# shwetabhardwaj44/EfficientVideoClassification_Youtube8M

Measured on AMD Instinct MI355X. Metric: frames/sec (whole node) H-LSTM teacher+student B=256x300x1152; GAP@20, higher is better.
Workload: dtype bf16; 1 GPU; HierarchicalLstmModel teacher_student every_n=10, lstm_cells=1024x2, MoE(2), batch 256 x 300 x 1152 per GPU; global_batch=256, frames_per_video=300, parallelism=dp1, num_frames=U{120..300}

## Files before the change

efficientvideoclassification_youtube8m_amd/_lib.py:

```python
from __future__ import annotations

import ctypes as C
import os

_HERE = os.path.dirname(os.path.abspath(__file__))
LIB_PATH = os.environ.get("EVC_LIB", os.path.join(_HERE, "libevc_hip.so"))

vp, i32, i64, f32 = C.c_void_p, C.c_int, C.c_int64, C.c_float

SIGNATURES = {
    "evc_check_device": [i32],
    "evc_l2norm_chunk_fwd": [vp, vp, vp, i32, i32, i32, i32, vp, i32, i32, vp, i32, vp, vp, i32, vp, i32, vp, i32, vp],
    "evc_sort_rows_by_len": [vp, i32, i32, vp, vp, vp, vp],
    "evc_frame_counts": [vp, i32, i32, i32, i32, i32, i32, vp, vp, vp, vp],
    "evc_gemm_nt": [vp, i64, vp, i64, vp, i64, i32, i32, i32, vp, i32, i32, vp],
    "evc_gemm_nt_sqnorm": [vp, i64, vp, i64, vp, i64, i32, i32, i32, vp, f32, vp, vp, i64, vp],
    "evc_gemm_tn": [vp, i64, vp, i64, vp, i64, i32, i32, i32, i32, i32, vp],
    "evc_gemm_tn2": [vp, i64, vp, i64, i32, vp, i64, i32, i32, vp, i64, i32, i32, i32, i32, vp],
    "evc_gemm_tn2_rows": [vp, i64, vp, i64, i32, vp, i64, i32, i32, vp, i64, i32, i32, i32, vp, i32, i32, vp],
    "evc_gemm_tn2_slabs": [vp, i64, vp, i64, i32, vp, i64, i32, i32, vp, i64, i64, i32, i32, i32, i32, vp],
    "evc_sum_slabs": [vp, i64, i32, i32, i32, i64, vp, i64, i32, vp],
    "evc_colsum_bf16": [vp, i64, i32, i32, i32, vp, vp],
    "evc_colsum_bf16_det": [vp, i64, i32, i32, i32, vp, vp, i32, vp],
    "evc_lstm_layer_fwd": [vp, vp, vp, vp, i32, i32, i32, i32, i32, vp, vp, vp, vp, i64, vp, vp, vp, vp, vp],
    "evc_lstm_layer_fwd_hp": [vp, vp, i64, vp, i64, vp, vp, i32, i32, i32, i32, vp, vp, vp, vp, vp, i64, vp, vp, vp],
    "evc_gemm_nt_split": [vp, i64, vp, i64, vp, i64, i32, i32, i32, vp, vp],
    "evc_cast_f32_to_f16_wide": [vp, i64, i32, i32, i32, i32, i32, vp, vp],
    "evc_cast_f32_to_bf16_wide": [vp, i64, i32, i32, vp, i64, i32, vp],
    "evc_lstm_layer_fwd_f16": [vp, i64, vp, vp, vp, i32, i32, i32, i32, vp, i32, vp, vp, vp, i64, vp, vp, vp, vp, vp],
    "evc_lstm_layer_fwd_f16_fp8lo": [vp, i64, i32, i64, i32, vp, vp, i32, i32, vp, vp, i32, i32, i32, vp, vp, vp, vp, i64, vp, vp, vp, vp, vp, vp, i32, vp],
    "evc_l2norm_chunk_int": [vp, vp, i32, i32, i32, i32, vp, i32, i32, vp, vp, vp, vp, vp, vp, i32, vp, i32, vp],
    "evc_lstm_level2_fwd_high": [vp, i64, i32, i64, i32, vp, vp, i32, i32, vp, vp, vp, i32, vp, i64, vp, vp, i32, i32, i32, vp, vp, vp, vp, vp, vp, vp, vp, i64,
                                 vp, vp, vp, vp, vp, vp, vp],
    "evc_lstm_layer_fwd_f16_dith": [vp, i64, i32, i64, i32, vp, i64, vp, i64, i32, vp, vp, i32, i32, i32, vp, vp, vp, vp, i64, vp, vp, vp, vp, vp],
    "evc_cast_f32_to_f16_dither": [vp, i64, i32, i64, C.c_uint32, vp, i64, i64, vp],
    "evc_lstm_stack2_fwd_f16_fp8lo": [vp, i32, vp, vp, vp, vp, vp, i32, i32, vp, vp, i32, i32, i32, i32, vp, vp, vp, vp, vp, vp, vp, vp, vp, i64, vp, vp, vp, vp, vp],
    "evc_cast_f32_to_fp8_lo": [vp, i64, i32, i32, i32, i32, i32, vp, i64, vp],
    "evc_cast_f32_to_fp8_lohi": [vp, i64, i32, i32, i32, i32, i32, vp, i64, vp],
    "evc_lstm_layer_bwd": [vp, vp, i32, i32, i32, i32, vp, vp, vp, vp, i64, vp, vp, vp, vp, vp, vp, vp, vp, vp],
    "evc_transpose_to_bf16": [vp, i32, i64, i32, i32, vp, i64, i32, i32, vp],
    "evc_cast_f32_to_bf16": [vp, i64, i32, i32, vp, i64, vp],
    "evc_cast_f32_to_f16": [vp, i64, i32, i32, vp, i64, vp],
    "evc_cast_f32_to_bf16_split": [vp, i64, i32, i32, vp, vp, i64, vp],
    "evc_rowsum_bf16": [vp, i64, i32, i32, vp, vp],
    "evc_lstm_stack2_fwd_f16": [vp, i32, vp, i32, vp, vp, vp, vp, i32, i32, i32, i32, vp, vp, vp, vp, vp, vp, vp, vp, vp, i64, vp, vp, vp, vp, vp],
    "evc_cast_f32_to_f16_segs": [vp, i64, i32, i32, i32, vp, vp],
    "evc_cast_f32_to_f16_wlo": [vp, i64, i32, i32, i32, vp, vp],
    "evc_lstm_level2_fwd": [vp, vp, vp, vp, vp, vp, i32, i32, i32, i32, vp, vp, vp, vp, vp, vp, i64, vp, vp, vp, vp, vp, vp, vp],
    "evc_lstm_stack2_fwd": [vp, vp, vp, vp, vp, vp, i32, i32, i32, i32, vp, vp, vp, vp, vp, vp, vp, i64, vp, vp, vp, vp, vp],
    "evc_moe_grad_update": [vp, i64, vp, i64, i32, i32, i32, vp, vp, vp, vp, vp, i64, f32, vp, vp, f32, f32, f32, f32, f32, vp],
    "evc_moe_grad_update_wide": [vp, i64, vp, i64, i32, i32, i32, vp, vp, vp, vp, vp, i64, vp, vp, vp, i32, i32, f32, vp, vp, f32, f32, f32, f32, f32, vp],
    "evc_gram_slabs": [vp, i64, i32, i32, i32, vp, vp],
    "evc_moe_grad_norms": [vp, i32, vp, i32, i32, vp, i64, vp, i64, vp, i32, i32, f32, vp, vp, vp, vp],
    "evc_moe_grad_update_apply": [vp, i64, vp, i64, i32, i32, i32, vp, vp, vp, vp, vp, i64, vp, vp, vp, i32, i32, f32, vp, vp, f32, f32, f32, f32, f32, vp, vp],
    "evc_gemm_nt_f16_fp8": [vp, i64, vp, i64, vp, i64, vp, i64, vp, i64, i32, i32, i32, i32, i32, vp, vp],
    "evc_cast_f32_to_f16_fp8x": [vp, i64, i32, i32, i32, i32, vp, vp],
    "evc_absmax_partials": [vp, i64, i32, i32, vp, vp],
    "evc_cast_f32_to_f16_fp8x_dyn": [vp, i64, i32, i32, i32, i32, vp, vp, vp],
    "evc_gemm_nt_f16_fp8_dyn": [vp, i64, vp, i64, vp, i64, vp, i64, vp, i64, i32, i32, i32, i32, i32, vp, i32, vp, vp],
    "evc_moe_grad_update_phase": [vp, i64, vp, i64, i32, i32, i32, vp, vp, vp, vp, vp, i64, f32, vp, vp, f32, f32, f32, f32, f32, i32, vp],
    "evc_moe_tail_fwd": [vp, vp, i32, i32, i32, vp, vp, vp],
    "evc_moe_tail_bwd": [vp, vp, vp, i32, i32, i32, vp, i64, vp, i64, vp],
    "evc_ce_loss": [vp, vp, i32, i32, f32, vp, vp, i32, vp],
    "evc_ce_loss_ordered": [vp, vp, i32, i32, f32, vp, vp, i32, vp, vp],
    "evc_rep_loss_ordered": [vp, vp, i32, i32, f32, vp, vp, i32, vp, vp],
    "evc_kl_pred_loss": [vp, vp, vp, vp, i32, i32, f32, vp, vp, i32, vp],
    "evc_kl_pred_loss_ordered": [vp, vp, vp, vp, i32, i32, f32, vp, vp, i32, vp, vp],
    "evc_rep_loss": [vp, vp, i32, i32, f32, vp, vp, i32, vp],
    "evc_distill_losses": [vp, vp, vp, vp, vp, vp, vp, i32, i32, i32, f32, f32, f32, vp, vp, vp, vp, vp],
    "evc_distill_losses_multi": [vp, vp, vp, vp, i32, vp, vp, vp, vp, vp, vp, vp, vp, i32, i32, i32, vp, vp, vp],
    "evc_distill_losses_ensemble": [i32, vp, vp, vp, vp, i32, vp, vp, vp, i32, i32, i32, f32, f32, f32, vp, vp, vp, vp, vp, vp, vp],
    "evc_distill_losses_sparse": [i32, vp, vp, i32, vp, i32, vp, vp, i32, i32, f32, f32, vp, vp, vp, vp, vp],
    "evc_label_loss": [i32, vp, vp, i32, i32, f32, vp, vp, vp, i32, vp, vp],
    "evc_grad_sqnorm": [vp, vp, f32, i64, vp, vp],
    "evc_clip_adam_step": [vp, vp, vp, vp, i64, f32, vp, f32, f32, f32, f32, f32, vp, vp],
    "evc_clip_adam_small": [i32, vp, vp, vp, vp, vp, vp, f32, f32, f32, f32, f32, vp],
    "evc_sqnorm2_partials": [vp, i64, vp, i64, vp, vp],
    "evc_lstm_adam_fused": [vp, vp, vp, vp, vp, vp, vp, vp, i32, i32, vp, vp, vp, f32, f32, f32, f32, f32, vp, vp, i64, vp, i64, i32, i32,
                            vp, i64, i32, i32, i32, i32, i32, vp],
    "evc_adam2d_fused": [vp, vp, vp, vp, i32, i32, vp, vp, f32, f32, f32, f32, f32, vp, vp, i64, vp, i64, vp, i64, i32, i32, i32, vp],
    "evc_meanpool_fwd": [vp, vp, vp, i32, i32, i32, i32, vp, vp, vp],
    "evc_sigmoid_fwd": [vp, i64, vp],
    "evc_sigmoid_bwd": [vp, vp, i64, vp, vp],
    "evc_sample_frames_gather": [vp, vp, vp, vp, i32, i32, i32, i32, i32, vp, vp, vp],
    "evc_sample_sequence_gather": [vp, vp, vp, vp, i32, i32, i32, i32, i32, vp, vp, vp],
    "evc_relu6_fwd": [vp, i64, vp, vp, vp],
    "evc_relu6_bwd": [vp, vp, i64, vp, vp, vp],
    "evc_framepool_mean_fwd": [vp, i32, i32, i32, vp, vp, vp],
    "evc_framepool_mean_bwd": [vp, i32, i32, i32, vp, vp],
    "evc_bn_stats": [vp, i32, i32, vp, vp, vp, vp],
    "evc_bn_apply": [vp, i32, i32, vp, vp, vp, vp, i32, vp, vp, vp],
    "evc_bn_relu6_bwd": [vp, vp, i32, i32, vp, vp, vp, vp, i32, vp, i32, vp, vp, vp, vp, vp, vp],
# ... 14 lines not shown
    "evc_netvlad_softmax_bwd": [vp, vp, i32, i32, vp, vp],
    "evc_netvlad_aggregate_fwd": [vp, vp, i32, i32, i32, i32, vp, vp, vp, vp, vp, vp, vp, vp],
    "evc_netvlad_aggregate_bwd": [vp, vp, i32, i32, i32, i32, vp, vp, vp, vp, vp, vp, vp, vp, vp],
    "evc_netvlad_aggregate_packed_fwd": [vp, vp, vp, i32, i32, i32, i32, i32, i32, vp, vp, vp, vp, vp, vp, vp, vp],
    "evc_netvlad_aggregate_packed_bwd": [vp, vp, vp, i32, i32, i32, i32, i32, i32, vp, vp, vp, vp, vp, vp, vp, vp, vp, i64, vp],
    "evc_netvlad_dcenters": [vp, vp, i32, i32, i32, vp, vp],
    "evc_netvlad_normalize_fwd": [vp, i32, i32, i32, vp, vp, vp, vp, vp],
    "evc_netvlad_normalize_bwd": [vp, vp, vp, vp, i32, i32, i32, vp, vp],
    "evc_nextvlad_assign_fwd": [vp, i32, i32, i32, vp, vp, vp, vp, vp, i64, vp, vp, vp],
    "evc_nextvlad_assign_bwd": [vp, i32, i32, i32, vp, vp, vp, vp, vp, i64, vp, vp, vp, vp, vp, i64, vp],
    "evc_nextvlad_aggregate_fwd": [vp, vp, i32, i32, i32, i32, i32, vp, vp, vp, vp],
    "evc_nextvlad_aggregate_bwd": [vp, vp, i32, i32, i32, i32, i32, vp, vp, vp, vp, vp, i64, vp],
    "evc_nextvlad_aggregate_packed_fwd": [vp, vp, vp, i32, i32, i32, i32, i32, i32, i32, vp, vp, vp, vp],
    "evc_nextvlad_aggregate_packed_fwd_mfma": [vp, vp, vp, i32, i32, i32, i32, i32, i32, i32, vp, vp, vp, vp],
    "evc_nextvlad_aggregate_packed_bwd": [vp, vp, vp, i32, i32, i32, i32, i32, i32, i32, vp, vp, vp, vp, vp, i64, vp],
    "evc_frames_gather_packed": [vp, vp, vp, vp, i32, i32, i32, i32, i32, i32, i32, vp, vp, vp],
    "evc_frames_gather_packed_sel": [vp, vp, vp, vp, vp, i32, i32, i32, i32, i32, i32, i32, i32, vp, vp, vp],
    "evc_scatter_rows": [vp, i64, vp, i32, i32, i32, vp, i64, vp],
    "evc_nextvlad_normalize_fwd": [vp, i32, i32, i32, vp, vp, vp],
    "evc_nextvlad_normalize_bwd": [vp, vp, vp, i32, i32, i32, vp, vp],
    "evc_nextvlad_gate_fwd": [vp, vp, i64, vp, vp],
    "evc_nextvlad_gate_bwd": [vp, vp, vp, i64, vp, vp, vp, vp],
    "evc_nextvlad_gate_bwd_add": [vp, vp, vp, vp, i64, vp, vp, vp, vp],
    "evc_nextvlad_colsum": [vp, i64, i32, i32, vp, vp, i64, vp],
    "evc_nextvlad_center_cast": [vp, i32, i32, vp, vp, vp],
    "evc_nextvlad_bias_logits": [vp, vp, i32, i32, vp, vp, i32, vp],
    "evc_nextvlad_wgrad_uncenter": [vp, vp, vp, i32, i32, vp, vp],
    "evc_nextvlad_dropout_fwd": [vp, i32, i32, vp, vp, vp, vp, C.c_uint32, f32, C.c_uint32, C.c_uint32, C.c_uint64, vp, vp],
    "evc_nextvlad_dropout_bwd": [vp, i32, i32, C.c_uint32, f32, C.c_uint32, C.c_uint32, C.c_uint64, vp],
    "evc_dbof_workspace": [i32, i32, vp, vp, vp],
    "evc_dbof_gather": [vp, vp, vp, vp, i32, i32, i32, i32, i32, vp, vp, vp, vp],
    "evc_bn_partials_reduce": [vp, i32, i32, vp, vp],
    "evc_bn_finalize_ema": [vp, i32, i32, vp, vp, vp, vp, f32, vp],
    "evc_dbof_input_bn_apply": [vp, i32, i32, i32, vp, vp, vp, vp, vp, vp, vp, vp],
    "evc_dbof_cluster_pool_fwd": [vp, vp, vp, vp, i32, i32, i32, i32, vp, vp, vp, vp, vp, vp],
    "evc_dbof_input_bn_apply_f16fp8": [vp, i32, i32, i32, vp, vp, vp, vp, vp, i32, i32, vp, vp],
    "evc_dbof_cluster_pool_fwd_f16fp8": [vp, vp, vp, i32, i32, i32, i32, i32, vp, vp, vp, vp, vp, vp],
    "evc_dbof_pool_finish": [vp, i32, i32, vp, vp, vp, vp, vp, vp, vp, vp],
    "evc_dbof_dact": [vp, vp, vp, vp, vp, vp, vp, vp, i32, i32, i32, i32, vp, vp, vp],
    "evc_gemm_tn_slabs": [vp, i64, vp, i64, vp, i32, i32, i32, i32, vp],
    "evc_dbof_wgrad_finish": [vp, i32, i32, i32, vp, vp, vp, vp, vp, vp, vp],
    "evc_topk_rows": [vp, i32, i32, i32, i32, vp, vp, vp],
    "evc_eval_select_rows": [vp, i32, vp, i32, i32, i32, i32, vp, vp, vp, vp, vp, vp, vp],
    "evc_ensemble_topk_rows": [vp, vp, vp, i32, vp, vp, i32, i32, i32, i32, i32, i32, vp, vp, vp, i64, vp],
    "evc_student_frame_select": [vp, i32, i32, i32, i32, C.c_uint32, C.c_uint32, i32, vp, vp],
    "evc_l2norm_chunk_sel_fwd": [vp, vp, vp, vp, i32, i32, i32, i32, i32, vp, i32, vp, i32, vp, i32, vp],
    "evc_l2norm_chunk_sel_int": [vp, vp, vp, i32, i32, i32, i32, i32, vp, vp, vp, vp, i32, vp],
    "evc_frame_change_keys": [vp, vp, vp, i32, i32, i32, vp, vp],
    "evc_student_frame_select_scored": [vp, vp, i32, i32, i32, i32, vp, vp],
    "evc_cascade_confidence_rows": [vp, i64, vp, i32, i32, i32, i32, vp, vp, i64, vp, vp],
    "evc_cascade_pick_rows": [vp, vp, vp, i32, f32, i32, vp, vp, vp, vp],
}
EXPORTS = tuple(SIGNATURES) + ("evc_version", "evc_last_error")

_lib = None


class EvcError(RuntimeError):
    pass


def load():
    global _lib
    if _lib is not None:
        return _lib
    if not os.path.exists(LIB_PATH):
        raise EvcError(
            "libevc_hip.so not found at %s - build it with "
            "`python -c 'import __graft_entry__ as g; g.build()'` or csrc/build.sh. "
            "There is no CPU fallback for the HIP kernels." % LIB_PATH)
    import torch
    lib = C.CDLL(LIB_PATH)
    for name, args in SIGNATURES.items():
        fn = getattr(lib, name)
        fn.argtypes = args
        fn.restype = C.c_int
    lib.evc_version.argtypes = []
    lib.evc_version.restype = C.c_int
    lib.evc_last_error.argtypes = []
    lib.evc_last_error.restype = C.c_char_p
    _lib = lib
    return lib


def call(name, *args):
    lib = load()
    rc = getattr(lib, name)(*args)
    if rc != 0:
        raise EvcError("%s failed (%d): %s" % (name, rc, lib.evc_last_error().decode()))
```

efficientvideoclassification_youtube8m_amd/csrc/evc_elementwise.hip:

```cpp
#include <stdarg.h>
#include "evc_common.h"
#include <mutex>

static thread_local char g_err[512] = "";
void evc_set_error(const char* fmt, ...) {
  va_list ap;
  va_start(ap, fmt);
  vsnprintf(g_err, sizeof(g_err), fmt, ap);
  va_end(ap);
}
extern "C" const char* evc_last_error(void) { return g_err; }
extern "C" int evc_version(void) { return EVC_VERSION; }
extern "C" int evc_check_device(int dev) {
  hipDeviceProp_t prop;
  EVC_CHECK_HIP(hipGetDeviceProperties(&prop, dev));
  EVC_REQUIRE(strncmp(prop.gcnArchName, "gfx950", 6) == 0, EVC_ERR_UNSUPPORTED_ARCH,
              "device %d is %s; libevc_hip is built for gfx950 only", dev, prop.gcnArchName);
  return EVC_OK;
}

__device__ __forceinline__ float block_sum(float v, float* sh) {
  v = wave_sum(v);
  const int lane = threadIdx.x & 63, w = threadIdx.x >> 6, nw = (blockDim.x + 63) >> 6;
  __syncthreads();
// ... 1748 lines not shown
  for (int s = 1; s < S; ++s) {
    const float v = yp[(long)s * C];
    if (v > best) { best = v; bi = s; }
  }
  const long o = (long)b * C + c;
  if (pf) pf[o] = best;
  if (pb) pb[o] = f32_to_bf16(best);
  if (am) am[o] = bi;
}
extern "C" int evc_framepool_max_fwd(const float* y, int B, int S, int C, float* pooled_f32, evc_bf16* pooled_bf16,
                                     int32_t* argmax, void* stream) {
  EVC_REQUIRE(B > 0 && S > 0 && C > 0, EVC_ERR_BAD_SHAPE, "evc_framepool_max_fwd: bad shape");
  hipLaunchKernelGGL(framepool_max_fwd_kernel, dim3((C + 255) / 256, B), dim3(256), 0, (hipStream_t)stream, y, S, C, pooled_f32,
                     pooled_bf16, argmax);
  EVC_LAUNCH_CHECK();
  return EVC_OK;
}
__global__ void framepool_max_bwd_kernel(const float* __restrict__ dp, const int* __restrict__ am, int S, int C, long n,
                                         float* __restrict__ dy) {
  for (long i = (long)blockIdx.x * blockDim.x + threadIdx.x; i < n; i += (long)gridDim.x * blockDim.x) {
    const int c = (int)(i % C);
    const long bs = i / C;
    const int s = (int)(bs % S);
    const long b = bs / S;
    dy[i] = (am[b * C + c] == s) ? dp[b * C + c] : 0.f;
  }
}
extern "C" int evc_framepool_max_bwd(const float* dpooled, const int32_t* argmax, int B, int S, int C, float* dy, void* stream) {
  EVC_REQUIRE(B > 0 && S > 0 && C > 0, EVC_ERR_BAD_SHAPE, "evc_framepool_max_bwd: bad shape");
  const long n = (long)B * S * C;
  hipLaunchKernelGGL(framepool_max_bwd_kernel, dim3(grid_for(n)), dim3(256), 0, (hipStream_t)stream, dpooled, argmax, S, C, n, dy);
  EVC_LAUNCH_CHECK();
  return EVC_OK;
}

__global__ void fill_kernel(float* p, long n, float v) {
  const long stride = (long)gridDim.x * blockDim.x, tid = (long)blockIdx.x * blockDim.x + threadIdx.x;
  if ((((uintptr_t)p) & 15) == 0) {
    const long n4 = n >> 2;
    const float4 v4 = make_float4(v, v, v, v);
    for (long i = tid; i < n4; i += stride) ((float4*)p)[i] = v4;
    for (long i = (n4 << 2) + tid; i < n; i += stride) p[i] = v;
  } else {
    for (long i = tid; i < n; i += stride) p[i] = v;
  }
}
extern "C" int evc_fill_f32(float* p, int64_t n, float value, void* stream) {
  EVC_REQUIRE(n > 0, EVC_ERR_BAD_SHAPE, "evc_fill_f32: n");
  hipLaunchKernelGGL(fill_kernel, dim3(grid_for(n)), dim3(256), 0, (hipStream_t)stream, p, (long)n, value);
  EVC_LAUNCH_CHECK();
  return EVC_OK;
}

__global__ void occupy_kernel(long long ticks) {
  extern __shared__ char occ_lds[];
  if (threadIdx.x == 0) occ_lds[0] = 0;
  const long long t0 = wall_clock64();
  while (wall_clock64() - t0 < ticks) __builtin_amdgcn_s_sleep(32);
  if (occ_lds[0] == 1) occ_lds[1] = 2;
}
extern "C" int evc_debug_occupy(int blocks, int threads, int lds_bytes, double microseconds, void* stream) {
  EVC_REQUIRE(blocks > 0 && blocks <= 1024 && threads >= 64 && threads <= 1024 && lds_bytes >= 0 && lds_bytes <= 160 * 1024 && microseconds >= 0,
              EVC_ERR_BAD_ARG, "evc_debug_occupy: blocks=%d threads=%d lds=%d us=%g", blocks, threads, lds_bytes, microseconds);
  if (lds_bytes > 64 * 1024) (void)hipFuncSetAttribute((const void*)occupy_kernel, hipFuncAttributeMaxDynamicSharedMemorySize, lds_bytes);
  hipLaunchKernelGGL(occupy_kernel, dim3(blocks), dim3(threads), lds_bytes, (hipStream_t)stream, (long long)(microseconds * 100.0));
  EVC_LAUNCH_CHECK();
  return EVC_OK;
}

extern "C" int evc_stream_create_cu_mask(const unsigned* mask, int words, void** stream_out) {
  EVC_REQUIRE(mask != nullptr && stream_out != nullptr && words > 0 && words <= 32, EVC_ERR_BAD_ARG, "evc_stream_create_cu_mask: words=%d", words);
  hipStream_t s = nullptr;
  hipError_t e = hipExtStreamCreateWithCUMask(&s, (uint32_t)words, mask);
  EVC_REQUIRE(e == hipSuccess, EVC_ERR_HIP, "hipExtStreamCreateWithCUMask: %s", hipGetErrorString(e));
  *stream_out = (void*)s;
  return EVC_OK;
}

extern "C" int evc_stream_destroy(void* stream) {
  EVC_REQUIRE(stream != nullptr, EVC_ERR_BAD_ARG, "evc_stream_destroy: null stream");
  hipError_t e = hipStreamDestroy((hipStream_t)stream);
  EVC_REQUIRE(e == hipSuccess, EVC_ERR_HIP, "hipStreamDestroy: %s", hipGetErrorString(e));
  return EVC_OK;
}
```

efficientvideoclassification_youtube8m_amd/csrc/evc_gemm_tn.hip:

```cpp
#include "gemm_shared.h"

struct StoreParamsT {
  float* C; long ldc; int M, N;
  int row_il_H;
  int accumulate, splits, ksteps_per_split;
  long slab_stride;
};

template <class Cfg, bool SEG = false>
__global__ __launch_bounds__(Cfg::NT) void gemm_tn_kernel(GemmOperandsT p, StoreParamsT s, int tiles_m, int tiles_n) {
  const int nwg = tiles_m * tiles_n;
  int bid = blockIdx.x, split = 0;
  if (s.splits > 1) {
    split = bid / nwg;
    bid -= split * nwg;
  }
  const int id = xcd_remap(bid, nwg);
  int tm, tn;
  tile_of(id, tiles_m, tiles_n, tm, tn, s.splits > 1 ? patch_rows(nwg, tiles_n) : 8);
  const int m0 = tm * Cfg::BM;
  int n0 = tn * Cfg::BU;
  int nb = n0;
  if (p.B2) {
    if (n0 >= p.N1) {
      p.B = p.B2; p.ldb = p.ldb2; nb = n0 - p.N1; p.N = s.N - p.N1;
      s.N = p.c_col2 + p.N;
      n0 = p.c_col2 + nb;
    } else {
      p.N = s.N = p.N1;
    }
  }
  if (SEG) {
    int off = split * s.ksteps_per_split, sg = 0;
    p.nk = min(s.ksteps_per_split, p.nk - off);
#pragma unroll
    for (int i = 0; i < 15; ++i) {
      const bool adv = sg == i && i + 1 < p.nseg && off >= (int)p.seg_len[i];
      off -= adv ? (int)p.seg_len[i] : 0;
      sg += adv ? 1 : 0;
    }
    p.seg0 = sg; p.seg_off0 = off;
  } else if (s.splits > 1) {
    const int k0 = split * s.ksteps_per_split;
    p.A += (long)k0 * 32 * p.lda;
    p.B += (long)k0 * 32 * p.ldb;
    p.nk = min(s.ksteps_per_split, p.nk - k0);
  }
  f32x4 acc[Cfg::MI][1][Cfg::NI];
  gemm_mainloop_tn<Cfg, true, TN_LOOP_MODE, SEG>(p, m0, nb, lds_dyn, acc);
  float* C = s.C + split * s.slab_stride;
  const int wave = threadIdx.x >> 6, wc = wave % Cfg::WC;
  const bool plain = s.slab_stride > 0 || (s.splits == 1 && !s.accumulate);
  const bool aligned = (s.ldc % 4) == 0 && ((uintptr_t)C % 16) == 0 && n0 + wc * Cfg::WU + Cfg::WU <= s.N;
  __syncthreads();
  if (plain && aligned) {
    store_tile_via_lds<Cfg, 4, false>(acc, lds_dyn, C, s.ldc, s.M, s.N, m0, n0, nullptr, s.row_il_H);
  } else if (s.splits == 1 && s.accumulate && aligned) {
    store_tile_via_lds<Cfg, 4, false, true>(acc, lds_dyn, C, s.ldc, s.M, s.N, m0, n0, nullptr, s.row_il_H);
  } else if (plain) {
    TileCoordsT<Cfg> tc;
#pragma unroll
    for (int mi = 0; mi < Cfg::MI; ++mi) {
      const int m = m0 + tc.row0 + mi * 16;
      if (m >= s.M) continue;
      const long mo = s.row_il_H > 0 ? (long)(m & 3) * s.row_il_H + (m >> 2) : m;
#pragma unroll
      for (int ni = 0; ni < Cfg::NI; ++ni)
#pragma unroll
        for (int r = 0; r < 4; ++r) {
          const int n = n0 + tc.unit0 + ni * 16 + r;
          if (n < s.N) C[mo * s.ldc + n] = acc[mi][0][ni][r];
        }
    }
  } else {
    store_tile_via_lds<Cfg, 4, true>(acc, lds_dyn, C, s.ldc, s.M, s.N, m0, n0, nullptr, s.row_il_H);
  }
}

static int tn_args_ok(const char* entry, const void* A, int64_t lda, const void* B, int64_t ldb, int M, int N, int K, int row_interleave_H,
                      int N1, const void* B2, int64_t ldb2, int c_col2, int nslab = 1, bool slabs_ok = true) {
  EVC_REQUIRE(M >= 8 && N >= 8 && K > 0 && M % 8 == 0 && N % 8 == 0 && K % 32 == 0, EVC_ERR_BAD_SHAPE,
              "%s: needs M %% 8 == 0, N %% 8 == 0, K %% 32 == 0 (M=%d N=%d K=%d)", entry, M, N, K);
  EVC_REQUIRE(nslab >= 1 && nslab <= K / 32, EVC_ERR_BAD_SHAPE, "%s: needs 1 <= nslab <= K/32 (K=%d nslab=%d)", entry, K, nslab);
  EVC_REQUIRE(lda % 8 == 0 && ldb % 8 == 0 && ((uintptr_t)A % 16) == 0 && ((uintptr_t)B % 16) == 0, EVC_ERR_BAD_ALIGN,
              "%s: operands must be 16-byte aligned (lda=%ld ldb=%ld)", entry, (long)lda, (long)ldb);
  EVC_REQUIRE(slabs_ok, EVC_ERR_BAD_ALIGN, "%s: slabs == NULL or slab_stride < M * ldc", entry);
  EVC_REQUIRE(row_interleave_H == 0 || M == 4 * row_interleave_H, EVC_ERR_BAD_SHAPE, "%s: row_interleave_H needs M == 4*H", entry);
  EVC_REQUIRE(!B2 || (N1 > 0 && N1 < N && N1 % 256 == 0 && ldb2 % 8 == 0 && ((uintptr_t)B2 % 16) == 0 && c_col2 >= N1), EVC_ERR_BAD_SHAPE,
              "%s: N1=%d must be a multiple of 256 inside (0, N=%d), B2 16-byte aligned with ldb2 %% 8 == 0, c_col2=%d >= N1", entry, N1, N, c_col2);
  EVC_REQUIRE((long)ceil_div(K / 32, nslab) * (nslab - 1) < K / 32, EVC_ERR_BAD_SHAPE, "%s: nslab=%d leaves an empty slab at K=%d", entry, nslab, K);
  return EVC_OK;
}

static inline GemmOperandsT tn_operands(const evc_bf16* A, int64_t lda, const evc_bf16* B, int64_t ldb, int M, int N, int K,
                                        int N1 = 0, const evc_bf16* B2 = nullptr, int64_t ldb2 = 0, int c_col2 = 0) {
  GemmOperandsT p{A, lda, B, ldb, M, N, K / 32};
  if (B2) { p.B2 = B2; p.ldb2 = ldb2; p.N1 = N1; p.c_col2 = c_col2; }
  return p;
}

static bool tn_live_segments(GemmOperandsT& p, int K, int slab_rows, const int32_t* rows_per_slab) {
  if (slab_rows % 32 != 0 || K % slab_rows != 0) return false;
  const int nslabs = K / slab_rows, slab_steps = slab_rows / 32;
  const long ld_max = p.lda > p.ldb ? p.lda : p.ldb;
  if ((long)nslabs * slab_steps >= 65536 || (long)K * (p.B2 && p.ldb2 > ld_max ? p.ldb2 : ld_max) * 2 >= (1L << 32)) return false;
  int n = 0, total = 0;
  for (int t = 0; t < nslabs; ++t) {
    const int r = rows_per_slab[t] < 0 ? 0 : (rows_per_slab[t] > slab_rows ? slab_rows : rows_per_slab[t]);
    const int steps = (r + 31) / 32;
    if (steps == 0) continue;
    if (n == 16) return false;
    p.seg_start[n] = (unsigned short)(t * slab_steps); p.seg_len[n] = (unsigned short)steps;
    ++n; total += steps;
  }
  if (total == 0 || total >= K / 32) return false;
  p.nseg = n; p.nk = total;
  return true;
}

template <class Cfg>
static int launch_tn(const GemmOperandsT& p, StoreParamsT s, bool seg, int tm, int tn, hipStream_t st) {
  s.ksteps_per_split = ceil_div(p.nk, s.splits);
  if (seg) launch_cfg<Cfg>(gemm_tn_kernel<Cfg, true>, tm * tn * s.splits, st, p, s, tm, tn);
  else launch_cfg<Cfg>(gemm_tn_kernel<Cfg>, tm * tn * s.splits, st, p, s, tm, tn);
  EVC_LAUNCH_CHECK();
  return EVC_OK;
}

static int gemm_tn_impl(const char* entry, const evc_bf16* A, int64_t lda, const evc_bf16* B, int64_t ldb, int N1, const evc_bf16* B2, int64_t ldb2,
                        int c_col2, float* C, int64_t ldc, int M, int N, int K, int row_interleave_H, int accumulate, void* stream,
                        int slab_rows = 0, const int32_t* rows_per_slab = nullptr) {
  EVC_TRY(tn_args_ok(entry, A, lda, B, ldb, M, N, K, row_interleave_H, N1, B2, ldb2, c_col2));
  hipStream_t st = (hipStream_t)stream;
  GemmOperandsT p = tn_operands(A, lda, B, ldb, M, N, K, N1, B2, ldb2, c_col2);
  const bool seg = rows_per_slab && slab_rows > 0 && !evc_deterministic() && tn_live_segments(p, K, slab_rows, rows_per_slab);
  K = p.nk * 32;
  StoreParamsT s{C, ldc, M, N, row_interleave_H, accumulate, 1, 0, 0};
  const int tm1 = ceil_div(M, 128), tn1 = ceil_div(N, 128);
  const bool short128 = forced_tile() == 11 || (forced_tile() == 0 && K <= 2048 && (long)tm1 * tn1 >= 192);
  const bool strip128 = !short128 && forced_tile() == 0 && N <= 128 && !B2;
  const bool tile128 = short128 || strip128;
  const int tm = tile128 ? tm1 : ceil_div(M, CfgPlainV2::BM), tn = short128 ? tn1 : strip128 ? 1 : ceil_div(N, CfgPlainV2::BU);
  if (!short128 && !evc_deterministic()) s.splits = split_k(256 / (tm * tn), p.nk, 32);
  if (s.splits > 1 && !accumulate) EVC_CHECK_HIP(hipMemset2DAsync(C, ldc * sizeof(float), 0, (size_t)N * sizeof(float), M, st));
  return tile128 ? launch_tn<CfgTn128>(p, s, seg, tm, tn, st) : launch_tn<CfgPlainV2>(p, s, seg, tm, tn, st);
}

extern "C" int evc_gemm_tn2_rows(const evc_bf16* A, int64_t lda, const evc_bf16* B1, int64_t ldb1, int N1, const evc_bf16* B2, int64_t ldb2,
                                 int N2, int c_col2, float* C, int64_t ldc, int M, int slab_rows, int nslabs, const int32_t* rows_per_slab,
                                 int row_interleave_H, int accumulate, void* stream) {
  EVC_REQUIRE(B1 && N1 > 0 && slab_rows > 0 && nslabs > 0 && rows_per_slab && (long)slab_rows * nslabs < (1L << 31), EVC_ERR_BAD_ARG,
              "evc_gemm_tn2_rows: B1, N1, slab_rows, nslabs, rows_per_slab are required");
  EVC_REQUIRE(!B2 || N2 > 0, EVC_ERR_BAD_ARG, "evc_gemm_tn2_rows: N2=%d", N2);
  EVC_REQUIRE(!B2 || accumulate || c_col2 == N1, EVC_ERR_BAD_ARG, "evc_gemm_tn2_rows: segments that are not adjacent in C (c_col2=%d, N1=%d) need accumulate", c_col2, N1);
  return gemm_tn_impl("evc_gemm_tn2_rows", A, lda, B1, ldb1, B2 ? N1 : 0, B2, ldb2, B2 ? c_col2 : 0, C, ldc, M, N1 + (B2 ? N2 : 0), slab_rows * nslabs,
                      row_interleave_H, accumulate, stream, slab_rows, rows_per_slab);
}

extern "C" int evc_gemm_tn(const evc_bf16* A, int64_t lda, const evc_bf16* B, int64_t ldb, float* C, int64_t ldc,
                           int M, int N, int K, int row_interleave_H, int accumulate, void* stream) {
  return gemm_tn_impl("evc_gemm_tn", A, lda, B, ldb, 0, nullptr, 0, 0, C, ldc, M, N, K, row_interleave_H, accumulate, stream);
}

extern "C" int evc_gemm_tn2(const evc_bf16* A, int64_t lda, const evc_bf16* B1, int64_t ldb1, int N1, const evc_bf16* B2, int64_t ldb2,
                            int N2, int c_col2, float* C, int64_t ldc, int M, int K, int row_interleave_H, int accumulate, void* stream) {
  EVC_REQUIRE(B1 && B2 && N1 > 0 && N2 > 0, EVC_ERR_BAD_ARG, "evc_gemm_tn2: two column segments are required");
  EVC_REQUIRE(accumulate || c_col2 == N1, EVC_ERR_BAD_ARG, "evc_gemm_tn2: segments that are not adjacent in C (c_col2=%d, N1=%d) need accumulate "
              "(the split-K join adds into a C the caller has zeroed)", c_col2, N1);
  return gemm_tn_impl("evc_gemm_tn2", A, lda, B1, ldb1, N1, B2, ldb2, c_col2, C, ldc, M, N1 + N2, K, row_interleave_H, accumulate, stream);
}

static int gemm_tn_slabs_impl(const char* entry, const evc_bf16* A, int64_t lda, const evc_bf16* B1, int64_t ldb1, int N1, const evc_bf16* B2, int64_t ldb2,
                              int N2, int c_col2, float* slabs, int64_t ldc, int64_t slab_stride, int M, int K, int row_interleave_H, int nslab, void* stream) {
  const int N = N1 + (B2 ? N2 : 0);
  EVC_REQUIRE(N1 >= 8, EVC_ERR_BAD_SHAPE, "%s: N1=%d", entry, N1);
  EVC_TRY(tn_args_ok(entry, A, lda, B1, ldb1, M, N, K, row_interleave_H, N1, B2, ldb2, c_col2, nslab, slabs && slab_stride >= (int64_t)M * ldc));
  return launch_tn<CfgPlainV2>(tn_operands(A, lda, B1, ldb1, M, N, K, N1, B2, ldb2, c_col2), StoreParamsT{slabs, ldc, M, N, row_interleave_H, 0, nslab, 0, slab_stride},
                               false, ceil_div(M, CfgPlainV2::BM), ceil_div(N, CfgPlainV2::BU), (hipStream_t)stream);
}
extern "C" int evc_gemm_tn2_slabs(const evc_bf16* A, int64_t lda, const evc_bf16* B1, int64_t ldb1, int N1, const evc_bf16* B2, int64_t ldb2,
                                  int N2, int c_col2, float* slabs, int64_t ldc, int64_t slab_stride, int M, int K, int row_interleave_H,
                                  int nslab, void* stream) {
  return gemm_tn_slabs_impl("evc_gemm_tn2_slabs", A, lda, B1, ldb1, N1, B2, ldb2, N2, c_col2, slabs, ldc, slab_stride, M, K, row_interleave_H, nslab, stream);
}
extern "C" int evc_gemm_tn_slabs(const evc_bf16* A, int64_t lda, const evc_bf16* B, int64_t ldb, float* slabs, int M, int N, int K,
                                 int nslab, void* stream) {
  return gemm_tn_slabs_impl("evc_gemm_tn_slabs", A, lda, B, ldb, N, nullptr, 0, 0, 0, slabs, N, (int64_t)M * N, M, K, 0, nslab, stream);
}

__global__ __launch_bounds__(256) void sum_slabs_kernel(const float* __restrict__ slabs, long slab_stride, int nslab, int M, int N4, long ld,
                                                        float* __restrict__ C, long ldc, int accumulate) {
  const long n = (long)M * N4;
  for (long i = (long)blockIdx.x * 256 + threadIdx.x; i < n; i += (long)gridDim.x * 256) {
    const long r = i / N4, c = (i - r * N4) * 4;
    float4 a = accumulate ? *(const float4*)(C + r * ldc + c) : make_float4(0.f, 0.f, 0.f, 0.f);
    for (int s = 0; s < nslab; ++s) {
      const float4 v = *(const float4*)(slabs + s * slab_stride + r * ld + c);
      a.x += v.x; a.y += v.y; a.z += v.z; a.w += v.w;
    }
    *(float4*)(C + r * ldc + c) = a;
  }
}
extern "C" int evc_sum_slabs(const float* slabs, int64_t slab_stride, int nslab, int M, int N, int64_t ld, float* C, int64_t ldc, int accumulate,
                             void* stream) {
  EVC_REQUIRE(slabs && C && nslab >= 1 && M > 0 && N > 0 && N % 4 == 0 && ld % 4 == 0 && ldc % 4 == 0 && slab_stride % 4 == 0 &&
              ((uintptr_t)slabs % 16) == 0 && ((uintptr_t)C % 16) == 0, EVC_ERR_BAD_SHAPE, "evc_sum_slabs: N, ld, ldc, slab_stride multiples of 4, 16-byte aligned");
  const long n = (long)M * (N / 4);
  long nb = (n + 255) / 256;
  nb = nb > 2048 ? 2048 : nb;
  hipLaunchKernelGGL(sum_slabs_kernel, dim3((unsigned)nb), dim3(256), 0, (hipStream_t)stream, slabs, (long)slab_stride, nslab, M, N / 4, (long)ld, C, (long)ldc,
                     accumulate);
  EVC_LAUNCH_CHECK();
  return EVC_OK;
}

struct MoeUpdateParams {
  float* p; float* m; float* v;
  bf16_t* p_bf16;
  bf16_t* pT_bf16; long ldT;
  bf16_t* p_wide;
  bf16_t* p_f16; uint8_t* p_fp8;
  float lo_scale, hi_scale;
  float* partial;
  float* wsq_partial;
  const float* sums;
  int V, K;
  float l2, clip, lr_t, b1, b2, eps;
};

__device__ __forceinline__ float4 ld_stream_moe(const float* p) {
  const f32x4 v = __builtin_nontemporal_load((const f32x4*)p);
// ... 294 lines not shown
```

efficientvideoclassification_youtube8m_amd/csrc/evc_lstm_bwd.hip:

```cpp
#include "gemm_shared.h"

struct LstmBwdParams {
  const int* len; int t;
  const uint2* gates;
  const bf16_t* c_new; const bf16_t* c_old;
  const float* dS_c; const float* dS_h; long ld_dS;
  const bf16_t* dh_above;
  float* dc_ws;
  int dc_bf16;
  uint2* dz4;
  const int* row_map;
  float* db;
  int m_active;
  int M, H;
  int fused_above;
};

static inline int bwd_dc_bf16() {
  static int v = -1;
  if (v < 0) { const char* e = getenv("EVC_BWD_DC_BF16"); v = (e && e[0] == '1') ? 1 : 0; }
  return v;
}

struct LstmBwdIn {
  int ln;
  float4 dcv;
  float4 dhs;
  uint2 dha;
  uint4 g01, g23;
  uint2 cnq, coq;
};

__device__ __forceinline__ void lstm_bwd_load(const LstmBwdParams& e, const int m, const int u, const bool in_range, LstmBwdIn& q) {
  q.ln = in_range ? e.len[m] : -1;
  q.dcv = q.dhs = make_float4(0.f, 0.f, 0.f, 0.f);
  q.dha = q.cnq = q.coq = make_uint2(0u, 0u);
  q.g01 = q.g23 = make_uint4(0u, 0u, 0u, 0u);
  if (e.t >= q.ln) return;
  const long hu = (long)m * e.H + u;
  if (e.t == q.ln - 1) {
    const long su = (long)(e.row_map ? e.row_map[m] : m) * e.ld_dS + u;
    q.dhs = *(const float4*)(e.dS_h + su);
    q.dcv = *(const float4*)(e.dS_c + su);
  } else {
    if (e.dc_bf16) {
      const uint2 d = *(const uint2*)((const bf16_t*)e.dc_ws + hu);
      q.dcv = make_float4(__uint_as_float(d.x << 16), __uint_as_float(d.x & 0xffff0000u), __uint_as_float(d.y << 16), __uint_as_float(d.y & 0xffff0000u));
    } else {
      q.dcv = *(const float4*)(e.dc_ws + hu);
    }
  }
  if (e.dh_above) q.dha = *(const uint2*)(e.dh_above + hu);
  const uint4* gp = (const uint4*)(e.gates + hu);
  q.g01 = gp[0]; q.g23 = gp[1];
  q.cnq = *(const uint2*)(e.c_new + hu);
  if (e.c_old) q.coq = *(const uint2*)(e.c_old + hu);
}

__device__ __forceinline__ void lstm_bwd_finish(const LstmBwdParams& e, const int m, const int u, const float (&dh_in)[4],
                                                const LstmBwdIn& q, float (&dzv)[4][4]) {
#pragma unroll
  for (int r = 0; r < 4; ++r)
#pragma unroll
    for (int g = 0; g < 4; ++g) dzv[r][g] = 0.f;
  if (q.ln < 0) return;
  const long hu = (long)m * e.H + u;
  uint4* dzp = (uint4*)(e.dz4 + hu);
  if (e.t >= q.ln) {
    dzp[0] = make_uint4(0u, 0u, 0u, 0u);
    dzp[1] = make_uint4(0u, 0u, 0u, 0u);
    return;
  }
  float dh[4] = {dh_in[0], dh_in[1], dh_in[2], dh_in[3]};
  if (e.t == q.ln - 1) {
    if (e.fused_above) { dh[0] += q.dhs.x; dh[1] += q.dhs.y; dh[2] += q.dhs.z; dh[3] += q.dhs.w; }
    else { dh[0] = q.dhs.x; dh[1] = q.dhs.y; dh[2] = q.dhs.z; dh[3] = q.dhs.w; }
  }
  if (e.dh_above) {
    dh[0] += __uint_as_float(q.dha.x << 16); dh[1] += __uint_as_float(q.dha.x & 0xffff0000u);
    dh[2] += __uint_as_float(q.dha.y << 16); dh[3] += __uint_as_float(q.dha.y & 0xffff0000u);
  }
  const float dci[4] = {q.dcv.x, q.dcv.y, q.dcv.z, q.dcv.w};
  const uint2 recs[4] = {make_uint2(q.g01.x, q.g01.y), make_uint2(q.g01.z, q.g01.w), make_uint2(q.g23.x, q.g23.y), make_uint2(q.g23.z, q.g23.w)};
  const float cna[4] = {__uint_as_float(q.cnq.x << 16), __uint_as_float(q.cnq.x & 0xffff0000u),
                        __uint_as_float(q.cnq.y << 16), __uint_as_float(q.cnq.y & 0xffff0000u)};
  const float coa[4] = {__uint_as_float(q.coq.x << 16), __uint_as_float(q.coq.x & 0xffff0000u),
                        __uint_as_float(q.coq.y << 16), __uint_as_float(q.coq.y & 0xffff0000u)};
  float dcn[4];
  uint2 dzr[4];
#pragma unroll
  for (int r = 0; r < 4; ++r) {
    const uint2 rec = recs[r];
    const float gi = __uint_as_float(rec.x << 16), gj = __uint_as_float(rec.x & 0xffff0000u);
    const float gf = __uint_as_float(rec.y << 16), go = __uint_as_float(rec.y & 0xffff0000u);
    const float tcv = tanhf_(cna[r]);
    const float cp = coa[r];
    const float dc = dci[r] + dh[r] * go * (1.f - tcv * tcv);
    dcn[r] = dc * gf;
    dzv[r][0] = dc * gj * gi * (1.f - gi); dzv[r][1] = dc * gi * (1.f - gj * gj);
    dzv[r][2] = dc * cp * gf * (1.f - gf); dzv[r][3] = dh[r] * tcv * go * (1.f - go);
    dzr[r] = make_uint2(pack_bf16x2(dzv[r][0], dzv[r][1]), pack_bf16x2(dzv[r][2], dzv[r][3]));
  }
  if (e.dc_bf16) *(uint2*)((bf16_t*)e.dc_ws + hu) = make_uint2(pack_bf16x2(dcn[0], dcn[1]), pack_bf16x2(dcn[2], dcn[3]));
  else *(float4*)(e.dc_ws + hu) = make_float4(dcn[0], dcn[1], dcn[2], dcn[3]);
  dzp[0] = make_uint4(dzr[0].x, dzr[0].y, dzr[1].x, dzr[1].y);
  dzp[1] = make_uint4(dzr[2].x, dzr[2].y, dzr[3].x, dzr[3].y);
}

template <int BM, int BU, int NT>
__device__ __forceinline__ void lstm_bwd_zero_tile(const LstmBwdParams& e, int m0, int u0) {
  const int cols = min(BU, e.H - u0) / 2;
  for (int i = threadIdx.x; i < BM * cols; i += NT) {
    const int m = m0 + i / cols, u = u0 + (i % cols) * 2;
    if (m < e.M) *(uint4*)(e.dz4 + (long)m * e.H + u) = make_uint4(0u, 0u, 0u, 0u);
  }
}

constexpr int BWD_TAIL_PRE = 8;
template <int N>
struct BwdTailRows {
  unsigned long long dcv[N], dhs[N];
  uint4 grec[N];
  uint32_t cn[N], co[N], dha[N];
};
__device__ __forceinline__ int bwd_tail_len(const LstmBwdParams& e, int m) {
  return m < e.M ? ((const __attribute__((address_space(4))) int*)e.len)[m] : -1;
}
template <int N>
__device__ __forceinline__ void lstm_bwd_tail_load(const LstmBwdParams& e, int m0, int u, bool u_in, int wave, int p0, BwdTailRows<N>& r) {
#pragma unroll
  for (int i = 0; i < N; ++i) {
    const int m = m0 + (p0 + i) * 8 + wave;
    const int ln = u_in ? bwd_tail_len(e, m) : -1;
    r.dcv[i] = r.dhs[i] = 0ull;
    r.grec[i] = make_uint4(0u, 0u, 0u, 0u);
    r.cn[i] = r.co[i] = r.dha[i] = 0u;
    if (e.t < ln) {
      const long hu = (long)m * e.H + u;
      const bool last = e.t == ln - 1;
      long su = 0;
      if (last) su = (long)(e.row_map ? ((const __attribute__((address_space(4))) int*)e.row_map)[m] : m) * e.ld_dS + u;
      if (e.dc_bf16 && !last) {
        const uint32_t d = *(const uint32_t*)((const bf16_t*)e.dc_ws + hu);
        r.dcv[i] = (unsigned long long)(d << 16) | ((unsigned long long)(d & 0xffff0000u) << 32);
      } else {
        r.dcv[i] = *(const unsigned long long*)(last ? e.dS_c + su : e.dc_ws + hu);
      }
      if (last) r.dhs[i] = *(const unsigned long long*)(e.dS_h + su);
      if (e.dh_above) r.dha[i] = *(const uint32_t*)(e.dh_above + hu);
      r.grec[i] = *(const uint4*)(e.gates + hu);
      r.cn[i] = *(const uint32_t*)(e.c_new + hu);
      if (e.c_old) r.co[i] = *(const uint32_t*)(e.c_old + hu);
    }
  }
}
template <int RS, int N>
__device__ __forceinline__ void lstm_bwd_tail_finish(const LstmBwdParams& e, int m0, int u, bool u_in, int lane, int wave, int p0, const BwdTailRows<N>& r,
                                                     const char* lds, float (&bs)[2][4]) {
  float2 dcn[N];
// ... 67 lines not shown
        *(f32x4*)(lds + (wr * Cfg::WM + mi * 16 + l) * RS + (wc * Cfg::WU + ni * 16 + g * 4) * 4) = acc[mi][0][ni];
    __syncthreads();
  }
  const int u = u0 + lane * 2;
  const bool u_in = u < e.H;
  float bs[2][4] = {{0.f, 0.f, 0.f, 0.f}, {0.f, 0.f, 0.f, 0.f}};
  constexpr int SLOTS = Cfg::BM / 8;
  constexpr int GROUP = PRE > 0 ? 8 : 4;
  static_assert(PRE % 4 == 0 && PRE <= SLOTS && (SLOTS - PRE) % GROUP == 0, "tile rows must divide into 8 waves x (PRE + k GROUP)");
  if constexpr (PRE > 0) {
    if constexpr (PRE < SLOTS) {
      BwdTailRows<GROUP> nb;
      lstm_bwd_tail_load<GROUP>(e, m0, u, u_in, wave, PRE, nb);
      lstm_bwd_tail_finish<RS, PRE>(e, m0, u, u_in, lane, wave, 0, pre, lds, bs);
#pragma unroll
      for (int p0 = PRE; p0 < SLOTS; p0 += GROUP) {
        lstm_bwd_tail_finish<RS, GROUP>(e, m0, u, u_in, lane, wave, p0, nb, lds, bs);
        if (p0 + GROUP < SLOTS) lstm_bwd_tail_load<GROUP>(e, m0, u, u_in, wave, p0 + GROUP, nb);
      }
    } else {
      lstm_bwd_tail_finish<RS, PRE>(e, m0, u, u_in, lane, wave, 0, pre, lds, bs);
    }
  } else {
#pragma unroll 1
    for (int p0 = 0; p0 < SLOTS; p0 += GROUP) {
      BwdTailRows<GROUP> cur;
      lstm_bwd_tail_load<GROUP>(e, m0, u, u_in, wave, p0, cur);
      lstm_bwd_tail_finish<RS, GROUP>(e, m0, u, u_in, lane, wave, p0, cur, lds, bs);
    }
  }
  if (e.db) {
    float* red = (float*)lds;
    __syncthreads();
    *(float4*)(red + ((wave * 128) + lane * 2) * 4) = make_float4(bs[0][0], bs[0][1], bs[0][2], bs[0][3]);
    *(float4*)(red + ((wave * 128) + lane * 2 + 1) * 4) = make_float4(bs[1][0], bs[1][1], bs[1][2], bs[1][3]);
    __syncthreads();
    const int uu = threadIdx.x >> 2, gg = threadIdx.x & 3;
    float v = 0.f;
#pragma unroll
    for (int w = 0; w < 8; ++w) v += red[(w * 128 + uu) * 4 + gg];
    if (u0 + uu < e.H) atomicAdd(e.db + (long)gg * e.H + u0 + uu, v);
  }
}

template <class Cfg, bool BATCH_LOADS = true>
__device__ __forceinline__ void lstm_bwd_step_body(const GemmOperands& p, const LstmBwdParams& e, int bid, int tiles_m, int tiles_n) {
  static_assert(Cfg::G == 1, "bwd step is a plain GEMM over the H units");
  const int nwg = tiles_m * tiles_n;
  const int id = xcd_remap(bid, nwg);
  int tm, tn;
  tile_of(id, tiles_m, tiles_n, tm, tn);
  const int m0 = tm * Cfg::BM, u0 = tn * Cfg::BU;
  if (m0 >= e.m_active) {
    lstm_bwd_zero_tile<Cfg::BM, Cfg::BU, Cfg::NT>(e, m0, u0);
    return;
  }
  f32x4 acc[Cfg::MI][1][Cfg::NI];
  constexpr bool ROWMAJOR = is_v2<Cfg>::value && Cfg::BU == 128 && Cfg::NT == 512 && Cfg::BM % 32 == 0 && BATCH_LOADS;
  constexpr int PRE = (ROWMAJOR && (Cfg::BM / 8 - BWD_TAIL_PRE) % 8 == 0 && BWD_TAIL_PRE <= Cfg::BM / 8) ? BWD_TAIL_PRE : 0;
  BwdTailRows<(PRE > 0 ? PRE : 1)> pre;
  if constexpr (PRE > 0) {
    const int lane = threadIdx.x & 63, wave = __builtin_amdgcn_readfirstlane(threadIdx.x >> 6);
    const int u = u0 + lane * 2;
    lstm_bwd_tail_load<PRE>(e, m0, u, u < e.H, wave, 0, pre);
  }
  run_mainloop<Cfg, 1, true, true, BWD_LOOP_MODE>(p, m0, u0, acc);
  if constexpr (ROWMAJOR) {
    lstm_bwd_tail_rowmajor<Cfg, PRE>(acc, e, m0, u0, lds_dyn, pre);
    return;
  }
  TileCoordsT<Cfg> tc;
#pragma unroll
  for (int ni = 0; ni < Cfg::NI; ++ni) {
    const int u = u0 + tc.unit0 + ni * 16;
    if (u >= e.H) continue;
    LstmBwdIn in[BATCH_LOADS ? Cfg::MI : 1];
    if constexpr (BATCH_LOADS) {
#pragma unroll
      for (int mi = 0; mi < Cfg::MI; ++mi) {
        const int m = m0 + tc.row0 + mi * 16;
        lstm_bwd_load(e, m, u, m < e.M, in[mi]);
      }
    }
    float bs[4][4];
#pragma unroll
    for (int r = 0; r < 4; ++r)
#pragma unroll
      for (int g = 0; g < 4; ++g) bs[r][g] = 0.f;
#pragma unroll
    for (int mi = 0; mi < Cfg::MI; ++mi) {
      const int m = m0 + tc.row0 + mi * 16;
      const float dh[4] = {acc[mi][0][ni][0], acc[mi][0][ni][1], acc[mi][0][ni][2], acc[mi][0][ni][3]};
      float dzv[4][4];
      if constexpr (!BATCH_LOADS) lstm_bwd_load(e, m, u, m < e.M, in[0]);
      lstm_bwd_finish(e, m, u, dh, in[BATCH_LOADS ? mi : 0], dzv);
#pragma unroll
      for (int r = 0; r < 4; ++r)
#pragma unroll
        for (int g = 0; g < 4; ++g) bs[r][g] += dzv[r][g];
    }
    if (e.db) {
#pragma unroll
      for (int r = 0; r < 4; ++r)
#pragma unroll
        for (int g = 0; g < 4; ++g) {
          float v = bs[r][g];
          v += __shfl_xor(v, 1, 64); v += __shfl_xor(v, 2, 64); v += __shfl_xor(v, 4, 64); v += __shfl_xor(v, 8, 64);
          if ((threadIdx.x & 15) == 0) atomicAdd(e.db + (long)g * e.H + u + r, v);
        }
    }
  }
}

template <class Cfg>
__global__ __launch_bounds__(Cfg::NT) void lstm_bwd_step_kernel(GemmOperands p, LstmBwdParams e, int tiles_m, int tiles_n) {
  lstm_bwd_step_body<Cfg>(p, e, blockIdx.x, tiles_m, tiles_n);
}

template <class Cfg>
__global__ __launch_bounds__(Cfg::NT, 4) void lstm_bwd_pair_kernel(GemmOperands pa, LstmBwdParams ea, int tma, GemmOperands pb,
                                                                LstmBwdParams eb, int tmb, int tiles_n) {
  const int na = tma * tiles_n;
  const bool first = (int)blockIdx.x < na;
  const GemmOperands p = first ? pa : pb;
  const LstmBwdParams e = first ? ea : eb;
  lstm_bwd_step_body<Cfg, false>(p, e, first ? blockIdx.x : blockIdx.x - na, first ? tma : tmb, tiles_n);
}

template <int KW, int STAGES, bool TWO_SEG>
__device__ __forceinline__ void lstm_bwd_skinny_lds_body(const GemmOperands& p, const LstmBwdParams& e, const int tiles_m, const int tiles_n, const int bid) {
  constexpr int NT = 64 * KW;
  constexpr int STAGE = 8192, RING = STAGES * STAGE;
  float (*part)[32][36] = (float (*)[32][36])lds_dyn;
  const int nwg = tiles_m * tiles_n;
  const int id = xcd_remap(bid, nwg);
  const int tm = id % tiles_m, tn = id / tiles_m;
  const int m0 = tm * 32, u0 = tn * 32;
  if (m0 >= e.m_active) {
    lstm_bwd_zero_tile<32, 32, NT>(e, m0, u0);
    return;
  }
  const int lane = threadIdx.x & 63;
  const int wave = __builtin_amdgcn_readfirstlane(threadIdx.x >> 6);
  char* ring = lds_dyn + wave * RING;
  const int nk = TWO_SEG ? p.nk1 + p.nk2 : p.nk1;
  const int per = (nk + KW - 1) / KW;
  const int k0 = min(wave * per, nk), k1 = min(nk, wave * per + per);
  const int n = k1 - k0;
  const int lc8 = ((lane & 7) ^ ((lane >> 3) & 7)) * 8;
  const bf16_t* asrc[4];
  const bf16_t* bsrc[4];
  long a2off[4], boff[4];
#pragma unroll
  for (int i = 0; i < 4; ++i) {
    const int r = (lane >> 3) + i * 8;
    const int m = min(m0 + r, p.M - 1), u = min(u0 + r, p.Nu - 1);
    asrc[i] = p.A1 + (long)m * p.lda1 + (long)k0 * 64 + lc8;
    bsrc[i] = p.B + (long)u * p.ldb + (long)k0 * 64 + lc8;
    a2off[i] = (long)m * p.lda2 + lc8;
    boff[i] = (long)u * p.ldb + lc8;
  }
  const bf16_t* const b2 = (TWO_SEG && p.B2) ? p.B2 : p.B + (long)p.nk1 * 64;
  auto stage = [&](int j) {
    char* sb = ring + (j % STAGES) * STAGE;
    const int kk = k0 + j;
    const bool s2 = TWO_SEG && kk >= p.nk1;
#pragma unroll
    for (int i = 0; i < 4; ++i) {
      const bf16_t* src = s2 ? p.A2 + a2off[i] + (long)(kk - p.nk1) * 64 : asrc[i] + (long)j * 64;
      __builtin_amdgcn_global_load_lds((const __attribute__((address_space(1))) void*)src,
                                       (__attribute__((address_space(3))) void*)(sb + i * 1024), 16, 0, 0);
    }
#pragma unroll
    for (int i = 0; i < 4; ++i) {
      const bf16_t* src = s2 ? b2 + boff[i] + (long)(kk - p.nk1) * 64 : bsrc[i] + (long)j * 64;
      __builtin_amdgcn_global_load_lds((const __attribute__((address_space(1))) void*)src,
                                       (__attribute__((address_space(3))) void*)(sb + 4096 + i * 1024), 16, 0, 0);
    }
  };
  f32x4 acc[2][2];
#pragma unroll
  for (int i = 0; i < 2; ++i)
#pragma unroll
    for (int j = 0; j < 2; ++j) acc[i][j] = f32x4{0.f, 0.f, 0.f, 0.f};
  const int frow = lane & 15, fq = lane >> 4;
#pragma unroll
  for (int j = 0; j < STAGES - 1; ++j)
    if (j < n) stage(j);
  for (int k = 0; k < n; ++k) {
    const int younger = min(n - 1 - k, STAGES - 2);
    if (younger >= 2) wait_vmcnt<16>();
    else if (younger == 1) wait_vmcnt<8>();
// ... 43 lines not shown
    if (m < e.M && u < e.H) {
      const float dh[4] = {s.x, s.y, s.z, s.w};
      LstmBwdIn in;
      lstm_bwd_load(e, m, u, true, in);
      lstm_bwd_finish(e, m, u, dh, in, dzv);
    }
  }
  if (e.db) {
    __syncthreads();
    float* cs = &part[0][0][0];
#pragma unroll
    for (int r = 0; r < 4; ++r)
#pragma unroll
      for (int g = 0; g < 4; ++g) cs[row * 128 + (ug + r) * 4 + g] = dzv[r][g];
    __syncthreads();
    if (threadIdx.x < 128) {
      float v = 0.f;
#pragma unroll 8
      for (int r = 0; r < 32; ++r) v += cs[r * 128 + threadIdx.x];
      const int u = u0 + (threadIdx.x >> 2), g = threadIdx.x & 3;
      if (u < e.H) atomicAdd(e.db + (long)g * e.H + u, v);
    }
  }
}

template <int KW, int STAGES>
__global__ __launch_bounds__(64 * KW) void lstm_bwd_step_skinny_lds_kernel(GemmOperands p, LstmBwdParams e, int tiles_m, int tiles_n) {
  lstm_bwd_skinny_lds_body<KW, STAGES, false>(p, e, tiles_m, tiles_n, blockIdx.x);
}

template <int KW, int STAGES>
__global__ __launch_bounds__(64 * KW) void lstm_bwd_skinny_pair_kernel(GemmOperands pa, LstmBwdParams ea, GemmOperands pb, LstmBwdParams eb,
                                                                       int tiles_m, int tiles_n) {
  const int n = tiles_m * tiles_n;
  const bool first = blockIdx.x < n;
  const GemmOperands p = first ? pa : pb;
  const LstmBwdParams e = first ? ea : eb;
  lstm_bwd_skinny_lds_body<KW, STAGES, true>(p, e, tiles_m, tiles_n, first ? blockIdx.x : blockIdx.x - n);
}

template <class Cfg>
static inline void launch_lstm_bwd(GemmOperands p, const LstmBwdParams& e, int k1, hipStream_t st) {
  p.nk1 = k1 / kdiv<Cfg>();
  const int tm = ceil_div(e.M, Cfg::BM), tn = ceil_div(e.H, Cfg::BU);
  launch_cfg<Cfg>(lstm_bwd_step_kernel<Cfg>, tm * tn, st, p, e, tm, tn);
}

typedef TileCfg2<128, 1, 128, 2, 4, 5, true> CfgBwdV2_128;
typedef TileCfg3<128, 1, 128, 2, 4, 4> CfgBwdV3_128;
typedef TileCfg3<64, 1, 64, 2, 4, 4> CfgBwdV3_64;
typedef TileCfg2<160, 1, 128, 2, 4, 5, true> CfgBwdV2_160;
typedef TileCfg2<192, 1, 128, 2, 4, 5, true> CfgBwdV2_192;

extern "C" int evc_lstm_layer_bwd(const evc_bf16* w_il, const int32_t* len, int T, int M, int Kin, int H,
                                  const void* gates, const evc_bf16* c_all, const float* dS_c, const float* dS_h, int64_t ld_dS,
                                  const evc_bf16* dh_above, float* dc_ws, evc_bf16* dz4, float* db,
                                  const int32_t* row_map, const int32_t* rows_per_step, const evc_bf16* dz_above,
                                  const evc_bf16* w_above, void* stream) {
  EVC_REQUIRE(T > 0 && M > 0 && H > 0 && Kin > 0 && H % 64 == 0, EVC_ERR_BAD_SHAPE, "evc_lstm_layer_bwd: bad shape");
  EVC_REQUIRE(ring_operand_ok(M, 4L * H) && ring_operand_ok(H, 4L * H), EVC_ERR_BAD_SHAPE,
              "evc_lstm_layer_bwd: a dz time slab spans 4 GiB or more (M=%d H=%d)", M, H);
  EVC_REQUIRE((dz_above != nullptr) == (w_above != nullptr) && !(dz_above && dh_above), EVC_ERR_BAD_ARG,
              "evc_lstm_layer_bwd: dz_above and w_above come together, and instead of dh_above");
  EVC_REQUIRE(!dz_above || (((uintptr_t)dz_above % 16) == 0 && ((uintptr_t)w_above % 16) == 0 && H % 128 == 0), EVC_ERR_BAD_ALIGN,
              "evc_lstm_layer_bwd: dz_above / w_above must be 16-byte aligned, H %% 128 == 0");
  EVC_REQUIRE(gates && c_all && ((uintptr_t)gates % 16) == 0 && ((uintptr_t)c_all % 8) == 0 && ((uintptr_t)dz4 % 16) == 0,
              EVC_ERR_BAD_ALIGN, "evc_lstm_layer_bwd: gates/c_all/dz4 alignment");
  EVC_REQUIRE(ld_dS % 4 == 0 && ((uintptr_t)dS_c % 16) == 0 && ((uintptr_t)dS_h % 16) == 0 && ((uintptr_t)dc_ws % 16) == 0 &&
              (!dh_above || ((uintptr_t)dh_above % 8) == 0), EVC_ERR_BAD_ALIGN, "evc_lstm_layer_bwd: f32 operands must allow 16-byte vector access");
  EVC_TRY(rows_per_step_ok("evc_lstm_layer_bwd", rows_per_step, T, M));
  hipStream_t st = (hipStream_t)stream;
  for (int t = T - 1; t >= 0; --t) {
    const int Mt = rows_per_step ? rows_per_step[t] : M;
    static const int cand[6] = {0, 1, 2, 3, 4, 6};
    static const int bm[7] = {192, 160, 128, 64, 32, 0, 64}, bn[7] = {128, 128, 128, 64, 32, 0, 64};
    static const double cf[7] = {1.0, 1.0, 1.02, 2.0, 1.9, 0.0, 1.36};
    int pick = 3;
    double bc = 1e300;
    const int ma = Mt > 0 ? Mt : 1;
    for (int ci = 0; ci < 6; ++ci) {
      const int i = cand[ci];
      const double c = tile_cost((long)ceil_div(ma, bm[i]) * ceil_div(H, bn[i]), bm[i], bn[i], cf[i]);
      if (c < bc) { bc = c; pick = i; }
    }
    if ((long)ceil_div(ma, 32) * ceil_div(H, 32) <= 512) pick = 5;
    if (forced_tile()) pick = forced_tile() - 1;
    if (dz_above && pick > 2) pick = 2;
    GemmOperands p;
    p.M = M; p.Nu = H; p.group_stride = 0; p.nk1 = p.nk2 = 0;
    p.A1lo = p.A2lo = p.Blo = nullptr;
    p.A1 = dz4 + (long)(t + 1 < T ? t + 1 : t) * M * 4 * H; p.lda1 = 4L * H;
    p.A2 = p.A1; p.lda2 = p.lda1;
    p.B = w_il + (long)Kin * 4 * H; p.ldb = 4L * H;
    const int k1 = (t == T - 1) ? 0 : 4 * H;
    if (dz_above) {
      p.A2 = dz_above + (long)t * M * 4 * H;
      p.nk2 = 4 * H / 32;
      p.B2 = w_above;
    }
    LstmBwdParams e;
    e.len = len; e.t = t;
    e.gates = (const uint2*)gates + (long)t * M * H;
    e.c_new = c_all + (long)(t + 1) * M * H;
    e.c_old = t > 0 ? c_all + (long)t * M * H : nullptr;
    e.dS_c = dS_c; e.dS_h = dS_h; e.ld_dS = ld_dS;
    e.dh_above = dh_above ? dh_above + (long)t * M * H : nullptr;
    e.dc_ws = dc_ws; e.dz4 = (uint2*)dz4 + (long)t * M * H;
    e.dc_bf16 = bwd_dc_bf16();
    e.row_map = row_map; e.db = db; e.m_active = Mt;
    e.M = M; e.H = H; e.fused_above = dz_above ? 1 : 0;
    switch (pick) {
      case 0: launch_lstm_bwd<CfgBwdV2_192>(p, e, k1, st); break;
      case 1: launch_lstm_bwd<CfgBwdV2_160>(p, e, k1, st); break;
      case 2:
        if (dz_above) launch_lstm_bwd<CfgBwdV2_128>(p, e, k1, st);
        else launch_lstm_bwd<CfgBwdV3_128>(p, e, k1, st);
        break;
      case 4: launch_lstm_bwd<CfgPlainTiny>(p, e, k1, st); break;
      case 6: launch_lstm_bwd<CfgBwdV3_64>(p, e, k1, st); break;
      case 5: {
        const int tm = ceil_div(M, 32), tn = ceil_div(H, 32);
        constexpr int KW = 4, STG = 2, LDS = KW * STG * 8192;
        p.nk1 = k1 / 64;
        allow_big_lds((const void*)lstm_bwd_step_skinny_lds_kernel<KW, STG>, LDS);
        hipLaunchKernelGGL((lstm_bwd_step_skinny_lds_kernel<KW, STG>), dim3(tm * tn), dim3(64 * KW), LDS, st, p, e, tm, tn);
        break;
      }
      default: launch_lstm_bwd<CfgPlainSmall>(p, e, k1, st); break;
    }
  }
  EVC_LAUNCH_CHECK();
  return EVC_OK;
}

extern "C" int evc_lstm_stack2_bwd(const evc_bf16* w_il0, const evc_bf16* w_il1, const int32_t* len, int T, int M, int Kin0, int H,
                                   const void* gates0, const evc_bf16* c_all0, const void* gates1, const evc_bf16* c_all1,
                                   const float* dS, int64_t ld_dS, float* dc_ws0, float* dc_ws1, evc_bf16* dz0, evc_bf16* dz1,
                                   float* db0, float* db1, const int32_t* row_map, const int32_t* rows_per_step, void* stream) {
  EVC_REQUIRE(T > 0 && M > 0 && H > 0 && Kin0 > 0 && H % 128 == 0, EVC_ERR_BAD_SHAPE, "evc_lstm_stack2_bwd: bad shape (H %% 128)");
  EVC_REQUIRE(ring_operand_ok(M, 4L * H) && ring_operand_ok(H, 4L * H), EVC_ERR_BAD_SHAPE, "evc_lstm_stack2_bwd: a dz time slab spans 4 GiB or more");
  EVC_REQUIRE(gates0 && gates1 && c_all0 && c_all1 && dz0 && dz1 && dc_ws0 && dc_ws1 && dS, EVC_ERR_BAD_ARG, "evc_lstm_stack2_bwd: null operand");
  EVC_REQUIRE(ld_dS % 4 == 0 && ((uintptr_t)dS % 16) == 0 && ((uintptr_t)dc_ws0 % 16) == 0 && ((uintptr_t)dc_ws1 % 16) == 0 &&
              ((uintptr_t)dz0 % 16) == 0 && ((uintptr_t)dz1 % 16) == 0, EVC_ERR_BAD_ALIGN, "evc_lstm_stack2_bwd: 16-byte alignment");
  EVC_TRY(rows_per_step_ok("evc_lstm_stack2_bwd", rows_per_step, T, M));
  typedef CfgBwdV2_128 Cfg;
  hipStream_t st = (hipStream_t)stream;
  const long slab = (long)M * H;
  const bool skinny = M <= 512;
  const int kdv = skinny ? 64 : 32;
  const int tn = skinny ? ceil_div(H, 32) : ceil_div(H, Cfg::BU), tm = skinny ? ceil_div(M, 32) : ceil_div(M, Cfg::BM);
  constexpr int SKW = 4, SSTG = 2;
  if (skinny) {
    allow_big_lds((const void*)lstm_bwd_skinny_pair_kernel<SKW, SSTG>, SKW * SSTG * 8192);
    allow_big_lds((const void*)lstm_bwd_step_skinny_lds_kernel<SKW, SSTG>, SKW * SSTG * 8192);
  }
  auto base = [&](GemmOperands& p) {
    p.M = M; p.Nu = H; p.group_stride = 0; p.nk1 = p.nk2 = 0;
    p.A1lo = p.A2lo = p.Blo = nullptr; p.B2 = nullptr;
    p.lda1 = p.lda2 = 4L * H; p.ldb = 4L * H;
  };
  auto tail = [&](LstmBwdParams& e, int layer, int t) {
    e.len = len; e.t = t;
    e.gates = (const uint2*)(layer ? gates1 : gates0) + (long)t * slab;
    const evc_bf16* ca = layer ? c_all1 : c_all0;
    e.c_new = ca + (long)(t + 1) * slab;
    e.c_old = t > 0 ? ca + (long)t * slab : nullptr;
    e.dS_c = dS + (long)(2 * layer) * H; e.dS_h = dS + (long)(2 * layer + 1) * H; e.ld_dS = ld_dS;
    e.dh_above = nullptr;
    e.dc_ws = layer ? dc_ws1 : dc_ws0;
    e.dc_bf16 = bwd_dc_bf16();
    e.dz4 = (uint2*)(layer ? dz1 : dz0) + (long)t * slab;
    e.row_map = row_map; e.db = layer ? db1 : db0;
    e.m_active = rows_per_step ? rows_per_step[t] : M;
    e.M = M; e.H = H;
    e.fused_above = layer == 0;
  };
  for (int i = 0; i <= T; ++i) {
    const int t1 = T - 1 - i, t0 = T - i;
    GemmOperands pa, pb;
    LstmBwdParams ea, eb;
    const bool has_a = t0 <= T - 1, has_b = t1 >= 0;
    if (has_a) {
      base(pa);
      pa.A1 = dz0 + (long)(t0 + 1 < T ? t0 + 1 : t0) * slab * 4;
      pa.nk1 = (t0 == T - 1) ? 0 : 4 * H / kdv;
// ... 30 lines not shown
```

efficientvideoclassification_youtube8m_amd/csrc/gemm_core_tn.h:

```cpp
#pragma once
#include "gemm_core_v2.h"

typedef __attribute__((ext_vector_type(4))) short s16x4;

struct GemmOperandsT {
  const bf16_t* A; long lda;
  const bf16_t* B; long ldb;
  int M, N;
  int nk;
  const bf16_t* B2 = nullptr; long ldb2 = 0; int N1 = 0;
  int c_col2 = 0;
  int nseg = 0, seg0 = 0, seg_off0 = 0;
  unsigned short seg_start[16] = {0}, seg_len[16] = {0};
};

__device__ __forceinline__ int tn_h(int row) { return (((row >> 3) & 1) << 2) | (row & 3); }

template <class Cfg, bool SWAP = false, int MODE = 0, bool SEG = false>
__device__ __forceinline__ void gemm_mainloop_tn(const GemmOperandsT& p, const int m0, const int n0, char* lds,
                                                 f32x4 (&acc)[Cfg::MI][1][Cfg::NI]) {
  static_assert(Cfg::G == 1 && Cfg::PIPE && !Cfg::RAGGED, "TN loop: plain tiles, pipelined, even staging");
  const int tid = threadIdx.x;
  const int lane = tid & 63;
  const int wave = __builtin_amdgcn_readfirstlane(tid >> 6);
  const int wr = wave / Cfg::WC, wc = wave % Cfg::WC;
  constexpr int ACPR = Cfg::BM / 8, BCPR = Cfg::BN / 8;
  constexpr int AROWB = Cfg::BM * 2, BROWB = Cfg::BN * 2;

#pragma unroll
  for (int mi = 0; mi < Cfg::MI; ++mi)
#pragma unroll
    for (int ni = 0; ni < Cfg::NI; ++ni) acc[mi][0][ni] = f32x4{0.f, 0.f, 0.f, 0.f};
  const int nk = p.nk;
  if (nk == 0) return;

  constexpr bool PRODUCERS = (MODE & LOOP_PRODUCER) != 0 && Cfg::NT == 512;
  constexpr int NPW = PRODUCERS ? 4 : Cfg::NT / 64;
  const bool producer = wave < NPW;
  constexpr int ACH = Cfg::BM / 16 / NPW, BCH = Cfg::BN / 16 / NPW, PER = ACH + BCH;
  static_assert(ACH * NPW * 16 == Cfg::BM && BCH * NPW * 16 == Cfg::BN, "pieces must divide over the staging waves");
  uint32_t a_vo[ACH], b_vo[BCH];
#pragma unroll
  for (int i = 0; i < ACH; ++i) {
    const int c = ((wave % NPW) + i * NPW) * 64 + lane;
    const int row = c / ACPR, pc = c % ACPR;
    int col = m0 + ((pc ^ (tn_h(row) << 1)) << 3);
    col = col + 8 <= p.M ? col : p.M - 8;
    a_vo[i] = (uint32_t)(((long)row * p.lda + col) * 2);
  }
#pragma unroll
  for (int i = 0; i < BCH; ++i) {
    const int c = ((wave % NPW) + i * NPW) * 64 + lane;
    const int row = c / BCPR, pc = c % BCPR;
    int col = n0 + ((pc ^ (tn_h(row) << 1)) << 3);
    col = col + 8 <= p.N ? col : p.N - 8;
    b_vo[i] = (uint32_t)(((long)row * p.ldb + col) * 2);
  }
  const char* const a_base = (const char*)p.A;
  const char* const b_base = (const char*)p.B;
  const uint32_t a_step = (uint32_t)(64 * p.lda), b_step = (uint32_t)(64 * p.ldb);
  uint32_t a_k = 0, b_k = 0;
  int slot_issue = 0, slot_read = 0;
  uint32_t seg_e[16];
  int seg = 0, seg_left = 0;
  auto seg_entry = [&](int sidx) {
    uint32_t e = 0;
#pragma unroll
    for (int i = 0; i < 16; ++i) e = sidx == i ? seg_e[i] : e;
    return e;
  };
  if constexpr (SEG) {
#pragma unroll
    for (int i = 0; i < 16; ++i) seg_e[i] = ((uint32_t)p.seg_len[i] << 16) | (uint32_t)p.seg_start[i];
    seg = p.seg0;
    const uint32_t e = seg_entry(seg);
    seg_left = (int)(e >> 16) - p.seg_off0;
    a_k = ((e & 0xffffu) + (uint32_t)p.seg_off0) * a_step;
    b_k = ((e & 0xffffu) + (uint32_t)p.seg_off0) * b_step;
  }
  auto advance = [&]() {
    if constexpr (SEG) {
      seg_left -= 1;
      if (__builtin_expect(seg_left == 0, 0)) {
        seg += 1;
        const uint32_t e = seg_entry(seg);
        a_k = (e & 0xffffu) * a_step;
        b_k = (e & 0xffffu) * b_step;
// ... 169 lines not shown
```

efficientvideoclassification_youtube8m_amd/engine.py:

```python
from __future__ import annotations

import math
import os
from collections import OrderedDict

import torch

from . import ops

BF16, F32 = torch.bfloat16, torch.float32


def _align(n, a=16):
    return (n + a - 1) // a * a


def drain(gen):
    try:
        while True:
            next(gen)
    except StopIteration as e:
        return e.value


# ... 15 lines not shown
    def drop_training_state(self):
        self.grad = self.m = self.v = None

    def view(self, buf, k):
        shp = self.shapes[k]
        n = int(math.prod(shp))
        o = self.offsets[k]
        return buf[o:o + n].view(*shp)

    def p(self, k):
        return self.view(self.master, k)

    def g(self, k):
        return self.view(self.grad, k)


class LstmStack:

    def __init__(self, tower, scope, T, M, Kin, training):
        self.tw, self.scope, self.T, self.M, self.Kin = tower, scope, T, M, Kin
        H, L, dev = tower.H, tower.L, tower.device
        self.H, self.L = H, L
        self.S = torch.zeros((M, 2 * L * H), dtype=F32, device=dev)
        self.hbuf = [torch.zeros((T + 1, M, H), dtype=BF16, device=dev) for _ in range(L)]
        self.kin = [Kin] + [H] * (L - 1)
        self.hoist = [M < self.HOIST_BELOW for _ in range(L)]
        self.zx = None
        if any(self.hoist):
            self.zx = torch.empty((T * M, 4 * H), dtype=F32, device=dev)
        self.training = training
        if training:
            self.gates = [torch.empty((T, M, H, 2), dtype=torch.int32, device=dev) for _ in range(L)]
            self.c_all = [torch.empty((T + 1, M, H), dtype=BF16, device=dev) for _ in range(L)]
            self.KP = ops.round_up(T * M, 64)
            self.dz = [torch.zeros((T, M, 4 * H), dtype=BF16, device=dev) for _ in range(L)]
            self.use_tn = (T * M) % 32 == 0 and all(k % 8 == 0 for k in self.kin)
            if not self.use_tn:
                self.dzT = torch.zeros((4 * H, self.KP), dtype=BF16, device=dev)
                self.xT = torch.empty((max(self.kin), self.KP), dtype=BF16, device=dev)
                self.hT_ws = torch.empty((H, self.KP), dtype=BF16, device=dev)
            self.dc_ws = torch.empty((M, H), dtype=F32, device=dev)
            self.dc_ws2 = torch.empty((M, H), dtype=F32, device=dev) if L == 2 else None
            self.dx = [torch.empty((T * M, self.kin[l]), dtype=BF16, device=dev) if (l > 0) else None for l in range(L)]

    def names(self, l):
        base = "%s/rnn/multi_rnn_cell/cell_%d/basic_lstm_cell/" % (self.scope, l)
        return base + "kernel", base + "bias"

    HOIST_BELOW = 1025
    fwd_walk2 = True
    fwd_walk2_high = False
    bwd_fuse = "off"
    small_pair = False
    timing = None
    timing_bwd = None

    def _timed(self, kind, launches, flops, stream=None):
        stack = self

        class _T:
            def __enter__(self_):
                self_.on = stack.timing_bwd is not None and kind in stack.timing_bwd
                if self_.on:
                    self_.e0 = torch.cuda.Event(enable_timing=True)
                    self_.e0.record(stream) if stream is not None else self_.e0.record()

            def __exit__(self_, *exc):
                if self_.on:
                    e1 = torch.cuda.Event(enable_timing=True)
                    e1.record(stream) if stream is not None else e1.record()
                    stack.timing_bwd[kind].append((self_.e0, e1, launches, flops))
                return False
        return _T()

    @staticmethod
    def _v(buf, *shape):
        n = 1
        for d in shape:
            n *= d
        return buf.view(-1)[:n].view(*shape)

    def forward(self, x, lens, plan=None):
        tw, H, L, T = self.tw, self.H, self.L, self.T
        M = plan.P if plan is not None else self.M
        self.plan, self.Mrun = plan, M
        if plan is not None:
            lens = plan.lens
            if plan.rows[0] < self.M:
                self.S.zero_()
        hb = [self._v(h, T + 1, M, H) for h in self.hbuf]
        gates = [self._v(g, T, M, H, 2) for g in self.gates] if self.training else [None] * L
        c_all = [self._v(c, T + 1, M, H) for c in self.c_all] if self.training else [None] * L
        self._hb = hb
        rows = plan.rows if plan is not None else [M] * T
        if isinstance(x, tuple) and x[1].dtype == ops.F16:
            x_bf, x16 = x[0], x[1]
            x_rs = x[2] if len(x) > 2 else None
            self.x_in, self.lens = x_bf, lens
            if self.scope == "RNN_L2" and L == 2 and plan is None:
                if self.zx is None:
                    self.zx = torch.empty((self.T * self.M, 4 * H), dtype=F32, device=self.S.device)
                (k0, b0), (k1, b1) = self.names(0), self.names(1)
                if k1 in tw.shadow8:
                    al = tw.act_lo()
                    wrow = 2 * H if al else 3 * H // 2
                    if not hasattr(self, "hrows16") or self.hrows16[0].shape[-1] != wrow:
                        self.hrows16 = [torch.zeros((self.T + 1, self.M, wrow), dtype=ops.F16, device=h.device) for h in self.hbuf]
                    hr = [self._v(h, T + 1, M, wrow) for h in self.hrows16]
                    ops.lstm_stack2_fwd_f16_fp8lo(x16, tw.shadow16[k0], tw.shadow8[k0], tw.store.p(b0), tw.shadow16[k1], tw.shadow8[k1], tw.store.p(b1),
                                                  lens, T, M, self.Kin, H, self.zx, hr[0], hr[1], hb[0], hb[1], self.S, gates, c_all,
                                                  x_segments=tw.f16_l2_x_segments, h_lo=al)
                    return self.S
                if not hasattr(self, "hbuf16w"):
                    self.hbuf16w = [torch.zeros((self.T + 1, self.M, 2 * H), dtype=ops.F16, device=h.device) for h in self.hbuf]
                hw = [self._v(h, T + 1, M, 2 * H) for h in self.hbuf16w]
                (k0, b0), (k1, b1) = self.names(0), self.names(1)
                ops.lstm_stack2_fwd_f16(x16, tw.shadow16[k0], tw.store.p(b0), tw.shadow16[k1], tw.store.p(b1), lens, T, M, self.Kin, H,
                                        self.zx, hw[0], hw[1], hb[0], hb[1], self.S, gates, c_all,
                                        x_segments=tw.f16_l2_x_segments, h0_ext=tw.f16_l2_h0_ext)
                return self.S
            if self.scope == "RNN_L1" and tw.fp8_lo():
                dl = tw.dither_layers()
                wh0 = tw.dither_wh0()
                al = tw.act_lo()
                widths = [H if (l in dl or (l == 0 and wh0)) else (2 * H if al else 3 * H // 2) for l in range(L)]
                if getattr(self, "_hbuf16_widths", None) != widths:
                    self.hbuf16 = [torch.zeros((self.T + 1, self.M, widths[l]), dtype=ops.F16, device=self.hbuf[l].device) for l in range(L)]
                    self._hbuf16_widths = widths
                h16 = [self._v(self.hbuf16[l], T + 1, M, widths[l]) for l in range(L)]
                assert x16.shape[-1] == (3 * self.Kin // 2 if x_rs is not None else 2 * self.Kin), \
                    "the fp8 L1 level takes ops.l2norm_chunk(..., f16_segments=1, fp8_tail=True) rows (or ops.l2norm_chunk_int's)"
                assert x_rs is None or tw.x_int(), "integer-frame rows need layer 0 on the f16 + e4m3 form (HLstmTower.x_int)"
                inp, ldx, kx16 = x16, x16.shape[-1], self.Kin
                if L == 2 and tuple(dl) == (1,) and not wh0 and self.fwd_walk2_high:
                    (k0, b0), (k1, b1) = self.names(0), self.names(1)
# ... 115 lines not shown
                e0.record()
            ops.lstm_layer_fwd(inp, tw.shadow_fwd[kn], tw.store.p(bn), lens, T, M, self.kin[l], H,
                               hb[l], self.S[:, (2 * l) * H:], self.S[:, (2 * l + 1) * H:], 2 * L * H,
                               gates[l], c_all[l], hoist=self.hoist[l], zx_ws=self.zx, plan=plan)
            if self.timing is not None:
                e1 = torch.cuda.Event(enable_timing=True)
                e1.record()
                kx = 0 if self.hoist[l] else self.kin[l]
                flops = sum(2.0 * r * 4 * H * (kx + (H if t > 0 else 0)) for t, r in enumerate(rows))
                self.timing.append((e0, e1, sum(1 for r in rows if r > 0), flops))
            inp = hb[l][1:]
        return self.S

    def profile_fwd_layers(self, reps=3):
        tw, H, T, M, plan = self.tw, self.H, self.T, self.Mrun, self.plan
        rows = plan.rows if plan is not None else [M] * T
        res = []
        inp = self.x_in
        if self.L == 2 and self.fwd_walk2 and not any(self.hoist) and self.Kin % 64 == 0 and H % 64 == 0:
            (k0, b0), (k1, b1) = self.names(0), self.names(1)
            gates = [self._v(self.gates[l], T, M, H, 2) if self.training else None for l in range(2)]
            c_all = [self._v(self.c_all[l], T + 1, M, H) if self.training else None for l in range(2)]
            args = (inp, tw.shadow_fwd[k0], tw.store.p(b0), tw.shadow_fwd[k1], tw.store.p(b1), self.lens, T, M, self.Kin, H, self._hb[0], self._hb[1],
                    self.S, gates, c_all)
            ops.lstm_level2_fwd(*args, plan=plan)
            e0, e1 = torch.cuda.Event(enable_timing=True), torch.cuda.Event(enable_timing=True)
            e0.record()
            for _ in range(reps):
                ops.lstm_level2_fwd(*args, plan=plan)
            e1.record()
            e1.synchronize()
            flops = sum(2.0 * r * 4 * H * (self.kin[l] + (H if t > 0 else 0)) for l in range(2) for t, r in enumerate(rows))
            live = sum(1 for r in rows if r > 0)
            return [(e0.elapsed_time(e1) / reps, live + 1 if live else 0, flops)]
        for l in range(self.L):
            kn, bn = self.names(l)
            gates = self._v(self.gates[l], T, M, H, 2) if self.training else None
            c_all = self._v(self.c_all[l], T + 1, M, H) if self.training else None
            args = (inp, tw.shadow_fwd[kn], tw.store.p(bn), self.lens, T, M, self.kin[l], H, self._hb[l],
                    self.S[:, (2 * l) * H:], self.S[:, (2 * l + 1) * H:], 2 * self.L * H, gates, c_all)
            ops.lstm_layer_fwd(*args, hoist=self.hoist[l], zx_ws=self.zx, plan=plan)
            e0, e1 = torch.cuda.Event(enable_timing=True), torch.cuda.Event(enable_timing=True)
            e0.record()
            for _ in range(reps):
                ops.lstm_layer_fwd(*args, hoist=self.hoist[l], zx_ws=self.zx, plan=plan)
            e1.record()
            e1.synchronize()
            kx = 0 if self.hoist[l] else self.kin[l]
            flops = sum(2.0 * r * 4 * H * (kx + (H if t > 0 else 0)) for t, r in enumerate(rows))
            res.append((e0.elapsed_time(e1) / reps, sum(1 for r in rows if r > 0), flops))
            inp = self._hb[l][1:]
        return res

    def _wgrad_tn(self, dz2, layer_in, h_prev, kin, rows, gW, live=None):
        H = self.H
        n1 = kin // 256 * 256
        if ops.DETERMINISTIC and rows % 32 == 0 and kin % 8 == 0:
            if n1 >= 256 and (kin == n1 or kin - n1 >= 8):
                ops.gemm_tn_det(dz2, layer_in, 4 * H, n1, rows, gW, row_interleave_H=H, accumulate=True, ldc=kin + H, B2=h_prev, N2=H, c_col2=kin)
                if kin > n1:
                    ops.gemm_tn_det(dz2, layer_in[:, n1:], 4 * H, kin - n1, rows, gW[:, n1:kin], row_interleave_H=H, accumulate=True, ldc=kin + H)
            else:
                ops.gemm_tn_det(dz2, layer_in, 4 * H, kin, rows, gW, row_interleave_H=H, accumulate=True, ldc=kin + H)
                ops.gemm_tn_det(dz2, h_prev, 4 * H, H, rows, gW[:, kin:], row_interleave_H=H, accumulate=True, ldc=kin + H)
            return
        if kin == H and kin % 256 == 0:
            ops.gemm_tn2(dz2, layer_in, kin, h_prev, H, 4 * H, rows, gW, row_interleave_H=H, accumulate=True, live_rows=live)
        elif kin - n1 in (64, 128) and n1 >= H and rows >= 16384 and (n1 + H) % 2048 == 0:
            ops.gemm_tn2(dz2, layer_in, n1, h_prev, H, 4 * H, rows, gW, row_interleave_H=H, accumulate=True, c_col2=kin, live_rows=live)
            ops.gemm_tn(dz2, layer_in[:, n1:], 4 * H, kin - n1, rows, gW[:, n1:kin], row_interleave_H=H, lda=dz2.stride(0),
                        ldb=layer_in.stride(0), ldc=kin + H, accumulate=True, live_rows=live)
        else:
            ops.gemm_tn(dz2, layer_in, 4 * H, kin, rows, gW, row_interleave_H=H, ldc=kin + H, accumulate=True, live_rows=live)
            ops.gemm_tn(dz2, h_prev, 4 * H, H, rows, gW[:, kin:], row_interleave_H=H, ldc=kin + H, accumulate=True, live_rows=live)

    def backward(self, dS, need_dx, aux=None, on_layer_grads=None):
        return drain(self.backward_layers(dS, need_dx, aux, on_layer_grads))

    def backward_layers(self, dS, need_dx, aux=None, on_layer_grads=None):
        tw, H, L, T, plan = self.tw, self.H, self.L, self.T, self.plan
        M = self.Mrun
        assert plan is None or not need_dx, "dX of a row-planned stack would be in slot order"
        dh_above = None
        dx_out = None
        main = torch.cuda.current_stream(tw.device)
        use_tn = (T * M) % 32 == 0 and all(k % 8 == 0 for k in self.kin)
        assert use_tn or not self.use_tn or M == self.M
        fuse_ok = L == 2 and use_tn and not need_dx and M >= 1024 and H % 128 == 0
        small_pair = (L == 2 and self.small_pair and use_tn and M <= 512 and H % 128 == 0 and plan is None and not ops.DETERMINISTIC
                      and self.dc_ws2 is not None)
        if small_pair or (fuse_ok and self.bwd_fuse == "pair"):
            (k0, b0), (k1, b1) = self.names(0), self.names(1)
            dz = [self._v(self.dz[l], T, M, 4 * H) for l in range(2)]
            gb = [tw.store.g(b0), tw.store.g(b1)]
            for g in gb:
                ops.fill_f32(g, 0.0)
            ops.lstm_stack2_bwd(tw.shadow_bwd[k0], tw.shadow_bwd[k1], self.lens, T, M, self.kin[0], H,
                                [self._v(self.gates[l], T, M, H, 2) for l in range(2)],
                                [self._v(self.c_all[l], T + 1, M, H) for l in range(2)], dS,
                                [self._v(self.dc_ws, M, H), self._v(self.dc_ws2, M, H)], dz, gb, plan=plan)
            side = main
            if aux is not None:
                ev = torch.cuda.Event()
                ev.record(main)
                aux.wait_event(ev)
                side = aux
            with torch.cuda.stream(side):
                for l, kn in ((1, k1), (0, k0)):
                    kin = self.kin[l]
                    gW = tw.store.g(kn)
                    dz2 = dz[l].view(T * M, 4 * H)
                    layer_in = (self.x_in if l == 0 else self._hb[0][1:]).reshape(T * M, kin)
                    h_prev = self._hb[l][:T].reshape(T * M, H)
                    ops.fill_f32(gW, 0.0)
                    self._wgrad_tn(dz2, layer_in, h_prev, kin, T * M, gW)
                    if on_layer_grads is not None:
                        on_layer_grads(l)
            if need_dx:
                if self.dx[0] is None:
                    self.dx[0] = torch.empty((T * M, self.kin[0]), dtype=F32, device=tw.device)
                ops.gemm_nt(dz[0].view(T * M, 4 * H), tw.shadow_bwd[k0], T * M, self.kin[0], 4 * H, self.dx[0])
                dx_out = self.dx[0]
            yield 1
            yield 0
            return dx_out
        if fuse_ok and self.bwd_fuse == "fused" and on_layer_grads is not None:
            deferred, user_cb = [], on_layer_grads
            on_layer_grads = deferred.append
        else:
            deferred = user_cb = None
        for l in range(L - 1, -1, -1):
            kn, bn = self.names(l)
            w = tw.shadow_bwd[kn]
            kin = self.kin[l]
            KP = self.KP
            dz = self._v(self.dz[l], T, M, 4 * H)
            gb = tw.store.g(bn)
            det = ops.DETERMINISTIC
            if not det:
                ops.fill_f32(gb, 0.0)
            fused = fuse_ok and self.bwd_fuse == "fused" and l + 1 < L
            rows = plan.rows if plan is not None else [M] * T
            with self._timed("bwd_step", sum(1 for r in rows if r > 0), sum(2.0 * r * H * 4 * H for r in rows[1:])):
                ops.lstm_layer_bwd(w, self.lens, T, M, kin, H, self._v(self.gates[l], T, M, H, 2), self._v(self.c_all[l], T + 1, M, H),
                                   dS[:, (2 * l) * H:], dS[:, (2 * l + 1) * H:], 2 * L * H,
                                   dh_above, self._v(self.dc_ws, M, H), dz, plan=plan, db=None if det else gb,
                                   dz_above=self._v(self.dz[l + 1], T, M, 4 * H) if fused else None,
                                   w_above=tw.shadow_bwd[self.names(l + 1)[0]] if fused else None)
            ops.mark("%s:%s_bptt%d_done" % (tw.scope, self.scope, l))
            dz2 = dz.view(T * M, 4 * H)
            if l > 0 and fuse_ok and self.bwd_fuse == "fused":
                pass
            elif l > 0:
                dxl = self._v(self.dx[l], T * M, kin)
                with self._timed("dx_nt", 1, 2.0 * T * M * kin * 4 * H):
                    ops.gemm_nt(dz2, w, T * M, kin, 4 * H, dxl)
                dh_above = dxl
            elif need_dx:
                if self.dx[0] is None:
                    self.dx[0] = torch.empty((T * M, kin), dtype=F32, device=tw.device)
                ops.gemm_nt(dz2, w, T * M, kin, 4 * H, self.dx[0])
                dx_out = self.dx[0]
            side = main
            if aux is not None:
                ev = torch.cuda.Event()
                ev.record(main)
                aux.wait_event(ev)
                side = aux
            with torch.cuda.stream(side):
                gW = tw.store.g(kn)
                layer_in = (self.x_in if l == 0 else self._hb[l - 1][1:]).reshape(T * M, kin)
                h_prev = self._hb[l][:T].reshape(T * M, H)
                if det:
                    ops.colsum_bf16(dz2, T * M, 4 * H, gb, deinterleave_H=H)
                if use_tn:
                    ops.fill_f32(gW, 0.0)
                    with self._timed("wgrad_tn", 1, 2.0 * (sum(rows) if plan is not None else T * M) * 4 * H * (kin + H), stream=side):
                        self._wgrad_tn(dz2, layer_in, h_prev, kin, T * M, gW, live=(rows, M) if plan is not None and M % 32 == 0 else None)
                else:
                    ops.transpose_to_bf16(dz2, T * M, 4 * H, self.dzT, KP, interleave_H=-H)
                    inT = self.xT[:kin]
                    ops.transpose_to_bf16(layer_in, T * M, kin, inT, KP)
                    ops.transpose_to_bf16(h_prev, T * M, H, self.hT_ws, KP)
                    ops.gemm_nt(self.dzT, inT, 4 * H, kin, KP, gW, ldc=kin + H)
                    ops.gemm_nt(self.dzT, self.hT_ws, 4 * H, H, KP, gW[:, kin:], ldc=kin + H)
                if on_layer_grads is not None:
                    on_layer_grads(l)
                if deferred is not None and l == 0:
                    for ll in deferred:
                        user_cb(ll)
            yield l
        return dx_out


class MoeHead:

    GATES, EXPERTS, EBIAS = "classifier/gates/weights", "classifier/experts/weights", "classifier/experts/biases"

    def __init__(self, tower, K, V, Mx):
        self.tw, self.K, self.V, self.Mx = tower, K, V, Mx

    @staticmethod
    def shapes(K, V, Mx):
        sh = OrderedDict()
        sh[MoeHead.GATES] = (V * (Mx + 1), K)
        sh[MoeHead.EXPERTS] = (V * Mx, K)
        sh[MoeHead.EBIAS] = (V * Mx,)
        return sh

    def alloc(self, B, training):
        dev, K, V, Mx = self.tw.device, self.K, self.V, self.Mx
        self.B = B
        self.Br = ops.round_up(B, 32)
        self.x_full = torch.zeros((self.Br, K), dtype=BF16, device=dev)
        self.x_bf = self.x_full[:B]
        self.gate_logits = torch.empty((B, V * (Mx + 1)), dtype=F32, device=dev)
        self.expert_logits = torch.empty((B, V * Mx), dtype=F32, device=dev)
        self.pred = torch.empty((B, V), dtype=F32, device=dev)
        self.rowsum = torch.empty((B,), dtype=F32, device=dev)
        if training:
            self.Bp = ops.round_up(B, 64)
            self.dgl_full = torch.zeros((self.Br, ops.round_up(V * (Mx + 1), 64)), dtype=BF16, device=dev)
            self.del_full = torch.zeros((self.Br, ops.round_up(V * Mx, 64)), dtype=BF16, device=dev)
            self.dgl, self.del_ = self.dgl_full[:B], self.del_full[:B]
            self.partial_ws = torch.empty(2 * ((V * (Mx + 1) + 127) // 128) * ((K + 127) // 128), dtype=F32, device=dev)
            self.gram_S = {"a": max(1, min(16, self.dgl_full.shape[1] // 32 // 16)), "x": max(1, min(8, K // 32 // 16))}
            self.gram_a = torch.empty(self.gram_S["a"] * self.Br * self.Br, dtype=F32, device=dev) if self.Br <= 512 else None
            self.gram_x = torch.empty(self.gram_S["x"] * self.Br * self.Br, dtype=F32, device=dev) if self.Br <= 512 else None
            self.norm_part = torch.empty(256 + 4 * self.Br, dtype=F32, device=dev)
            self.wsq = torch.zeros((2, 2), dtype=F32, device=dev)
            self._wsq_valid = [False, False]
# ... 950 lines not shown
```

efficientvideoclassification_youtube8m_amd/ops.py:

```python
from __future__ import annotations

import ctypes as C

import os

import torch

from . import _lib

BF16 = torch.bfloat16
F16 = torch.float16
F32 = torch.float32


def _p(t):
    if t is None:
        return None
    if not t.is_cuda:
        raise _lib.EvcError("evc ops need device tensors (got a CPU tensor); there is no CPU path")
    return t.data_ptr()


def _stream():
    return torch.cuda.current_stream().cuda_stream
# ... 2 lines not shown
MARKS = None


def mark(name):
    if MARKS is not None:
        ev = torch.cuda.Event(enable_timing=True)
        ev.record()
        MARKS.append((name, torch.cuda.current_stream().cuda_stream, ev))


def round_up(x, m):
    return (x + m - 1) // m * m


def check_device(dev=0):
    _lib.call("evc_check_device", dev)


def gemm_nt(A, B, M, N, K, out, bias=None, accumulate=False, lda=None, ldb=None, ldc=None):
    assert A.dtype == BF16 and B.dtype == BF16
    lda = A.stride(0) if lda is None else lda
    ldb = B.stride(0) if ldb is None else ldb
    ldc = out.stride(0) if ldc is None else ldc
    _lib.call("evc_gemm_nt", _p(A), lda, _p(B), ldb, _p(out), ldc, M, N, K, _p(bias),
              1 if out.dtype == BF16 else 0, 1 if accumulate else 0, _stream())
    return out


def _slab_rows_arg(live_rows, K):
    rows, slab = live_rows
    assert slab % 32 == 0 and K == slab * len(rows), (K, slab, len(rows))
    return slab, len(rows), (C.c_int32 * len(rows))(*[int(r) for r in rows])


def gemm_nt_sqnorm(A, B, M, N, K, out, p, l2_coeff, sums, ws=None):
    assert A.dtype == BF16 and B.dtype == BF16 and out.dtype == F32 and out.is_contiguous() and (p is None or (p.dtype == F32 and p.shape == out.shape and p.is_contiguous()))
    need = gemm_nt_sqnorm_ws(M, N)
    if ws is None:
        ws = torch.empty(need, dtype=F32, device=out.device)
    assert ws.dtype == F32 and ws.numel() >= need and ws.is_contiguous()
    _lib.call("evc_gemm_nt_sqnorm", _p(A), A.stride(0), _p(B), B.stride(0), _p(out), out.stride(0), M, N, K, _p(p), float(l2_coeff), _p(sums), _p(ws), ws.numel(),
              _stream())
    return out


def gemm_nt_sqnorm_ws(M, N):
    return 16 * ((M + 127) // 128) * ((N + 127) // 128)


def gemm_nt_sqnorm_ok(M, N, K):
    return M > 512 and N % 256 == 0 and K % 64 == 0 and K < 8192 and os.environ.get("EVC_FUSED_GRAD_NORM", "0") == "1"


def gemm_tn(A, B, M, N, K, out, row_interleave_H=0, accumulate=False, lda=None, ldb=None, ldc=None, live_rows=None):
    assert A.dtype == BF16 and B.dtype == BF16 and out.dtype == F32
    if live_rows is not None:
        slab, ns, arr = _slab_rows_arg(live_rows, K)
        _lib.call("evc_gemm_tn2_rows", _p(A), A.stride(0) if lda is None else lda, _p(B), B.stride(0) if ldb is None else ldb, N, None, 0, 0, 0,
                  _p(out), out.stride(0) if ldc is None else ldc, M, slab, ns, arr, row_interleave_H, 1 if accumulate else 0, _stream())
        return out
    _lib.call("evc_gemm_tn", _p(A), A.stride(0) if lda is None else lda, _p(B), B.stride(0) if ldb is None else ldb,
              _p(out), out.stride(0) if ldc is None else ldc, M, N, K, row_interleave_H, 1 if accumulate else 0, _stream())
    return out


def gemm_tn_det(A, B, M, N, K, out, row_interleave_H=0, accumulate=False, ldc=None, B2=None, N2=0, c_col2=None):
    assert A.dtype == BF16 and B.dtype == BF16 and out.dtype == F32
    ldc = out.stride(0) if ldc is None else ldc
    ntot = (c_col2 + N2) if B2 is not None else N
    tiles = ((M + 255) // 256) * ((N + N2 + 255) // 256)
    nslab = max(1, min(256 // max(1, tiles), K // 1024))
    while nslab > 1 and ((K // 32 + nslab - 1) // nslab) * (nslab - 1) >= K // 32:
        nslab -= 1
    ws = torch.empty((nslab, M, ntot), dtype=F32, device=out.device)
    _lib.call("evc_gemm_tn2_slabs", _p(A), A.stride(0), _p(B), B.stride(0), N, _p(B2), B2.stride(0) if B2 is not None else 0, N2,
              (c_col2 if c_col2 is not None else N), _p(ws), ntot, M * ntot, M, K, row_interleave_H, nslab, _stream())
    for c0, w in ((0, N),) + (((c_col2, N2),) if B2 is not None else ()):
        _lib.call("evc_sum_slabs", _p(ws[0, :, c0:]), M * ntot, nslab, M, w, ntot, _p(out[:, c0:]), ldc, 1 if accumulate else 0, _stream())
    return out


def gemm_tn2(A, B1, N1, B2, N2, M, K, out, row_interleave_H=0, accumulate=False, ldc=None, c_col2=None, live_rows=None):
    assert A.dtype == BF16 and B1.dtype == BF16 and B2.dtype == BF16 and out.dtype == F32
    if live_rows is not None:
        slab, ns, arr = _slab_rows_arg(live_rows, K)
        _lib.call("evc_gemm_tn2_rows", _p(A), A.stride(0), _p(B1), B1.stride(0), N1, _p(B2), B2.stride(0), N2, N1 if c_col2 is None else c_col2,
                  _p(out), out.stride(0) if ldc is None else ldc, M, slab, ns, arr, row_interleave_H, 1 if accumulate else 0, _stream())
        return out
    _lib.call("evc_gemm_tn2", _p(A), A.stride(0), _p(B1), B1.stride(0), N1, _p(B2), B2.stride(0), N2, N1 if c_col2 is None else c_col2,
              _p(out), out.stride(0) if ldc is None else ldc, M, K, row_interleave_H, 1 if accumulate else 0, _stream())
    return out


def fill_f32(t, value):
    assert t.dtype == F32 and t.is_contiguous()
    _lib.call("evc_fill_f32", _p(t), t.numel(), float(value), _stream())


DETERMINISTIC = os.environ.get("EVC_DETERMINISTIC", "0") not in ("", "0")


def colsum_bf16(x, R, C, out, deinterleave_H=0):
    if DETERMINISTIC and R >= 128:
        ws = torch.empty((128, C), dtype=F32, device=x.device)
        _lib.call("evc_colsum_bf16_det", _p(x), x.stride(0), R, C, deinterleave_H, _p(out), _p(ws), 128, _stream())
        return out
    _lib.call("evc_colsum_bf16", _p(x), x.stride(0), R, C, deinterleave_H, _p(out), _stream())
    return out


def transpose_to_bf16(x, R, C, out, Rpad, ld_in=None, interleave_H=0):
    ld_in = x.stride(0) if ld_in is None else ld_in
    _lib.call("evc_transpose_to_bf16", _p(x), 1 if x.dtype == F32 else 0, ld_in, R, C, _p(out), out.stride(0), Rpad,
              interleave_H, _stream())
    return out


def cast_bf16(x, out=None):
    x2 = x.reshape(-1, x.shape[-1]) if x.dim() > 1 else x.reshape(1, -1)
    if out is None:
        out = torch.empty(x.shape, dtype=BF16, device=x.device)
    o2 = out.reshape(x2.shape)
    _lib.call("evc_cast_f32_to_bf16", _p(x2), x2.stride(0), x2.shape[0], x2.shape[1], _p(o2), o2.stride(0), _stream())
    return out


def cast_f16(x, out):
    assert x.dtype == F32 and out.dtype == F16 and x.dim() == 2
    _lib.call("evc_cast_f32_to_f16", _p(x), x.stride(0), x.shape[0], x.shape[1], _p(out), out.stride(0), _stream())
    return out


def cast_f16_wide(w, Kin, H, nseg, out, h_ext=False):
    assert w.dtype == F32 and out.dtype == F16 and w.shape[1] == Kin + H and out.is_contiguous()
    assert out.shape == (w.shape[0], nseg * Kin + (2 if h_ext else 1) * H)
    _lib.call("evc_cast_f32_to_f16_wide", _p(w), w.stride(0), w.shape[0], Kin, H, nseg, 1 if h_ext else 0, _p(out), _stream())
    return out


def cast_f16_segs(x, nseg, out):
    assert x.dtype == F32 and out.dtype == F16 and out.shape == (x.shape[0], nseg * x.shape[1]) and out.is_contiguous()
    _lib.call("evc_cast_f32_to_f16_segs", _p(x), x.stride(0), x.shape[0], x.shape[1], nseg, _p(out), _stream())
    return out


def cast_f16_wlo(w, Kin, H, out):
    assert w.dtype == F32 and out.dtype == F16 and w.shape[1] == Kin + H and out.shape == (w.shape[0], 2 * (Kin + H)) and out.is_contiguous()
    _lib.call("evc_cast_f32_to_f16_wlo", _p(w), w.stride(0), w.shape[0], Kin, H, _p(out), _stream())
    return out

# ... 315 lines not shown


def cast_f16_dither(p, out, seed, col0=0):
    assert p.dtype == F32 and p.is_contiguous() and out.dtype == F16 and out.is_contiguous() and out.shape[1:] == p.shape
    assert col0 == 0 or (p.dim() == 2 and 0 < col0 <= p.shape[1])
    _lib.call("evc_cast_f32_to_f16_dither", _p(p), p.numel(), out.shape[0], out.stride(0) if out.shape[0] > 1 else p.numel(), int(seed) & 0xFFFFFFFF, _p(out),
              p.shape[1] if col0 else 0, col0, _stream())


def lstm_level2_fwd(x, wT0, bias0, wT1, bias1, lens, T, M, Kin, H, hbuf0, hbuf1, S, gates=(None, None), c_all=(None, None), plan=None):
    assert x.dtype == BF16 and wT0.dtype == BF16 and wT1.dtype == BF16 and hbuf0.dtype == BF16 and hbuf1.dtype == BF16
    _lib.call("evc_lstm_level2_fwd", _p(x), _p(wT0), _p(bias0), _p(wT1), _p(bias1), _p(lens), T, M, Kin, H, _p(hbuf0), _p(hbuf1),
              _p(S[:, 0:]), _p(S[:, H:]), _p(S[:, 2 * H:]), _p(S[:, 3 * H:]), S.stride(0),
              _p(gates[0]), _p(c_all[0]), _p(gates[1]), _p(c_all[1]), *_plan_args(plan), _stream())


def lstm_stack2_fwd(x, wT0, bias0, wT1, bias1, lens, T, M, Kin, H, zx_ws, hbuf0, hbuf1, S, gates=(None, None), c_all=(None, None)):
    _lib.call("evc_lstm_stack2_fwd", _p(x), _p(wT0), _p(bias0), _p(wT1), _p(bias1), _p(lens), T, M, Kin, H, _p(zx_ws),
              _p(hbuf0), _p(hbuf1), _p(S[:, 0:]), _p(S[:, H:]), _p(S[:, 2 * H:]), _p(S[:, 3 * H:]), S.stride(0),
              _p(gates[0]), _p(c_all[0]), _p(gates[1]), _p(c_all[1]), _stream())


def lstm_stack2_fwd_f16(x16, wT0_16, bias0, wT1_wlo, bias1, lens, T, M, Kin, H, zx_ws, h0_wide, h1_wide, hbuf0, hbuf1, S,
                        gates=(None, None), c_all=(None, None), x_segments=1, h0_ext=False):
    assert x16.dtype == F16 and wT0_16.dtype == F16 and wT1_wlo.dtype == F16 and h0_wide.dtype == F16 and hbuf0.dtype == BF16
    assert x16.shape[-1] == x_segments * Kin and wT0_16.shape[1] == x_segments * Kin + (2 if h0_ext else 1) * H
    _lib.call("evc_lstm_stack2_fwd_f16", _p(x16), x_segments, _p(wT0_16), 1 if h0_ext else 0, _p(bias0), _p(wT1_wlo), _p(bias1), _p(lens),
              T, M, Kin, H, _p(zx_ws),
              _p(h0_wide), _p(h1_wide), _p(hbuf0), _p(hbuf1), _p(S[:, 0:]), _p(S[:, H:]), _p(S[:, 2 * H:]), _p(S[:, 3 * H:]), S.stride(0),
              _p(gates[0]), _p(c_all[0]), _p(gates[1]), _p(c_all[1]), _stream())


def lstm_stack2_fwd_f16_fp8lo(x16, wT0_16, wT0_8, bias0, wT1_16, wT1_8, bias1, lens, T, M, Kin, H, zx_ws, h0_rows, h1_rows, hbuf0, hbuf1, S,
                              gates=(None, None), c_all=(None, None), x_segments=1, w8_scale_exp=FP8_W_SCALE_EXP, h_lo=False):
    k8 = 2 if h_lo else 1
    assert x16.dtype == F16 and wT0_16.dtype == F16 and wT1_16.dtype == F16 and wT0_8.dtype == torch.uint8 and wT1_8.dtype == torch.uint8
    assert x16.shape[-1] == x_segments * Kin and wT0_16.shape == (4 * H, x_segments * Kin + H) and wT0_8.shape == (4 * H, k8 * H)
    assert wT1_16.shape == (4 * H, 2 * H) and wT1_8.shape == (4 * H, 2 * k8 * H) and h0_rows.dtype == F16 and hbuf0.dtype == BF16
    assert h0_rows.shape[-1] == h1_rows.shape[-1] == (2 * H if h_lo else 3 * H // 2)
    assert all(t.is_contiguous() for t in (wT0_16, wT0_8, wT1_16, wT1_8))
    _lib.call("evc_lstm_stack2_fwd_f16_fp8lo", _p(x16), x_segments, _p(wT0_16), _p(wT0_8), _p(bias0), _p(wT1_16), _p(wT1_8), w8_scale_exp, 1 if h_lo else 0, _p(bias1),
              _p(lens), T, M, Kin, H, _p(zx_ws), _p(h0_rows), _p(h1_rows), _p(hbuf0), _p(hbuf1),
              _p(S[:, 0:]), _p(S[:, H:]), _p(S[:, 2 * H:]), _p(S[:, 3 * H:]), S.stride(0),
              _p(gates[0]), _p(c_all[0]), _p(gates[1]), _p(c_all[1]), _stream())


def lstm_layer_fwd_hp(x_lohi, wx_hilo, wh_hilo, bias, lens, T, M, Kin, H, zx_ws, hbuf, hbuf_lohi, c_state, h_state, ld_state,
                      gates=None, c_all=None):
    _lib.call("evc_lstm_layer_fwd_hp", _p(x_lohi), _p(wx_hilo), wx_hilo.stride(0), _p(wh_hilo), wh_hilo.stride(0), _p(bias), _p(lens),
              T, M, Kin, H, _p(zx_ws), _p(hbuf), _p(hbuf_lohi), _p(c_state), _p(h_state), ld_state, _p(gates), _p(c_all), _stream())


def lstm_layer_bwd(w_il, lens, T, M, Kin, H, gates, c_all, dS_c, dS_h, ld_dS, dh_above, dc_ws, dz4, plan=None, db=None,
                   dz_above=None, w_above=None):
    _lib.call("evc_lstm_layer_bwd", _p(w_il), _p(lens), T, M, Kin, H, _p(gates), _p(c_all), _p(dS_c), _p(dS_h), ld_dS,
              _p(dh_above), _p(dc_ws), _p(dz4), _p(db), *_plan_args(plan), _p(dz_above), _p(w_above), _stream())


def lstm_stack2_bwd(w_il0, w_il1, lens, T, M, Kin0, H, gates, c_all, dS, dc_ws, dz, db, plan=None):
    _lib.call("evc_lstm_stack2_bwd", _p(w_il0), _p(w_il1), _p(lens), T, M, Kin0, H, _p(gates[0]), _p(c_all[0]), _p(gates[1]),
              _p(c_all[1]), _p(dS), dS.stride(0), _p(dc_ws[0]), _p(dc_ws[1]), _p(dz[0]), _p(dz[1]), _p(db[0]), _p(db[1]),
              *_plan_args(plan), _stream())


TOPK_MAX_K = 256


def topk_rows(x, k):
    if x.dtype != F32 or x.dim() != 2 or (x.shape[0] > 0 and x.shape[1] > 1 and x.stride(1) != 1):
        raise _lib.EvcError("topk_rows: needs a 2-D float32 tensor with contiguous rows (got %s %s)" % (x.dtype, tuple(x.shape)))
    B, cols = x.shape
    kk = max(int(k), 0)
    values = torch.empty((B, kk), dtype=F32, device=x.device)
    indices = torch.empty((B, kk), dtype=torch.int32, device=x.device)
    ld = x.stride(0) if B > 1 else cols
    _lib.call("evc_topk_rows", _p(x), ld, B, cols, int(k), _p(values), _p(indices), _stream())
    return values, indices


def eval_select_rows(predictions, labels, k):
    x, y = predictions, labels
    if x.dtype != F32 or x.dim() != 2 or (x.shape[0] > 0 and x.shape[1] > 1 and x.stride(1) != 1):
        raise _lib.EvcError("eval_select_rows: needs 2-D float32 predictions with contiguous rows (got %s %s)" % (x.dtype, tuple(x.shape)))
    if y.dtype != torch.uint8 or y.dim() != 2 or tuple(y.shape) != tuple(x.shape) or (y.shape[0] > 0 and y.shape[1] > 1 and y.stride(1) != 1):
        raise _lib.EvcError("eval_select_rows: needs uint8 labels of the predictions' shape %s with contiguous rows (got %s %s)"
                            % (tuple(x.shape), y.dtype, tuple(y.shape)))
    if y.device != x.device:
        raise _lib.EvcError("eval_select_rows: predictions on %s, labels on %s" % (x.device, y.device))
    B, cols = x.shape
    kk = max(int(k), 0)
    out = {"top_val": torch.empty((B, kk), dtype=F32, device=x.device), "top_idx": torch.empty((B, kk), dtype=torch.int32, device=x.device),
           "top_lab": torch.empty((B, kk), dtype=torch.uint8, device=x.device), "n_pos": torch.empty((B,), dtype=torch.int32, device=x.device),
           "perr_hits": torch.empty((B,), dtype=torch.int32, device=x.device),
           "class_pos": torch.zeros((cols,), dtype=torch.int32, device=x.device)}
    _lib.call("evc_eval_select_rows", _p(x), x.stride(0) if B > 1 else cols, _p(y), y.stride(0) if B > 1 else cols, B, cols, int(k),
              _p(out["top_val"]), _p(out["top_idx"]), _p(out["top_lab"]), _p(out["n_pos"]), _p(out["perr_hits"]), _p(out["class_pos"]),
              _stream())
    return out


ENSEMBLE_MAX_MEMBERS = 8
ENSEMBLE_MAX_PRIORS = 8
ENSEMBLE_MAX_KP = 256
ENSEMBLE_MODES = {"max": 0, "mean": 1}


def ensemble_topk_rows(preds, k, mode="max", weights=None, priors=None, dense=False):
# ... 772 lines not shown
```

include/evc.h:

```cpp
#ifndef EVC_H_
#define EVC_H_

#include <stdint.h>

#ifdef __cplusplus
extern "C" {
#endif

#define EVC_OK 0
#define EVC_ERR_BAD_SHAPE (-1)
#define EVC_ERR_BAD_ALIGN (-2)
#define EVC_ERR_UNSUPPORTED_ARCH (-3)
#define EVC_ERR_HIP (-4)
#define EVC_ERR_BAD_ARG (-5)

#define EVC_VERSION 107

typedef uint16_t evc_bf16;
typedef uint16_t evc_f16;

int evc_version(void);
const char* evc_last_error(void);
int evc_check_device(int dev);

// ... 27 lines not shown

int evc_lstm_layer_fwd_hp(const evc_bf16* x_lohi, const evc_bf16* wx_hilo, int64_t ldwx, const evc_bf16* wh_hilo, int64_t ldwh,
                          const float* bias, const int32_t* len, int T, int M, int Kin, int H, float* zx_ws,
                          evc_bf16* hbuf, evc_bf16* hbuf_lohi, float* c_state, float* h_state, int64_t ld_state,
                          void* gates, evc_bf16* c_all, void* stream);
int evc_lstm_layer_fwd_f16(const evc_f16* x, int64_t ldx ,
                           const evc_f16* wT, const float* bias, const int32_t* len,
                           int T, int M, int Kin, int H, evc_f16* hbuf,
                           int h_wide ,
                           evc_bf16* hbuf_bf16,
                           float* c_state, float* h_state, int64_t ld_state, void* gates, evc_bf16* c_all,
                           const int32_t* row_map, const int32_t* rows_per_step, void* stream);
int evc_lstm_layer_fwd_f16_fp8lo(const evc_f16* x, int64_t ldx, int kx16, int64_t x8_off, int kx8, const evc_f16* wT16,
                                 const uint8_t* wT8, int w8_scale_exp, int h_lo, const float* bias, const int32_t* len,
                                 int T, int M, int H, evc_f16* hbuf, evc_bf16* hbuf_bf16, float* c_state, float* h_state,
                                 int64_t ld_state, void* gates, evc_bf16* c_all, const int32_t* row_map,
                                 const int32_t* rows_per_step, const float* x_row_scale, const float* x_col_const, int b8_gap, void* stream);
int evc_lstm_layer_fwd_f16_dith(const evc_f16* x, int64_t ldx, int kx16, int64_t x8_off, int kx8, const evc_f16* wT16,
                                int64_t w16_step_stride, const uint8_t* wT8, int64_t ldb8, int scale8_exp, const float* bias,
                                const int32_t* len, int T, int M, int H, evc_f16* hbuf, evc_bf16* hbuf_bf16, float* c_state,
                                float* h_state, int64_t ld_state, void* gates, evc_bf16* c_all, const int32_t* row_map,
                                const int32_t* rows_per_step, void* stream);
int evc_lstm_level2_fwd_high(const evc_f16* x, int64_t ldx, int kx16, int64_t x8_off, int kx8, const evc_f16* wT16_0, const uint8_t* wT8_0,
                             int w8_scale_exp, int h_lo, const float* bias0, const float* x_row_scale, const float* x_col_const, int b8_gap,
                             const evc_f16* wT16_1, int64_t w16_step_stride, const float* bias1, const int32_t* len, int T, int M, int H,
                             evc_f16* hbuf0, evc_bf16* hbuf0_bf16, evc_f16* hbuf1, evc_bf16* hbuf1_bf16, float* c_state0, float* h_state0,
                             float* c_state1, float* h_state1, int64_t ld_state, void* gates0, evc_bf16* c_all0, void* gates1, evc_bf16* c_all1,
                             const int32_t* row_map, const int32_t* rows_per_step, void* stream);
int evc_lstm_stack2_fwd_f16(const evc_f16* x, int x_segments ,
                            const evc_f16* wT0, int h0_ext , const float* bias0,
                            const evc_f16* wT1_wlo, const float* bias1,
                            const int32_t* len, int T, int M, int Kin, int H, float* zx_ws,
                            evc_f16* h0_wide, evc_f16* h1_wide, evc_bf16* hbuf0, evc_bf16* hbuf1,
                            float* c_state0, float* h_state0, float* c_state1, float* h_state1, int64_t ld_state,
                            void* gates0, evc_bf16* c_all0, void* gates1, evc_bf16* c_all1, void* stream);
int evc_lstm_stack2_fwd_f16_fp8lo(const evc_f16* x, int x_segments, const evc_f16* wT0, const uint8_t* wT0_8, const float* bias0,
                                  const evc_f16* wT1, const uint8_t* wT1_8, int w8_scale_exp, int h_lo, const float* bias1,
                                  const int32_t* len, int T, int M, int Kin, int H, float* zx_ws,
                                  evc_f16* h0_rows, evc_f16* h1_rows, evc_bf16* hbuf0, evc_bf16* hbuf1,
                                  float* c_state0, float* h_state0, float* c_state1, float* h_state1, int64_t ld_state,
                                  void* gates0, evc_bf16* c_all0, void* gates1, evc_bf16* c_all1, void* stream);
int evc_lstm_stack2_fwd(const evc_bf16* x, const evc_bf16* wT0, const float* bias0, const evc_bf16* wT1, const float* bias1,
                        const int32_t* len, int T, int M, int Kin, int H, float* zx_ws,
                        evc_bf16* hbuf0, evc_bf16* hbuf1, float* c_state0, float* h_state0, float* c_state1,
                        float* h_state1, int64_t ld_state, void* gates0, evc_bf16* c_all0, void* gates1,
                        evc_bf16* c_all1, void* stream);


int evc_lstm_layer_bwd(const evc_bf16* w_il, const int32_t* len, int T, int M, int Kin, int H,
                       const void* gates, const evc_bf16* c_all, const float* dS_c, const float* dS_h, int64_t ld_dS,
                       const evc_bf16* dh_above, float* dc_ws, evc_bf16* dz4, float* db,
                       const int32_t* row_map, const int32_t* rows_per_step, const evc_bf16* dz_above,
                       const evc_bf16* w_above, void* stream);

int evc_moe_grad_update(const evc_bf16* dlogits, int64_t ld_dlogits, const evc_bf16* x, int64_t ldx, int rows,
                        int V, int K, float* p, float* m, float* v, evc_bf16* p_bf16, evc_bf16* pT_bf16, int64_t ldT,
                        float l2_coeff, float* sums, float* partial_ws, float clip_norm, float lr_t,
                        float beta1, float beta2, float eps, void* stream);
int evc_moe_grad_update_phase(const evc_bf16* dlogits, int64_t ld_dlogits, const evc_bf16* x, int64_t ldx, int rows,
                              int V, int K, float* p, float* m, float* v, evc_bf16* p_bf16, evc_bf16* pT_bf16, int64_t ldT,
                              float l2_coeff, float* sums, float* partial_ws, float clip_norm, float lr_t,
                              float beta1, float beta2, float eps, int phase, void* stream);
int evc_gram_slabs(const evc_bf16* A, int64_t lda, int R, int Kc, int S, float* slabs, void* stream);
int evc_moe_grad_norms(const float* gram_a, int SA, const float* gram_x, int SX, int R, const evc_bf16* dlogits, int64_t ld_dlogits,
                       const float* logits, int64_t ld_logits, const float* bias, int B, int V, float l2_coeff, const float* wsq,
                       float* part_ws, float* sums, void* stream);
int evc_moe_grad_update_apply(const evc_bf16* dlogits, int64_t ld_dlogits, const evc_bf16* x, int64_t ldx, int rows,
                              int V, int K, float* p, float* m, float* v, evc_bf16* p_bf16, evc_bf16* pT_bf16, int64_t ldT,
                              evc_bf16* p_wide_hilo, evc_f16* p_f16, uint8_t* p_fp8, int fp8_lo_exp, int fp8_hi_exp,
                              float l2_coeff, const float* sums, float* partial_ws, float clip_norm, float lr_t,
                              float beta1, float beta2, float eps, float* wsq_out, void* stream);
int evc_moe_grad_update_wide(const evc_bf16* dlogits, int64_t ld_dlogits, const evc_bf16* x, int64_t ldx, int rows,
                             int V, int K, float* p, float* m, float* v, evc_bf16* p_bf16, evc_bf16* pT_bf16, int64_t ldT,
                             evc_bf16* p_wide_hilo, evc_f16* p_f16, uint8_t* p_fp8, int fp8_lo_exp, int fp8_hi_exp,
                             float l2_coeff, float* sums, float* partial_ws, float clip_norm, float lr_t,
                             float beta1, float beta2, float eps, void* stream);

int evc_transpose_to_bf16(const void* in, int in_f32, int64_t ld_in, int R, int C,
                          evc_bf16* out, int64_t ld_out, int Rpad, int interleave_H, void* stream);
int evc_cast_f32_to_bf16(const float* in, int64_t ld_in, int R, int C, evc_bf16* out, int64_t ld_out, void* stream);
int evc_cast_f32_to_fp8_lo(const float* in, int64_t ld_in, int R, int C, int lo_exp, int hi_cols, int hi_exp, uint8_t* out, int64_t ld_out,
                           void* stream);
int evc_cast_f32_to_fp8_lohi(const float* in, int64_t ld_in, int R, int C, int lo_exp, int hi_cols, int hi_exp, uint8_t* out, int64_t ld_out,
                             void* stream);
int evc_cast_f32_to_f16(const float* in, int64_t ld_in, int R, int C, evc_f16* out, int64_t ld_out, void* stream);
int evc_cast_f32_to_f16_dither(const float* in, int64_t n, int T, int64_t img_stride, uint32_t seed, evc_f16* out, int64_t row_len, int64_t col0,
                               void* stream);
int evc_cast_f32_to_f16_wide(const float* in, int64_t ld_in, int R, int Kin, int H, int nseg, int h_ext, evc_f16* out, void* stream);
int evc_cast_f32_to_f16_segs(const float* in, int64_t ld_in, int R, int C, int nseg, evc_f16* out, void* stream);
int evc_cast_f32_to_f16_wlo(const float* in, int64_t ld_in, int R, int Kin, int H, evc_f16* out, void* stream);
int evc_cast_f32_to_bf16_wide(const float* in, int64_t ld_in, int R, int C, evc_bf16* out, int64_t ld_out, int lo_first, void* stream);
int evc_gemm_nt_split(const evc_bf16* A_lohi, int64_t lda, const evc_bf16* B_hilo, int64_t ldb, float* C, int64_t ldc,
                      int M, int N, int K, const float* bias, void* stream);
int evc_gemm_nt_f16_fp8(const evc_f16* A16, int64_t lda, const uint8_t* A8, int64_t lda8, const evc_f16* B16, int64_t ldb,
                        const uint8_t* B8, int64_t ldb8, float* C, int64_t ldc, int M, int N, int K16, int K8, int scale_exp,
                        const float* bias, void* stream);
int evc_cast_f32_to_f16_fp8x(const float* in, int64_t ld_in, int R, int C, int hi_exp, int lo_exp, evc_f16* out, void* stream);
int evc_absmax_partials(const float* in, int64_t ld_in, int R, int C, float* ws, void* stream);
int evc_cast_f32_to_f16_fp8x_dyn(const float* in, int64_t ld_in, int R, int C, int hi_exp, int lo_exp, const float* amax_ws, evc_f16* out, void* stream);
int evc_gemm_nt_f16_fp8_dyn(const evc_f16* A16, int64_t lda, const uint8_t* A8, int64_t lda8, const evc_f16* B16, int64_t ldb,
                            const uint8_t* B8, int64_t ldb8, float* C, int64_t ldc, int M, int N, int K16, int K8, int scale_exp,
                            const float* amax_ws, int a8_hi_exp, const float* bias, void* stream);
int evc_cast_f32_to_bf16_split(const float* in, int64_t ld_in, int R, int C, evc_bf16* hi, evc_bf16* lo,
                               int64_t ld_out, void* stream);
int evc_rowsum_bf16(const evc_bf16* in, int64_t ld_in, int R, int C, float* out, void* stream);
int evc_colsum_bf16(const evc_bf16* in, int64_t ld_in, int R, int C, int deinterleave_H, float* out, void* stream);
// ... 77 lines not shown
                       double* ws , void* stream);
int evc_bn_bwd_finalize(const float* x, const float* dy, int R, int R_total, int C, const float* mean,
                        const float* var, const float* gamma, const float* beta, int relu6,
                        const int32_t* argmax, int S, const double* ws, float* dx_f32, evc_bf16* dx_bf16,
                        float* dgamma, float* dbeta, void* stream);
int evc_bn_relu6_bwd(const float* x, const float* dy, int R, int C, const float* mean, const float* var,
                     const float* gamma, const float* beta, int relu6, const int32_t* argmax, int S,
                     double* ws ,
                     float* dx_f32, evc_bf16* dx_bf16, float* dgamma, float* dbeta, void* stream);
int evc_bn_relu6_framepool_fwd(const float* act, int B, int S, int C, const float* mean, const float* var,
                               const float* gamma, const float* beta, float* pooled_f32, evc_bf16* pooled_bf16,
                               int32_t* argmax, void* stream);
int evc_framepool_max_fwd(const float* y, int B, int S, int C, float* pooled_f32, evc_bf16* pooled_bf16,
                          int32_t* argmax, void* stream);
int evc_framepool_max_bwd(const float* dpooled, const int32_t* argmax, int B, int S, int C, float* dy, void* stream);

int evc_lstm_level2_fwd(const evc_bf16* x, const evc_bf16* wT0, const float* bias0, const evc_bf16* wT1, const float* bias1,
                        const int32_t* len, int T, int M, int Kin, int H, evc_bf16* hbuf0, evc_bf16* hbuf1,
                        float* c_state0, float* h_state0, float* c_state1, float* h_state1, int64_t ld_state,
                        void* gates0, evc_bf16* c_all0, void* gates1, evc_bf16* c_all1,
                        const int32_t* row_map, const int32_t* rows_per_step, void* stream);

int evc_lstm_stack2_bwd(const evc_bf16* w_il0, const evc_bf16* w_il1, const int32_t* len, int T, int M, int Kin0, int H,
                        const void* gates0, const evc_bf16* c_all0, const void* gates1, const evc_bf16* c_all1,
                        const float* dS, int64_t ld_dS, float* dc_ws0, float* dc_ws1, evc_bf16* dz0, evc_bf16* dz1,
                        float* db0, float* db1, const int32_t* row_map, const int32_t* rows_per_step, void* stream);

int evc_dbof_workspace(int B, int S, int32_t* padded_rows, int32_t* gather_part_rows, int32_t* gemm_part_rows);
int evc_dbof_gather(const float* x_f32, const uint8_t* x_u8, const float* u, const int32_t* num_frames, int B, int T,
                    int F, int S, int normalize, float* r, int32_t* idx_out, float* part, void* stream);
int evc_bn_partials_reduce(const float* part, int P, int C, double* ws, void* stream);
int evc_bn_finalize_ema(const double* ws, int R_total, int C, float* mean, float* var, float* moving_mean,
                        float* moving_var, float decay, void* stream);
int evc_dbof_input_bn_apply(const float* r, int B, int S, int F, const float* mean, const float* var, const float* gamma,
                            const float* beta, evc_bf16* r_bn, evc_bf16* r_bn_lo, evc_bf16* xhat, void* stream);
int evc_dbof_cluster_pool_fwd(const evc_bf16* r_bn, const evc_bf16* r_bn_lo, const evc_bf16* wT, const evc_bf16* wT_lo,
                              int B, int S, int F, int C, const float* gamma, evc_bf16* act, float* part, float* xsel,
                              uint8_t* arg, void* stream);
int evc_dbof_input_bn_apply_f16fp8(const float* r, int B, int S, int F, const float* mean, const float* var, const float* gamma,
                                   const float* beta, evc_f16* r_rows, int hi_exp, int lo_exp, evc_bf16* xhat, void* stream);
int evc_dbof_cluster_pool_fwd_f16fp8(const evc_f16* r_rows, const evc_f16* wT16, const uint8_t* wT8, int scale_exp,
                                     int B, int S, int F, int C, const float* gamma, evc_bf16* act, float* part, float* xsel,
                                     uint8_t* arg, void* stream);
int evc_dbof_pool_finish(const float* xsel, int B, int C, const float* mean, const float* var, const float* gamma,
                         const float* beta, float* pooled_f32, evc_bf16* pooled_bf16, evc_bf16* pooled_lo, void* stream);
int evc_dbof_dact(evc_bf16* act, const float* dpooled, const float* pooled, const uint8_t* arg, const float* mean,
                  const float* var, const float* gamma, const double* ws, int R_total, int B, int S, int C, float* dgamma,
                  float* dbeta, void* stream);
int evc_gemm_tn2(const evc_bf16* A, int64_t lda, const evc_bf16* B1, int64_t ldb1, int N1, const evc_bf16* B2, int64_t ldb2,
                 int N2, int c_col2, float* C, int64_t ldc, int M, int K, int row_interleave_H, int accumulate, void* stream);
int evc_gemm_tn2_rows(const evc_bf16* A, int64_t lda, const evc_bf16* B1, int64_t ldb1, int N1, const evc_bf16* B2, int64_t ldb2,
                      int N2, int c_col2, float* C, int64_t ldc, int M, int slab_rows, int nslabs, const int32_t* rows_per_slab,
                      int row_interleave_H, int accumulate, void* stream);
int evc_gemm_tn_slabs(const evc_bf16* A, int64_t lda, const evc_bf16* B, int64_t ldb, float* slabs, int M, int N, int K,
                      int nslab, void* stream);
int evc_gemm_tn2_slabs(const evc_bf16* A, int64_t lda, const evc_bf16* B1, int64_t ldb1, int N1, const evc_bf16* B2, int64_t ldb2,
                       int N2, int c_col2, float* slabs, int64_t ldc, int64_t slab_stride, int M, int K, int row_interleave_H,
                       int nslab, void* stream);
int evc_sum_slabs(const float* slabs, int64_t slab_stride, int nslab, int M, int N, int64_t ld, float* C, int64_t ldc, int accumulate,
                  void* stream);
int evc_dbof_wgrad_finish(const float* slabs, int nslab, int C, int F, const float* W, const float* gamma_in, float* dW,
                          float* dgamma_in, float* dbeta_in, float* part_ws, void* stream);

int evc_netvlad_softmax_fwd(const float* act, int R, int K, const float* mean, const float* var, const float* gamma,
                            const float* beta, float* a, void* stream);
int evc_netvlad_softmax_bwd(const float* a, const float* da, int R, int K, float* dz, void* stream);
int evc_netvlad_aggregate_fwd(const float* a, const float* r, int B, int S, int K, int F, const float* mean, const float* var,
                              const float* gamma, const float* beta, const float* c2, float* V, float* asum, void* stream);
int evc_netvlad_aggregate_bwd(const float* a, const float* r, int B, int S, int K, int F, const float* mean, const float* var,
                              const float* gamma, const float* beta, const float* c2, const float* dV, float* da, float* dx,
                              void* stream);
int evc_netvlad_dcenters(const float* asum, const float* dV, int B, int K, int F, float* dc2, void* stream);
int evc_netvlad_normalize_fwd(const float* V, int B, int K, int F, float* n1, float* n2, float* Y_f32, evc_bf16* Y_bf16,
                              void* stream);
int evc_netvlad_normalize_bwd(const float* V, const float* n1, const float* n2, const float* dY, int B, int K, int F, float* dV,
                              void* stream);
int evc_netvlad_aggregate_packed_fwd(const float* a, const float* r, const int32_t* row_off, int B, int T, int K, int F, int R, int max_k,
                                     const float* mean, const float* var, const float* gamma, const float* beta, const float* c2,
                                     float* V, float* asum, void* stream);
int evc_netvlad_aggregate_packed_bwd(const float* a, const float* r, const int32_t* row_off, int B, int T, int K, int F, int R, int max_k,
                                     const float* mean, const float* var, const float* gamma, const float* beta, const float* c2,
                                     const float* dV, float* da, float* dx, float* ws, int64_t ws_floats, void* stream);

int evc_nextvlad_assign_fwd(const float* act, int R, int G, int K, const float* mean, const float* var, const float* gamma,
                            const float* beta, const float* att_logits, int64_t ld_att, const float* att_bias, float* a, void* stream);
int evc_nextvlad_assign_bwd(const float* act, int R, int G, int K, const float* mean, const float* var, const float* gamma,
                            const float* beta, const float* att_logits, int64_t ld_att, const float* att_bias, const float* da,
                            float* dz, float* datt_logit, evc_bf16* datt_logit_bf16, int64_t ld_bf16, void* stream);
int evc_nextvlad_aggregate_fwd(const float* a, const float* xe, int B, int S, int G, int K, int D, const float* c2, float* V,
                               float* asum, void* stream);
int evc_nextvlad_aggregate_bwd(const float* a, const float* xe, int B, int S, int G, int K, int D, const float* c2, const float* dV,
                               float* da, float* dxe, float* ws, int64_t ws_floats, void* stream);
int evc_nextvlad_aggregate_packed_fwd(const float* a, const float* xe, const int32_t* row_off, int B, int T, int G, int K, int D, int R,
                                      int max_k, const float* c2, float* V, float* asum, void* stream);
int evc_nextvlad_aggregate_packed_bwd(const float* a, const float* xe, const int32_t* row_off, int B, int T, int G, int K, int D, int R,
                                      int max_k, const float* c2, const float* dV, float* da, float* dxe, float* ws, int64_t ws_floats,
                                      void* stream);
int evc_nextvlad_aggregate_packed_fwd_mfma(const float* a, const float* xe, const int32_t* row_off, int B, int T, int G, int K, int D,
                                           int R, int max_k, const float* c2, float* V, float* asum, void* stream);
int evc_frames_gather_packed(const float* x, const uint8_t* x_u8, const int32_t* num_frames, const int32_t* row_off, int B, int T, int F,
                             int every_n, int R, int Rp, int normalize, float* out, evc_bf16* out_bf16, void* stream);
int evc_frames_gather_packed_sel(const float* x, const uint8_t* x_u8, const int32_t* num_frames, const int32_t* row_off, const int32_t* sel,
                                 int B, int Bsel, int T, int F, int every_n, int R, int Rp, int normalize, float* out, evc_bf16* out_bf16,
                                 void* stream);
int evc_scatter_rows(const float* src, int64_t ld_src, const int32_t* sel, int n, int rows_dst, int C, float* dst, int64_t ld_dst, void* stream);
int evc_nextvlad_normalize_fwd(const float* V, int B, int K, int D, float* U, float* norms, void* stream);
// ... 14 lines not shown
int evc_sqnorm2_partials(const float* ga, int64_t na, const float* gb, int64_t nb, float* part, void* stream);
int evc_lstm_adam_fused(float* p, const float* g, float* m, float* v, float* pb, const float* gb, float* mb, float* vb, int H, int C,
                        const float* part, float* sums_w, float* sums_b, float clip_norm, float lr_t, float beta1, float beta2, float eps,
                        evc_bf16* p_bf16, evc_bf16* pT_bf16, int64_t ldT, evc_f16* p_f16, int64_t ld16, int nin, int nseg,
                        uint8_t* p_fp8, int64_t ld8, int fp8_col0, int fp8_hi_cols, int fp8_lo_exp, int fp8_hi_exp, int fp8_hi_tail, void* stream);

int evc_sample_sequence_gather(const float* x, const uint8_t* x_u8, const float* u, const int32_t* num_frames, int B, int T, int F,
                               int S, int normalize, float* out, int32_t* idx_out, void* stream);
int evc_relu6_fwd(const float* x, int64_t n, float* y_f32, evc_bf16* y_bf16, void* stream);
int evc_relu6_bwd(const float* x, const float* dy, int64_t n, float* dx_f32, evc_bf16* dx_bf16, void* stream);
int evc_framepool_mean_fwd(const float* y, int B, int S, int C, float* pooled_f32, evc_bf16* pooled_bf16, void* stream);
int evc_framepool_mean_bwd(const float* dpooled, int B, int S, int C, float* dy, void* stream);
int evc_colsum_bf16_det(const evc_bf16* in, int64_t ld_in, int R, int C, int deinterleave_H, float* out, float* ws, int ws_rows, void* stream);
int evc_adam2d_fused(float* p, const float* g, float* m, float* v, int R, int C, const float* part, float* sums_w, float clip_norm, float lr_t,
                     float beta1, float beta2, float eps, evc_bf16* p_bf16, evc_bf16* pT_bf16, int64_t ldT, evc_f16* p_f16, int64_t ld16,
                     uint8_t* p_fp8, int64_t ld8, int fp8_hi_cols, int fp8_lo_exp, int fp8_hi_exp, void* stream);

int evc_topk_rows(const float* x, int ld, int rows, int cols, int k, float* out_val, int32_t* out_idx, void* stream);
int evc_eval_select_rows(const float* pred, int ld, const uint8_t* labels, int ld_lab, int rows, int cols, int k, float* top_val,
                         int32_t* top_idx, uint8_t* top_lab, int32_t* n_pos, int32_t* perr_hits, int32_t* class_pos, void* stream);
int evc_ensemble_topk_rows(const float* const* preds, const int64_t* ld, const float* weights, int M, const int32_t* prior_idx,
                           const float* prior_val, int P, int kp, int rows, int cols, int mode, int k, float* out_val, int32_t* out_idx,
                           float* out_dense, int64_t ld_dense, void* stream);

#define EVC_SELECT_UNIFORM 0
#define EVC_SELECT_FIRST 1
#define EVC_SELECT_MIDDLE 2
#define EVC_SELECT_LAST 3
#define EVC_SELECT_FIRST_MIDDLE_LAST 4
#define EVC_SELECT_RANDOM 5
int evc_student_frame_select(const int32_t* num_frames, int B, int T, int every_n, int strategy, uint32_t seed, uint32_t draw, int row0,
                             int32_t* src, void* stream);
int evc_l2norm_chunk_sel_fwd(const float* x_raw, const uint8_t* x_u8, const int32_t* num_frames, const int32_t* src, int B, int T, int F,
                             int every_n, int C2, evc_bf16* out2, int normalize, evc_bf16* out2_lo, int aux_mode,
                             const int32_t* row_pos2, int rows2, void* stream);
int evc_l2norm_chunk_sel_int(const uint8_t* x_u8, const int32_t* num_frames, const int32_t* src, int B, int T, int F, int every_n, int C2,
                             evc_bf16* out2, evc_f16* out2_int, float* rs2, const int32_t* row_pos2, int rows2, void* stream);

#define EVC_SELECT_CHANGE 6
#define EVC_SELECT_SEGMENT_CHANGE 7
int evc_frame_change_keys(const float* x_f32, const uint8_t* x_u8, const int32_t* num_frames, int B, int T, int F, uint32_t* keys ,
                          void* stream);
int evc_student_frame_select_scored(const int32_t* num_frames, const uint32_t* keys, int B, int T, int every_n, int strategy,
                                    int32_t* src , void* stream);

#define EVC_CONF_TOP1 0
#define EVC_CONF_MARGIN 1
int evc_cascade_confidence_rows(const float* pred, int64_t ld, const uint8_t* active, int rows, int cols, int kind, int stage, float* conf,
                                float* merged, int64_t ld_merged, uint8_t* stage_of, void* stream);
int evc_cascade_pick_rows(const float* conf, const uint8_t* active, const int32_t* num_frames, int rows, float threshold, int max_rows,
                          uint8_t* active_next, int32_t* num_frames_next, int32_t* count, void* stream);

int evc_fill_f32(float* p, int64_t n, float value, void* stream);
int evc_debug_occupy(int blocks, int threads, int lds_bytes, double microseconds, void* stream);
int evc_stream_create_cu_mask(const unsigned* mask, int words, void** stream_out);
int evc_stream_destroy(void* stream);

#ifdef __cplusplus
}
#endif
#endif
```

Before: 8.061 million frames/sec.

## Skip leading dead K-steps in TN weight-grad GEMMs and dead-tile zeroing in LSTM bwd

Adds k_skip variants of the TN weight-gradient GEMMs (row-segmented and slab), so a leading range of K blocks known to contribute nothing is skipped, with split-k planning recomputed over the shortened range. It also adds an LSTM backward entry that avoids zero-filling dz tiles for rows that are never read. A plan query and a strided column fill are added as helpers. The aim is to cut wasted GEMM work and memory writes on padded or inactive timesteps of variable-length sequences. The risk is wrong gradients if the skipped range or the unread rows are ever actually used.

```diff
diff --git a/efficientvideoclassification_youtube8m_amd/_lib.py b/efficientvideoclassification_youtube8m_amd/_lib.py
--- a/efficientvideoclassification_youtube8m_amd/_lib.py
+++ b/efficientvideoclassification_youtube8m_amd/_lib.py
@@ -19,6 +19,10 @@
     "evc_gemm_tn2": [vp, i64, vp, i64, i32, vp, i64, i32, i32, vp, i64, i32, i32, i32, i32, vp],
     "evc_gemm_tn2_rows": [vp, i64, vp, i64, i32, vp, i64, i32, i32, vp, i64, i32, i32, i32, vp, i32, i32, vp],
     "evc_gemm_tn2_slabs": [vp, i64, vp, i64, i32, vp, i64, i32, i32, vp, i64, i64, i32, i32, i32, i32, vp],
+    "evc_gemm_tn2_rows_skip": [vp, i64, vp, i64, i32, vp, i64, i32, i32, vp, i64, i32, i32, i32, vp, i32, i32, i32, vp],
+    "evc_gemm_tn_plan": [i64, i64, i32, i64, i32, i32, i32, i32, vp, i32, vp, vp, vp],
+    "evc_gemm_tn2_slabs_skip": [vp, i64, vp, i64, i32, vp, i64, i32, i32, vp, i64, i64, i32, i32, i32, i32, i32, vp],
+    "evc_fill_f32_cols": [vp, i64, i32, i32, f32, vp],
     "evc_sum_slabs": [vp, i64, i32, i32, i32, i64, vp, i64, i32, vp],
     "evc_colsum_bf16": [vp, i64, i32, i32, i32, vp, vp],
     "evc_colsum_bf16_det": [vp, i64, i32, i32, i32, vp, vp, i32, vp],
@@ -38,6 +42,7 @@
     "evc_cast_f32_to_fp8_lo": [vp, i64, i32, i32, i32, i32, i32, vp, i64, vp],
     "evc_cast_f32_to_fp8_lohi": [vp, i64, i32, i32, i32, i32, i32, vp, i64, vp],
     "evc_lstm_layer_bwd": [vp, vp, i32, i32, i32, i32, vp, vp, vp, vp, i64, vp, vp, vp, vp, vp, vp, vp, vp, vp],
+    "evc_lstm_layer_bwd_live": [vp, vp, i32, i32, i32, i32, vp, vp, vp, vp, i64, vp, vp, vp, vp, vp, vp, vp, vp, i32, vp],
     "evc_transpose_to_bf16": [vp, i32, i64, i32, i32, vp, i64, i32, i32, vp],
     "evc_cast_f32_to_bf16": [vp, i64, i32, i32, vp, i64, vp],
     "evc_cast_f32_to_f16": [vp, i64, i32, i32, vp, i64, vp],
@@ -158,6 +163,7 @@
     "evc_cascade_pick_rows": [vp, vp, vp, i32, f32, i32, vp, vp, vp, vp],
 }
 EXPORTS = tuple(SIGNATURES) + ("evc_version", "evc_last_error")
+NEWER = ("evc_gemm_tn2_rows_skip", "evc_gemm_tn_plan", "evc_gemm_tn2_slabs_skip", "evc_fill_f32_cols", "evc_lstm_layer_bwd_live")
 
 _lib = None
 
@@ -178,6 +184,8 @@
     import torch
     lib = C.CDLL(LIB_PATH)
     for name, args in SIGNATURES.items():
+        if name in NEWER and "EVC_LIB" in os.environ and not hasattr(lib, name):
+            continue
         fn = getattr(lib, name)
         fn.argtypes = args
         fn.restype = C.c_int
@@ -189,6 +197,10 @@
     return lib
 
 
+def has(name):
+    return hasattr(load(), name)
+
+
 def call(name, *args):
     lib = load()
     rc = getattr(lib, name)(*args)
diff --git a/efficientvideoclassification_youtube8m_amd/csrc/evc_elementwise.hip b/efficientvideoclassification_youtube8m_amd/csrc/evc_elementwise.hip
--- a/efficientvideoclassification_youtube8m_amd/csrc/evc_elementwise.hip
+++ b/efficientvideoclassification_youtube8m_amd/csrc/evc_elementwise.hip
@@ -1824,6 +1824,22 @@
   return EVC_OK;
 }
 
+__global__ void fill_cols_kernel(float* p, long ld, int rows, int cols4, float v) {
+  const long n = (long)rows * cols4, stride = (long)gridDim.x * blockDim.x;
+  const float4 v4 = make_float4(v, v, v, v);
+  for (long i = (long)blockIdx.x * blockDim.x + threadIdx.x; i < n; i += stride) {
+    const long r = i / cols4, c = i - r * cols4;
+    *(float4*)(p + r * ld + c * 4) = v4;
+  }
+}
+extern "C" int evc_fill_f32_cols(float* p, int64_t ld, int rows, int cols, float value, void* stream) {
+  EVC_REQUIRE(p && rows > 0 && cols > 0 && cols % 4 == 0 && ld % 4 == 0 && ld >= cols && ((uintptr_t)p % 16) == 0, EVC_ERR_BAD_SHAPE,
+              "evc_fill_f32_cols: rows=%d cols=%d (%%4) ld=%ld (%%4, >= cols), 16-byte aligned", rows, cols, (long)ld);
+  hipLaunchKernelGGL(fill_cols_kernel, dim3(grid_for((long)rows * (cols / 4))), dim3(256), 0, (hipStream_t)stream, p, (long)ld, rows, cols / 4, value);
+  EVC_LAUNCH_CHECK();
+  return EVC_OK;
+}
+
 __global__ void occupy_kernel(long long ticks) {
   extern __shared__ char occ_lds[];
   if (threadIdx.x == 0) occ_lds[0] = 0;
diff --git a/efficientvideoclassification_youtube8m_amd/csrc/evc_gemm_tn.hip b/efficientvideoclassification_youtube8m_amd/csrc/evc_gemm_tn.hip
--- a/efficientvideoclassification_youtube8m_amd/csrc/evc_gemm_tn.hip
+++ b/efficientvideoclassification_youtube8m_amd/csrc/evc_gemm_tn.hip
@@ -5,6 +5,7 @@
   int row_il_H;
   int accumulate, splits, ksteps_per_split;
   long slab_stride;
+  int ksteps_per_split2;
 };
 
 template <class Cfg, bool SEG = false>
@@ -21,18 +22,22 @@
   const int m0 = tm * Cfg::BM;
   int n0 = tn * Cfg::BU;
   int nb = n0;
+  int skip = 0, kps = s.ksteps_per_split;
   if (p.B2) {
     if (n0 >= p.N1) {
       p.B = p.B2; p.ldb = p.ldb2; nb = n0 - p.N1; p.N = s.N - p.N1;
       s.N = p.c_col2 + p.N;
       n0 = p.c_col2 + nb;
+      skip = p.k_skip2; kps = s.ksteps_per_split2;
     } else {
       p.N = s.N = p.N1;
     }
+  } else {
+    skip = p.k_skip2;
   }
   if (SEG) {
-    int off = split * s.ksteps_per_split, sg = 0;
-    p.nk = min(s.ksteps_per_split, p.nk - off);
+    int off = skip + split * kps, sg = 0;
+    p.nk = min(kps, p.nk - off);
 #pragma unroll
     for (int i = 0; i < 15; ++i) {
       const bool adv = sg == i && i + 1 < p.nseg && off >= (int)p.seg_len[i];
@@ -40,11 +45,13 @@
       sg += adv ? 1 : 0;
     }
     p.seg0 = sg; p.seg_off0 = off;
-  } else if (s.splits > 1) {
-    const int k0 = split * s.ksteps_per_split;
+  } else if (s.splits > 1 || skip) {
+    const bool slabs = s.slab_stride > 0;
+    const int k0 = slabs ? max(skip, split * s.ksteps_per_split) : skip + split * kps;
+    const int k1 = slabs ? min((split + 1) * s.ksteps_per_split, p.nk) : min(k0 + kps, p.nk);
     p.A += (long)k0 * 32 * p.lda;
     p.B += (long)k0 * 32 * p.ldb;
-    p.nk = min(s.ksteps_per_split, p.nk - k0);
+    p.nk = k1 - k0;
   }
   f32x4 acc[Cfg::MI][1][Cfg::NI];
   gemm_mainloop_tn<Cfg, true, TN_LOOP_MODE, SEG>(p, m0, nb, lds_dyn, acc);
@@ -121,29 +128,69 @@
 template <class Cfg>
 static int launch_tn(const GemmOperandsT& p, StoreParamsT s, bool seg, int tm, int tn, hipStream_t st) {
   s.ksteps_per_split = ceil_div(p.nk, s.splits);
+  s.ksteps_per_split2 = p.k_skip2 && !s.slab_stride ? ceil_div(p.nk - p.k_skip2, s.splits) : s.ksteps_per_split;
   if (seg) launch_cfg<Cfg>(gemm_tn_kernel<Cfg, true>, tm * tn * s.splits, st, p, s, tm, tn);
   else launch_cfg<Cfg>(gemm_tn_kernel<Cfg>, tm * tn * s.splits, st, p, s, tm, tn);
   EVC_LAUNCH_CHECK();
   return EVC_OK;
 }
 
+enum TnTileId { TN_TILE_256 = 1, TN_TILE_128 = 11 };
+struct TnPlan { int tile, tm, tn, splits; bool seg; };
+
+static TnPlan tn_plan(GemmOperandsT& p, int M, int N, int K, int slab_rows, const int32_t* rows_per_slab, int k_skip) {
+  TnPlan pl;
+  pl.seg = rows_per_slab && slab_rows > 0 && !evc_deterministic() && tn_live_segments(p, K, slab_rows, rows_per_slab);
+  K = p.nk * 32;
+  int skip = k_skip;
+  if (pl.seg) {
+    skip = 0;
+    for (int i = 0; i < p.nseg; ++i) skip += max(0, min((int)p.seg_len[i], k_skip - (int)p.seg_start[i]));
+  }
+  int nk_short = p.nk - skip;
+  if (p.B2) {
+    p.k_skip2 = skip;
+  } else if (skip) {
+    if (pl.seg) {
+      int i = 0, n = 0;
+      while (i < p.nseg && skip >= (int)p.seg_len[i]) skip -= p.seg_len[i++];
+      for (; i < p.nseg; ++i, ++n, skip = 0) {
+        p.seg_start[n] = (unsigned short)(p.seg_start[i] + skip); p.seg_len[n] = (unsigned short)(p.seg_len[i] - skip);
+      }
+      for (i = n; i < 16; ++i) p.seg_start[i] = p.seg_len[i] = 0;
+      p.nseg = n;
+    } else {
+      p.A += (long)skip * 32 * p.lda;
+      p.B += (long)skip * 32 * p.ldb;
+    }
+    p.nk = nk_short;
+  }
+  const int tm1 = ceil_div(M, 128), tn1 = ceil_div(N, 128);
+  const bool short128 = forced_tile() == 11 || (forced_tile() == 0 && K <= 2048 && (long)tm1 * tn1 >= 192);
+  const bool strip128 = !short128 && forced_tile() == 0 && N <= 128 && !p.B2;
+  const bool tile128 = short128 || strip128;
+  const int tm = tile128 ? tm1 : ceil_div(M, CfgPlainV2::BM), tn = short128 ? tn1 : strip128 ? 1 : ceil_div(N, CfgPlainV2::BU);
+  pl.splits = 1;
+  if (!short128 && !evc_deterministic()) {
+    pl.splits = split_k(256 / (tm * tn), nk_short, 32);
+    while (pl.splits > 1 && (long)ceil_div(p.nk, pl.splits) * (pl.splits - 1) >= p.nk) --pl.splits;
+  }
+  pl.tile = tile128 ? TN_TILE_128 : TN_TILE_256;
+  pl.tm = tm; pl.tn = tn;
+  return pl;
+}
+
 static int gemm_tn_impl(const char* entry, const evc_bf16* A, int64_t lda, const evc_bf16* B, int64_t ldb, int N1, const evc_bf16* B2, int64_t ldb2,
                         int c_col2, float* C, int64_t ldc, int M, int N, int K, int row_interleave_H, int accumulate, void* stream,
-                        int slab_rows = 0, const int32_t* rows_per_slab = nullptr) {
+                        int slab_rows = 0, const int32_t* rows_per_slab = nullptr, int k_skip = 0) {
   EVC_TRY(tn_args_ok(entry, A, lda, B, ldb, M, N, K, row_interleave_H, N1, B2, ldb2, c_col2));
+  EVC_REQUIRE(k_skip >= 0 && k_skip <= K / 32, EVC_ERR_BAD_ARG, "%s: k_skip=%d outside [0, K/32=%d]", entry, k_skip, K / 32);
   hipStream_t st = (hipStream_t)stream;
   GemmOperandsT p = tn_operands(A, lda, B, ldb, M, N, K, N1, B2, ldb2, c_col2);
-  const bool seg = rows_per_slab && slab_rows > 0 && !evc_deterministic() && tn_live_segments(p, K, slab_rows, rows_per_slab);
-  K = p.nk * 32;
-  StoreParamsT s{C, ldc, M, N, row_interleave_H, accumulate, 1, 0, 0};
-  const int tm1 = ceil_div(M, 128), tn1 = ceil_div(N, 128);
-  const bool short128 = forced_tile() == 11 || (forced_tile() == 0 && K <= 2048 && (long)tm1 * tn1 >= 192);
-  const bool strip128 = !short128 && forced_tile() == 0 && N <= 128 && !B2;
-  const bool tile128 = short128 || strip128;
-  const int tm = tile128 ? tm1 : ceil_div(M, CfgPlainV2::BM), tn = short128 ? tn1 : strip128 ? 1 : ceil_div(N, CfgPlainV2::BU);
-  if (!short128 && !evc_deterministic()) s.splits = split_k(256 / (tm * tn), p.nk, 32);
+  const TnPlan pl = tn_plan(p, M, N, K, slab_rows, rows_per_slab, k_skip);
+  StoreParamsT s{C, ldc, M, N, row_interleave_H, accumulate, pl.splits, 0, 0};
   if (s.splits > 1 && !accumulate) EVC_CHECK_HIP(hipMemset2DAsync(C, ldc * sizeof(float), 0, (size_t)N * sizeof(float), M, st));
-  return tile128 ? launch_tn<CfgTn128>(p, s, seg, tm, tn, st) : launch_tn<CfgPlainV2>(p, s, seg, tm, tn, st);
+  return pl.tile == TN_TILE_128 ? launch_tn<CfgTn128>(p, s, pl.seg, pl.tm, pl.tn, st) : launch_tn<CfgPlainV2>(p, s, pl.seg, pl.tm, pl.tn, st);
 }
 
 extern "C" int evc_gemm_tn2_rows(const evc_bf16* A, int64_t lda, const evc_bf16* B1, int64_t ldb1, int N1, const evc_bf16* B2, int64_t ldb2,
@@ -157,6 +204,37 @@
                       row_interleave_H, accumulate, stream, slab_rows, rows_per_slab);
 }
 
+static int tn_skip_args_ok(const char* entry, const void* B1, int N1, const void* B2, int N2, int c_col2, int slab_rows, int nslabs, int accumulate) {
+  EVC_REQUIRE(B1 && N1 > 0 && slab_rows > 0 && nslabs > 0 && (long)slab_rows * nslabs < (1L << 31), EVC_ERR_BAD_ARG, "%s: B1, N1, slab_rows, nslabs are required", entry);
+  EVC_REQUIRE(!B2 || N2 > 0, EVC_ERR_BAD_ARG, "%s: N2=%d", entry, N2);
+  EVC_REQUIRE(!B2 || accumulate || c_col2 == N1, EVC_ERR_BAD_ARG, "%s: segments that are not adjacent in C (c_col2=%d, N1=%d) need accumulate", entry, c_col2, N1);
+  return EVC_OK;
+}
+extern "C" int evc_gemm_tn2_rows_skip(const evc_bf16* A, int64_t lda, const evc_bf16* B1, int64_t ldb1, int N1, const evc_bf16* B2, int64_t ldb2,
+                                      int N2, int c_col2, float* C, int64_t ldc, int M, int slab_rows, int nslabs, const int32_t* rows_per_slab,
+                                      int k_skip, int row_interleave_H, int accumulate, void* stream) {
+  EVC_TRY(tn_skip_args_ok("evc_gemm_tn2_rows_skip", B1, N1, B2, N2, c_col2, slab_rows, nslabs, accumulate));
+  return gemm_tn_impl("evc_gemm_tn2_rows_skip", A, lda, B1, ldb1, B2 ? N1 : 0, B2, ldb2, B2 ? c_col2 : 0, C, ldc, M, N1 + (B2 ? N2 : 0), slab_rows * nslabs,
+                      row_interleave_H, accumulate, stream, slab_rows, rows_per_slab, k_skip);
+}
+
+extern "C" int evc_gemm_tn_plan(int64_t lda, int64_t ldb1, int N1, int64_t ldb2, int N2, int M, int slab_rows, int nslabs, const int32_t* rows_per_slab,
+                                int k_skip, int* tile, int* splits, int* live_walk) {
+  EVC_REQUIRE(tile && splits && live_walk, EVC_ERR_BAD_ARG, "evc_gemm_tn_plan: tile, splits and live_walk are required");
+  const bf16_t* const some = (const bf16_t*)(uintptr_t)16;
+  const bf16_t* const B2 = N2 > 0 ? some : nullptr;
+  EVC_TRY(tn_skip_args_ok("evc_gemm_tn_plan", some, N1, B2, N2, N1, slab_rows, nslabs, 1));
+  const int N = N1 + (B2 ? N2 : 0), K = slab_rows * nslabs;
+  EVC_TRY(tn_args_ok("evc_gemm_tn_plan", some, lda, some, ldb1, M, N, K, 0, B2 ? N1 : 0, B2, ldb2, B2 ? N1 : 0));
+  EVC_REQUIRE(k_skip >= 0 && k_skip <= K / 32, EVC_ERR_BAD_ARG, "evc_gemm_tn_plan: k_skip=%d outside [0, K/32=%d]", k_skip, K / 32);
+  GemmOperandsT p = tn_operands(some, lda, some, ldb1, M, N, K, B2 ? N1 : 0, B2, ldb2, B2 ? N1 : 0);
+  const TnPlan pl = tn_plan(p, M, N, K, slab_rows, rows_per_slab, k_skip);
+  *tile = pl.tile;
+  *splits = pl.splits;
+  *live_walk = pl.seg ? 1 : 0;
+  return EVC_OK;
+}
+
 extern "C" int evc_gemm_tn(const evc_bf16* A, int64_t lda, const evc_bf16* B, int64_t ldb, float* C, int64_t ldc,
                            int M, int N, int K, int row_interleave_H, int accumulate, void* stream) {
   return gemm_tn_impl("evc_gemm_tn", A, lda, B, ldb, 0, nullptr, 0, 0, C, ldc, M, N, K, row_interleave_H, accumulate, stream);
@@ -171,12 +249,22 @@
 }
 
 static int gemm_tn_slabs_impl(const char* entry, const evc_bf16* A, int64_t lda, const evc_bf16* B1, int64_t ldb1, int N1, const evc_bf16* B2, int64_t ldb2,
-                              int N2, int c_col2, float* slabs, int64_t ldc, int64_t slab_stride, int M, int K, int row_interleave_H, int nslab, void* stream) {
+                              int N2, int c_col2, float* slabs, int64_t ldc, int64_t slab_stride, int M, int K, int row_interleave_H, int nslab, void* stream,
+                              int k_skip = 0) {
   const int N = N1 + (B2 ? N2 : 0);
   EVC_REQUIRE(N1 >= 8, EVC_ERR_BAD_SHAPE, "%s: N1=%d", entry, N1);
   EVC_TRY(tn_args_ok(entry, A, lda, B1, ldb1, M, N, K, row_interleave_H, N1, B2, ldb2, c_col2, nslab, slabs && slab_stride >= (int64_t)M * ldc));
-  return launch_tn<CfgPlainV2>(tn_operands(A, lda, B1, ldb1, M, N, K, N1, B2, ldb2, c_col2), StoreParamsT{slabs, ldc, M, N, row_interleave_H, 0, nslab, 0, slab_stride},
+  EVC_REQUIRE(k_skip >= 0 && k_skip <= K / 32, EVC_ERR_BAD_ARG, "%s: k_skip=%d outside [0, K/32=%d]", entry, k_skip, K / 32);
+  GemmOperandsT p = tn_operands(A, lda, B1, ldb1, M, N, K, N1, B2, ldb2, c_col2);
+  p.k_skip2 = k_skip;
+  return launch_tn<CfgPlainV2>(p, StoreParamsT{slabs, ldc, M, N, row_interleave_H, 0, nslab, 0, slab_stride},
                                false, ceil_div(M, CfgPlainV2::BM), ceil_div(N, CfgPlainV2::BU), (hipStream_t)stream);
+}
+extern "C" int evc_gemm_tn2_slabs_skip(const evc_bf16* A, int64_t lda, const evc_bf16* B1, int64_t ldb1, int N1, const evc_bf16* B2, int64_t ldb2,
+                                       int N2, int c_col2, float* slabs, int64_t ldc, int64_t slab_stride, int M, int K, int k_skip, int row_interleave_H,
+                                       int nslab, void* stream) {
+  return gemm_tn_slabs_impl("evc_gemm_tn2_slabs_skip", A, lda, B1, ldb1, N1, B2, ldb2, N2, c_col2, slabs, ldc, slab_stride, M, K, row_interleave_H, nslab, stream,
+                            k_skip);
 }
 extern "C" int evc_gemm_tn2_slabs(const evc_bf16* A, int64_t lda, const evc_bf16* B1, int64_t ldb1, int N1, const evc_bf16* B2, int64_t ldb2,
                                   int N2, int c_col2, float* slabs, int64_t ldc, int64_t slab_stride, int M, int K, int row_interleave_H,
diff --git a/efficientvideoclassification_youtube8m_amd/csrc/evc_lstm_bwd.hip b/efficientvideoclassification_youtube8m_amd/csrc/evc_lstm_bwd.hip
--- a/efficientvideoclassification_youtube8m_amd/csrc/evc_lstm_bwd.hip
+++ b/efficientvideoclassification_youtube8m_amd/csrc/evc_lstm_bwd.hip
@@ -14,6 +14,7 @@
   int m_active;
   int M, H;
   int fused_above;
+  int dead_unread = 0;
 };
 
 static inline int bwd_dc_bf16() {
@@ -105,6 +106,10 @@
   else *(float4*)(e.dc_ws + hu) = make_float4(dcn[0], dcn[1], dcn[2], dcn[3]);
   dzp[0] = make_uint4(dzr[0].x, dzr[0].y, dzr[1].x, dzr[1].y);
   dzp[1] = make_uint4(dzr[2].x, dzr[2].y, dzr[3].x, dzr[3].y);
+}
+
+__device__ __forceinline__ bool lstm_bwd_dead_tile_read(const LstmBwdParams& e, int m0) {
+  return !e.dead_unread || m0 < ((e.m_active + 31) & ~31);
 }
 
 template <int BM, int BU, int NT>
@@ -278,7 +283,7 @@
   tile_of(id, tiles_m, tiles_n, tm, tn);
   const int m0 = tm * Cfg::BM, u0 = tn * Cfg::BU;
   if (m0 >= e.m_active) {
-    lstm_bwd_zero_tile<Cfg::BM, Cfg::BU, Cfg::NT>(e, m0, u0);
+    if (lstm_bwd_dead_tile_read(e, m0)) lstm_bwd_zero_tile<Cfg::BM, Cfg::BU, Cfg::NT>(e, m0, u0);
     return;
   }
   f32x4 acc[Cfg::MI][1][Cfg::NI];
@@ -363,7 +368,7 @@
   const int tm = id % tiles_m, tn = id / tiles_m;
   const int m0 = tm * 32, u0 = tn * 32;
   if (m0 >= e.m_active) {
-    lstm_bwd_zero_tile<32, 32, NT>(e, m0, u0);
+    if (lstm_bwd_dead_tile_read(e, m0)) lstm_bwd_zero_tile<32, 32, NT>(e, m0, u0);
     return;
   }
   const int lane = threadIdx.x & 63;
@@ -513,11 +518,11 @@
 typedef TileCfg2<160, 1, 128, 2, 4, 5, true> CfgBwdV2_160;
 typedef TileCfg2<192, 1, 128, 2, 4, 5, true> CfgBwdV2_192;
 
-extern "C" int evc_lstm_layer_bwd(const evc_bf16* w_il, const int32_t* len, int T, int M, int Kin, int H,
-                                  const void* gates, const evc_bf16* c_all, const float* dS_c, const float* dS_h, int64_t ld_dS,
-                                  const evc_bf16* dh_above, float* dc_ws, evc_bf16* dz4, float* db,
-                                  const int32_t* row_map, const int32_t* rows_per_step, const evc_bf16* dz_above,
-                                  const evc_bf16* w_above, void* stream) {
+static int lstm_layer_bwd_impl(const evc_bf16* w_il, const int32_t* len, int T, int M, int Kin, int H,
+                               const void* gates, const evc_bf16* c_all, const float* dS_c, const float* dS_h, int64_t ld_dS,
+                               const evc_bf16* dh_above, float* dc_ws, evc_bf16* dz4, float* db,
+                               const int32_t* row_map, const int32_t* rows_per_step, const evc_bf16* dz_above,
+                               const evc_bf16* w_above, int dz_dead_unread, void* stream) {
   EVC_REQUIRE(T > 0 && M > 0 && H > 0 && Kin > 0 && H % 64 == 0, EVC_ERR_BAD_SHAPE, "evc_lstm_layer_bwd: bad shape");
   EVC_REQUIRE(ring_operand_ok(M, 4L * H) && ring_operand_ok(H, 4L * H), EVC_ERR_BAD_SHAPE,
               "evc_lstm_layer_bwd: a dz time slab spans 4 GiB or more (M=%d H=%d)", M, H);
@@ -570,6 +575,7 @@
     e.dc_bf16 = bwd_dc_bf16();
     e.row_map = row_map; e.db = db; e.m_active = Mt;
     e.M = M; e.H = H; e.fused_above = dz_above ? 1 : 0;
+    e.dead_unread = dz_dead_unread;
     switch (pick) {
       case 0: launch_lstm_bwd<CfgBwdV2_192>(p, e, k1, st); break;
       case 1: launch_lstm_bwd<CfgBwdV2_160>(p, e, k1, st); break;
@@ -592,6 +598,24 @@
   }
   EVC_LAUNCH_CHECK();
   return EVC_OK;
+}
+
+extern "C" int evc_lstm_layer_bwd(const evc_bf16* w_il, const int32_t* len, int T, int M, int Kin, int H,
+                                  const void* gates, const evc_bf16* c_all, const float* dS_c, const float* dS_h, int64_t ld_dS,
+                                  const evc_bf16* dh_above, float* dc_ws, evc_bf16* dz4, float* db,
+                                  const int32_t* row_map, const int32_t* rows_per_step, const evc_bf16* dz_above,
+                                  const evc_bf16* w_above, void* stream) {
+  return lstm_layer_bwd_impl(w_il, len, T, M, Kin, H, gates, c_all, dS_c, dS_h, ld_dS, dh_above, dc_ws, dz4, db, row_map, rows_per_step, dz_above, w_above, 0, stream);
+}
+extern "C" int evc_lstm_layer_bwd_live(const evc_bf16* w_il, const int32_t* len, int T, int M, int Kin, int H,
+                                       const void* gates, const evc_bf16* c_all, const float* dS_c, const float* dS_h, int64_t ld_dS,
+                                       const evc_bf16* dh_above, float* dc_ws, evc_bf16* dz4, float* db,
+                                       const int32_t* row_map, const int32_t* rows_per_step, const evc_bf16* dz_above,
+                                       const evc_bf16* w_above, int dz_dead_unread, void* stream) {
+  EVC_REQUIRE(dz_dead_unread == 0 || (dz_dead_unread == 1 && rows_per_step && !dz_above), EVC_ERR_BAD_ARG,
+              "evc_lstm_layer_bwd_live: dz_dead_unread goes with rows_per_step and without dz_above");
+  return lstm_layer_bwd_impl(w_il, len, T, M, Kin, H, gates, c_all, dS_c, dS_h, ld_dS, dh_above, dc_ws, dz4, db, row_map, rows_per_step, dz_above, w_above,
+                             dz_dead_unread, stream);
 }
 
 extern "C" int evc_lstm_stack2_bwd(const evc_bf16* w_il0, const evc_bf16* w_il1, const int32_t* len, int T, int M, int Kin0, int H,
diff --git a/efficientvideoclassification_youtube8m_amd/csrc/gemm_core_tn.h b/efficientvideoclassification_youtube8m_amd/csrc/gemm_core_tn.h
--- a/efficientvideoclassification_youtube8m_amd/csrc/gemm_core_tn.h
+++ b/efficientvideoclassification_youtube8m_amd/csrc/gemm_core_tn.h
@@ -10,6 +10,7 @@
   int nk;
   const bf16_t* B2 = nullptr; long ldb2 = 0; int N1 = 0;
   int c_col2 = 0;
+  int k_skip2 = 0;
   int nseg = 0, seg0 = 0, seg_off0 = 0;
   unsigned short seg_start[16] = {0}, seg_len[16] = {0};
 };
@@ -32,7 +33,7 @@
 #pragma unroll
     for (int ni = 0; ni < Cfg::NI; ++ni) acc[mi][0][ni] = f32x4{0.f, 0.f, 0.f, 0.f};
   const int nk = p.nk;
-  if (nk == 0) return;
+  if (nk <= 0) return;
 
   constexpr bool PRODUCERS = (MODE & LOOP_PRODUCER) != 0 && Cfg::NT == 512;
   constexpr int NPW = PRODUCERS ? 4 : Cfg::NT / 64;
diff --git a/efficientvideoclassification_youtube8m_amd/engine.py b/efficientvideoclassification_youtube8m_amd/engine.py
--- a/efficientvideoclassification_youtube8m_amd/engine.py
+++ b/efficientvideoclassification_youtube8m_amd/engine.py
@@ -91,6 +91,8 @@
     fwd_walk2_high = False
     bwd_fuse = "off"
     small_pair = False
+    wgrad_zero_work = True
+    bwd_skip_dead = True
     timing = None
     timing_bwd = None
 
@@ -119,7 +121,14 @@
             n *= d
         return buf.view(-1)[:n].view(*shape)
 
+    _h0_zero = False
+
     def forward(self, x, lens, plan=None):
+        S = self._forward(x, lens, plan)
+        self._h0_zero = True
+        return S
+
+    def _forward(self, x, lens, plan=None):
         tw, H, L, T = self.tw, self.H, self.L, self.T
         M = plan.P if plan is not None else self.M
         self.plan, self.Mrun = plan, M
@@ -341,27 +350,56 @@
             inp = self._hb[l][1:]
         return res
 
-    def _wgrad_tn(self, dz2, layer_in, h_prev, kin, rows, gW, live=None):
+    def _wgrad_tn(self, dz2, layer_in, h_prev, kin, rows, gW, live=None, k_skip=0, assign=False):
         H = self.H
         n1 = kin // 256 * 256
         if ops.DETERMINISTIC and rows % 32 == 0 and kin % 8 == 0:
+            acc = not assign
             if n1 >= 256 and (kin == n1 or kin - n1 >= 8):
-                ops.gemm_tn_det(dz2, layer_in, 4 * H, n1, rows, gW, row_interleave_H=H, accumulate=True, ldc=kin + H, B2=h_prev, N2=H, c_col2=kin)
+                ops.gemm_tn_det(dz2, layer_in, 4 * H, n1, rows, gW, row_interleave_H=H, accumulate=acc, ldc=kin + H, B2=h_prev, N2=H, c_col2=kin, k_skip=k_skip)
                 if kin > n1:
-                    ops.gemm_tn_det(dz2, layer_in[:, n1:], 4 * H, kin - n1, rows, gW[:, n1:kin], row_interleave_H=H, accumulate=True, ldc=kin + H)
+                    ops.gemm_tn_det(dz2, layer_in[:, n1:], 4 * H, kin - n1, rows, gW[:, n1:kin], row_interleave_H=H, accumulate=acc, ldc=kin + H)
             else:
-                ops.gemm_tn_det(dz2, layer_in, 4 * H, kin, rows, gW, row_interleave_H=H, accumulate=True, ldc=kin + H)
-                ops.gemm_tn_det(dz2, h_prev, 4 * H, H, rows, gW[:, kin:], row_interleave_H=H, accumulate=True, ldc=kin + H)
+                ops.gemm_tn_det(dz2, layer_in, 4 * H, kin, rows, gW, row_interleave_H=H, accumulate=acc, ldc=kin + H)
+                ops.gemm_tn_det(dz2, h_prev, 4 * H, H, rows, gW[:, kin:], row_interleave_H=H, accumulate=acc, ldc=kin + H, k_skip=k_skip)
             return
+        lda, ldx, ldh, ldc = dz2.stride(0), layer_in.stride(0), h_prev.stride(0), kin + H
         if kin == H and kin % 256 == 0:
-            ops.gemm_tn2(dz2, layer_in, kin, h_prev, H, 4 * H, rows, gW, row_interleave_H=H, accumulate=True, live_rows=live)
+            launches = [([(0, kin + H)], dict(N1=kin, ldb1=ldx, N2=H, ldb2=ldh, k_skip=k_skip),
+                         lambda acc: ops.gemm_tn2(dz2, layer_in, kin, h_prev, H, 4 * H, rows, gW, row_interleave_H=H, accumulate=acc, live_rows=live, k_skip=k_skip))]
         elif kin - n1 in (64, 128) and n1 >= H and rows >= 16384 and (n1 + H) % 2048 == 0:
-            ops.gemm_tn2(dz2, layer_in, n1, h_prev, H, 4 * H, rows, gW, row_interleave_H=H, accumulate=True, c_col2=kin, live_rows=live)
-            ops.gemm_tn(dz2, layer_in[:, n1:], 4 * H, kin - n1, rows, gW[:, n1:kin], row_interleave_H=H, lda=dz2.stride(0),
-                        ldb=layer_in.stride(0), ldc=kin + H, accumulate=True, live_rows=live)
+            launches = [([(0, n1), (kin, kin + H)], dict(N1=n1, ldb1=ldx, N2=H, ldb2=ldh, k_skip=k_skip),
+                         lambda acc: ops.gemm_tn2(dz2, layer_in, n1, h_prev, H, 4 * H, rows, gW, row_interleave_H=H, accumulate=acc, c_col2=kin, live_rows=live,
+                                                  k_skip=k_skip)),
+                        ([(n1, kin)], dict(N1=kin - n1, ldb1=ldx),
+                         lambda acc: ops.gemm_tn(dz2, layer_in[:, n1:], 4 * H, kin - n1, rows, gW[:, n1:kin], row_interleave_H=H, lda=lda, ldb=ldx, ldc=ldc,
+                                                 accumulate=acc, live_rows=live))]
         else:
-            ops.gemm_tn(dz2, layer_in, 4 * H, kin, rows, gW, row_interleave_H=H, ldc=kin + H, accumulate=True, live_rows=live)
-            ops.gemm_tn(dz2, h_prev, 4 * H, H, rows, gW[:, kin:], row_interleave_H=H, ldc=kin + H, accumulate=True, live_rows=live)
+            launches = [([(0, kin)], dict(N1=kin, ldb1=ldx),
+                         lambda acc: ops.gemm_tn(dz2, layer_in, 4 * H, kin, rows, gW, row_interleave_H=H, ldc=ldc, accumulate=acc, live_rows=live)),
+                        ([(kin, kin + H)], dict(N1=H, ldb1=ldh, k_skip=k_skip),
+                         lambda acc: ops.gemm_tn(dz2, h_prev, 4 * H, H, rows, gW[:, kin:], row_interleave_H=H, ldc=ldc, accumulate=acc, live_rows=live, k_skip=k_skip))]
+        if not assign or not ops.TN_PLAN:
+            if assign:
+                ops.fill_f32(gW, 0.0)
+            for _, _, launch in launches:
+                launch(True)
+            return
+        acc = [ops.gemm_tn_plan(4 * H, K=rows, lda=lda, live_rows=live, **plan)[1] > 1 or len(cols) > 1 for cols, plan, _ in launches]
+        if all(acc):
+            ops.fill_f32(gW, 0.0)
+        else:
+            for (cols, _, _), a in zip(launches, acc):
+                for c0, c1 in (cols if a else ()):
+                    ops.fill_f32_cols(gW[:, c0:c1], 0.0)
+        for (_, _, launch), a in zip(launches, acc):
+            launch(a)
+
+    def _h0_skip(self, l, h_prev, M):
+        if not (self.wgrad_zero_work and self._h0_zero and ops.TN_PLAN and M % 32 == 0):
+            return 0
+        assert h_prev.data_ptr() == self.hbuf[l].data_ptr() and h_prev.stride(0) == self.H, "the skip is for the h image forward() cleared"
+        return M // 32
 
     def backward(self, dS, need_dx, aux=None, on_layer_grads=None):
         return drain(self.backward_layers(dS, need_dx, aux, on_layer_grads))
@@ -401,8 +439,9 @@
                     dz2 = dz[l].view(T * M, 4 * H)
                     layer_in = (self.x_in if l == 0 else self._hb[0][1:]).reshape(T * M, kin)
                     h_prev = self._hb[l][:T].reshape(T * M, H)
-                    ops.fill_f32(gW, 0.0)
-                    self._wgrad_tn(dz2, layer_in, h_prev, kin, T * M, gW)
+                    if not self.wgrad_zero_work:
+                        ops.fill_f32(gW, 0.0)
+                    self._wgrad_tn(dz2, layer_in, h_prev, kin, T * M, gW, k_skip=self._h0_skip(l, h_prev, M), assign=self.wgrad_zero_work)
                     if on_layer_grads is not None:
                         on_layer_grads(l)
             if need_dx:
@@ -430,12 +469,14 @@
                 ops.fill_f32(gb, 0.0)
             fused = fuse_ok and self.bwd_fuse == "fused" and l + 1 < L
             rows = plan.rows if plan is not None else [M] * T
+            dead_unread = bool(self.bwd_skip_dead and plan is not None and M % 32 == 0 and use_tn and not det and not (fuse_ok and self.bwd_fuse != "off") and ops.TN_PLAN
+                               and ops.gemm_tn_plan(4 * H, H, T * M, lda=4 * H, ldb1=max(kin, H), live_rows=(rows, M))[2])
             with self._timed("bwd_step", sum(1 for r in rows if r > 0), sum(2.0 * r * H * 4 * H for r in rows[1:])):
                 ops.lstm_layer_bwd(w, self.lens, T, M, kin, H, self._v(self.gates[l], T, M, H, 2), self._v(self.c_all[l], T + 1, M, H),
                                    dS[:, (2 * l) * H:], dS[:, (2 * l + 1) * H:], 2 * L * H,
                                    dh_above, self._v(self.dc_ws, M, H), dz, plan=plan, db=None if det else gb,
                                    dz_above=self._v(self.dz[l + 1], T, M, 4 * H) if fused else None,
-                                   w_above=tw.shadow_bwd[self.names(l + 1)[0]] if fused else None)
+                                   w_above=tw.shadow_bwd[self.names(l + 1)[0]] if fused else None, dz_dead_unread=dead_unread)
             ops.mark("%s:%s_bptt%d_done" % (tw.scope, self.scope, l))
             dz2 = dz.view(T * M, 4 * H)
             if l > 0 and fuse_ok and self.bwd_fuse == "fused":
@@ -463,9 +504,11 @@
                 if det:
                     ops.colsum_bf16(dz2, T * M, 4 * H, gb, deinterleave_H=H)
                 if use_tn:
-                    ops.fill_f32(gW, 0.0)
+                    if not self.wgrad_zero_work:
+                        ops.fill_f32(gW, 0.0)
                     with self._timed("wgrad_tn", 1, 2.0 * (sum(rows) if plan is not None else T * M) * 4 * H * (kin + H), stream=side):
-                        self._wgrad_tn(dz2, layer_in, h_prev, kin, T * M, gW, live=(rows, M) if plan is not None and M % 32 == 0 else None)
+                        self._wgrad_tn(dz2, layer_in, h_prev, kin, T * M, gW, live=(rows, M) if plan is not None and M % 32 == 0 else None,
+                                       k_skip=self._h0_skip(l, h_prev, M), assign=self.wgrad_zero_work)
                 else:
                     ops.transpose_to_bf16(dz2, T * M, 4 * H, self.dzT, KP, interleave_H=-H)
                     inT = self.xT[:kin]
diff --git a/efficientvideoclassification_youtube8m_amd/ops.py b/efficientvideoclassification_youtube8m_amd/ops.py
--- a/efficientvideoclassification_youtube8m_amd/ops.py
+++ b/efficientvideoclassification_youtube8m_amd/ops.py
@@ -78,19 +78,36 @@
     return M > 512 and N % 256 == 0 and K % 64 == 0 and K < 8192 and os.environ.get("EVC_FUSED_GRAD_NORM", "0") == "1"
 
 
-def gemm_tn(A, B, M, N, K, out, row_interleave_H=0, accumulate=False, lda=None, ldb=None, ldc=None, live_rows=None):
+def _tn_rows_args(live_rows, K, k_skip):
+    if live_rows is not None:
+        return _slab_rows_arg(live_rows, K)
+    return K, 1, None
+
+
+def gemm_tn_plan(M, N1, K, lda, ldb1, N2=0, ldb2=0, live_rows=None, k_skip=0):
+    slab, ns, arr = _tn_rows_args(live_rows, K, k_skip)
+    tile, splits, walk = C.c_int(0), C.c_int(0), C.c_int(0)
+    _lib.call("evc_gemm_tn_plan", lda, ldb1, N1, ldb2, N2, M, slab, ns, arr, k_skip, C.byref(tile), C.byref(splits), C.byref(walk))
+    return tile.value, splits.value, bool(walk.value)
+
+
+def gemm_tn(A, B, M, N, K, out, row_interleave_H=0, accumulate=False, lda=None, ldb=None, ldc=None, live_rows=None, k_skip=0):
     assert A.dtype == BF16 and B.dtype == BF16 and out.dtype == F32
+    lda, ldb, ldc = A.stride(0) if lda is None else lda, B.stride(0) if ldb is None else ldb, out.stride(0) if ldc is None else ldc
+    if k_skip:
+        slab, ns, arr = _tn_rows_args(live_rows, K, k_skip)
+        _lib.call("evc_gemm_tn2_rows_skip", _p(A), lda, _p(B), ldb, N, None, 0, 0, 0, _p(out), ldc, M, slab, ns, arr, k_skip, row_interleave_H,
+                  1 if accumulate else 0, _stream())
+        return out
     if live_rows is not None:
         slab, ns, arr = _slab_rows_arg(live_rows, K)
-        _lib.call("evc_gemm_tn2_rows", _p(A), A.stride(0) if lda is None else lda, _p(B), B.stride(0) if ldb is None else ldb, N, None, 0, 0, 0,
-                  _p(out), out.stride(0) if ldc is None else ldc, M, slab, ns, arr, row_interleave_H, 1 if accumulate else 0, _stream())
+        _lib.call("evc_gemm_tn2_rows", _p(A), lda, _p(B), ldb, N, None, 0, 0, 0, _p(out), ldc, M, slab, ns, arr, row_interleave_H, 1 if accumulate else 0, _stream())
         return out
-    _lib.call("evc_gemm_tn", _p(A), A.stride(0) if lda is None else lda, _p(B), B.stride(0) if ldb is None else ldb,
-              _p(out), out.stride(0) if ldc is None else ldc, M, N, K, row_interleave_H, 1 if accumulate else 0, _stream())
-    return out
-
-
-def gemm_tn_det(A, B, M, N, K, out, row_interleave_H=0, accumulate=False, ldc=None, B2=None, N2=0, c_col2=None):
+    _lib.call("evc_gemm_tn", _p(A), lda, _p(B), ldb, _p(out), ldc, M, N, K, row_interleave_H, 1 if accumulate else 0, _stream())
+    return out
+
+
+def gemm_tn_det(A, B, M, N, K, out, row_interleave_H=0, accumulate=False, ldc=None, B2=None, N2=0, c_col2=None, k_skip=0):
     assert A.dtype == BF16 and B.dtype == BF16 and out.dtype == F32
     ldc = out.stride(0) if ldc is None else ldc
     ntot = (c_col2 + N2) if B2 is not None else N
@@ -99,22 +116,32 @@
     while nslab > 1 and ((K // 32 + nslab - 1) // nslab) * (nslab - 1) >= K // 32:
         nslab -= 1
     ws = torch.empty((nslab, M, ntot), dtype=F32, device=out.device)
-    _lib.call("evc_gemm_tn2_slabs", _p(A), A.stride(0), _p(B), B.stride(0), N, _p(B2), B2.stride(0) if B2 is not None else 0, N2,
-              (c_col2 if c_col2 is not None else N), _p(ws), ntot, M * ntot, M, K, row_interleave_H, nslab, _stream())
+    args = (_p(A), A.stride(0), _p(B), B.stride(0), N, _p(B2), B2.stride(0) if B2 is not None else 0, N2,
+            (c_col2 if c_col2 is not None else N), _p(ws), ntot, M * ntot, M, K)
+    if k_skip:
+        _lib.call("evc_gemm_tn2_slabs_skip", *args, k_skip, row_interleave_H, nslab, _stream())
+    else:
+        _lib.call("evc_gemm_tn2_slabs", *args, row_interleave_H, nslab, _stream())
     for c0, w in ((0, N),) + (((c_col2, N2),) if B2 is not None else ()):
         _lib.call("evc_sum_slabs", _p(ws[0, :, c0:]), M * ntot, nslab, M, w, ntot, _p(out[:, c0:]), ldc, 1 if accumulate else 0, _stream())
     return out
 
 
-def gemm_tn2(A, B1, N1, B2, N2, M, K, out, row_interleave_H=0, accumulate=False, ldc=None, c_col2=None, live_rows=None):
+def gemm_tn2(A, B1, N1, B2, N2, M, K, out, row_interleave_H=0, accumulate=False, ldc=None, c_col2=None, live_rows=None, k_skip=0):
     assert A.dtype == BF16 and B1.dtype == BF16 and B2.dtype == BF16 and out.dtype == F32
+    ldc, c_col2 = out.stride(0) if ldc is None else ldc, N1 if c_col2 is None else c_col2
+    if k_skip:
+        slab, ns, arr = _tn_rows_args(live_rows, K, k_skip)
+        _lib.call("evc_gemm_tn2_rows_skip", _p(A), A.stride(0), _p(B1), B1.stride(0), N1, _p(B2), B2.stride(0), N2, c_col2, _p(out), ldc, M, slab, ns, arr, k_skip,
+                  row_interleave_H, 1 if accumulate else 0, _stream())
+        return out
     if live_rows is not None:
         slab, ns, arr = _slab_rows_arg(live_rows, K)
-        _lib.call("evc_gemm_tn2_rows", _p(A), A.stride(0), _p(B1), B1.stride(0), N1, _p(B2), B2.stride(0), N2, N1 if c_col2 is None else c_col2,
-                  _p(out), out.stride(0) if ldc is None else ldc, M, slab, ns, arr, row_interleave_H, 1 if accumulate else 0, _stream())
+        _lib.call("evc_gemm_tn2_rows", _p(A), A.stride(0), _p(B1), B1.stride(0), N1, _p(B2), B2.stride(0), N2, c_col2,
+                  _p(out), ldc, M, slab, ns, arr, row_interleave_H, 1 if accumulate else 0, _stream())
         return out
-    _lib.call("evc_gemm_tn2", _p(A), A.stride(0), _p(B1), B1.stride(0), N1, _p(B2), B2.stride(0), N2, N1 if c_col2 is None else c_col2,
-              _p(out), out.stride(0) if ldc is None else ldc, M, K, row_interleave_H, 1 if accumulate else 0, _stream())
+    _lib.call("evc_gemm_tn2", _p(A), A.stride(0), _p(B1), B1.stride(0), N1, _p(B2), B2.stride(0), N2, c_col2,
+              _p(out), ldc, M, K, row_interleave_H, 1 if accumulate else 0, _stream())
     return out
 
 
@@ -122,6 +149,24 @@
     assert t.dtype == F32 and t.is_contiguous()
     _lib.call("evc_fill_f32", _p(t), t.numel(), float(value), _stream())
 
+
+def fill_f32_cols(t, value):
+    assert t.dtype == F32 and t.dim() == 2 and t.stride(1) == 1
+    _lib.call("evc_fill_f32_cols", _p(t), t.stride(0), t.shape[0], t.shape[1], float(value), _stream())
+
+
+class _Once:
+
+    def __init__(self, ask):
+        self.ask, self.v = ask, None
+
+    def __bool__(self):
+        if self.v is None:
+            self.v = bool(self.ask())
+        return self.v
+
+
+TN_PLAN = _Once(lambda: _lib.has("evc_gemm_tn_plan"))
 
 DETERMINISTIC = os.environ.get("EVC_DETERMINISTIC", "0") not in ("", "0")
 
@@ -543,7 +588,11 @@
 
 
 def lstm_layer_bwd(w_il, lens, T, M, Kin, H, gates, c_all, dS_c, dS_h, ld_dS, dh_above, dc_ws, dz4, plan=None, db=None,
-                   dz_above=None, w_above=None):
+                   dz_above=None, w_above=None, dz_dead_unread=False):
+    if dz_dead_unread:
+        _lib.call("evc_lstm_layer_bwd_live", _p(w_il), _p(lens), T, M, Kin, H, _p(gates), _p(c_all), _p(dS_c), _p(dS_h), ld_dS,
+                  _p(dh_above), _p(dc_ws), _p(dz4), _p(db), *_plan_args(plan), _p(dz_above), _p(w_above), 1, _stream())
+        return
     _lib.call("evc_lstm_layer_bwd", _p(w_il), _p(lens), T, M, Kin, H, _p(gates), _p(c_all), _p(dS_c), _p(dS_h), ld_dS,
               _p(dh_above), _p(dc_ws), _p(dz4), _p(db), *_plan_args(plan), _p(dz_above), _p(w_above), _stream())
 
diff --git a/include/evc.h b/include/evc.h
--- a/include/evc.h
+++ b/include/evc.h
@@ -103,6 +103,11 @@
                        const evc_bf16* dh_above, float* dc_ws, evc_bf16* dz4, float* db,
                        const int32_t* row_map, const int32_t* rows_per_step, const evc_bf16* dz_above,
                        const evc_bf16* w_above, void* stream);
+int evc_lstm_layer_bwd_live(const evc_bf16* w_il, const int32_t* len, int T, int M, int Kin, int H,
+                       const void* gates, const evc_bf16* c_all, const float* dS_c, const float* dS_h, int64_t ld_dS,
+                       const evc_bf16* dh_above, float* dc_ws, evc_bf16* dz4, float* db,
+                       const int32_t* row_map, const int32_t* rows_per_step, const evc_bf16* dz_above,
+                       const evc_bf16* w_above, int dz_dead_unread, void* stream);
 
 int evc_moe_grad_update(const evc_bf16* dlogits, int64_t ld_dlogits, const evc_bf16* x, int64_t ldx, int rows,
                         int V, int K, float* p, float* m, float* v, evc_bf16* p_bf16, evc_bf16* pT_bf16, int64_t ldT,
@@ -286,6 +291,14 @@
 int evc_gemm_tn2_rows(const evc_bf16* A, int64_t lda, const evc_bf16* B1, int64_t ldb1, int N1, const evc_bf16* B2, int64_t ldb2,
                       int N2, int c_col2, float* C, int64_t ldc, int M, int slab_rows, int nslabs, const int32_t* rows_per_slab,
                       int row_interleave_H, int accumulate, void* stream);
+int evc_gemm_tn2_rows_skip(const evc_bf16* A, int64_t lda, const evc_bf16* B1, int64_t ldb1, int N1, const evc_bf16* B2, int64_t ldb2,
+                           int N2, int c_col2, float* C, int64_t ldc, int M, int slab_rows, int nslabs, const int32_t* rows_per_slab,
+                           int k_skip, int row_interleave_H, int accumulate, void* stream);
+int evc_gemm_tn_plan(int64_t lda, int64_t ldb1, int N1, int64_t ldb2, int N2, int M, int slab_rows, int nslabs, const int32_t* rows_per_slab,
+                     int k_skip, int* tile, int* splits, int* live_walk);
+int evc_gemm_tn2_slabs_skip(const evc_bf16* A, int64_t lda, const evc_bf16* B1, int64_t ldb1, int N1, const evc_bf16* B2, int64_t ldb2,
+                            int N2, int c_col2, float* slabs, int64_t ldc, int64_t slab_stride, int M, int K, int k_skip, int row_interleave_H,
+                            int nslab, void* stream);
 int evc_gemm_tn_slabs(const evc_bf16* A, int64_t lda, const evc_bf16* B, int64_t ldb, float* slabs, int M, int N, int K,
                       int nslab, void* stream);
 int evc_gemm_tn2_slabs(const evc_bf16* A, int64_t lda, const evc_bf16* B1, int64_t ldb1, int N1, const evc_bf16* B2, int64_t ldb2,
@@ -406,6 +419,7 @@
                           uint8_t* active_next, int32_t* num_frames_next, int32_t* count, void* stream);
 
 int evc_fill_f32(float* p, int64_t n, float value, void* stream);
+int evc_fill_f32_cols(float* p, int64_t ld, int rows, int cols, float value, void* stream);
 int evc_debug_occupy(int blocks, int threads, int lds_bytes, double microseconds, void* stream);
 int evc_stream_create_cu_mask(const unsigned* mask, int words, void** stream_out);
 int evc_stream_destroy(void* stream);
```

Result: faster. 8.143 million frames/sec (median of 6 runs) (+1.0%).
